# wenz116/lang2seg

Measured on AMD Instinct MI355X. Metric: train images/sec (cycle loss on), 600×1000 input, at 1/2/4/8 MI355X, higher is better.
Workload: dtype bf16; 1 GPU; train_cycle.sh step: ResNet-101 C4 + 7 spatial dynamic filters + att2in2 cycle loss, 600x1000 image, 20-token expression (V=3349), 12000->2000 proposals, 256 RoIs, per-GPU batch 1; variant=cycle, parallelism=dp1

## Files before the change

### include/lang2seg_hip.h

```cpp
#ifndef LANG2SEG_HIP_H
#define LANG2SEG_HIP_H
#include <stdint.h>
#ifdef __HIPCC__
#include <hip/hip_runtime.h>
#else
typedef struct ihipStream_t* hipStream_t;
#endif
#ifdef __cplusplus
extern "C" {
#endif

#define L2S_F32 0
#define L2S_BF16 1

int l2s_version(void);

#define L2S_CONV_RELU 1
#define L2S_CONV_OUT_F32 4
#define L2S_CONV_DECONV2X2 8
#define L2S_CONV_SCATTER 16
#define L2S_ALGO_AUTO 0
#define L2S_ALGO_STAGED 1
#define L2S_ALGO_DMA 2
#define L2S_ALGO_DMA_STAMPED 4
// ... 333 lines not shown
typedef struct { int roi; int cls; float box[4]; float score; int area; } l2s_det_record;
size_t l2s_detect_ws_bytes(int post, int ncls);
int l2s_detect_nms(const float* cls_prob, const float* bbox_pred, const float* rois, const int* nkeep, int post, int ncls, float im_scale,
                   int im_h, int im_w, int bbox_reg, float thresh, float nms_thresh, void* ws, float* boxes_dump, hipStream_t s);
int l2s_detect_select(const void* ws, int post, int ncls, int max_per_image, float im_scale, l2s_det_record* rec, float* mask_rois,
                      int* mask_labels, int cap, int* count, hipStream_t s);
int l2s_detect_paste(const float* mask_prob, int ms, l2s_det_record* rec, const int* count, int cap, int ih, int iw, uint8_t* canvases,
                     hipStream_t s);

typedef struct { int I; int U; int hit; int reserved; } l2s_det_gt;
typedef struct { int det; int cls; int hit; int reserved; long long I; long long U; double key; } l2s_det_choice;
int l2s_detect_gt_iou(const uint8_t* canvases, const l2s_det_record* rec, const int* count, int cap, int ih, int iw, const uint8_t* gt, int Hs,
                      int Ws, const float* gt_box, float im_scale, l2s_det_gt* out, int* gt_area, hipStream_t s);
int l2s_detect_choose(const l2s_det_record* rec, const l2s_det_gt* gt, const int* count, int cap, const int* gt_area, const float* expr,
                      const float* lambdas, int n_lambda, int per_token, int n_tok, l2s_det_choice* out, hipStream_t s);

int l2s_decode_pick(const float* logits, int V1, int t, int sample_max, float temperature, const float* u_in, const uint64_t* seed_dev,
                    uint64_t salt, int* finished, int64_t* seq, float* seq_logprobs, int64_t* next_token, hipStream_t s);
#define L2S_BEAM_MAX 16
#define L2S_BEAM_MAX_T 64
#define L2S_BEAM_RECORD_WORDS(T) (2 * (T) + 2)
typedef struct {
  const float* logits; int ld_logits;
  int V1, B, t, T, R, n_state;
  int* beam_seq; float* beam_seq_logprobs; float* beam_logprobs_sum;
  const float* state_in[4]; float* state_out[4]; int ld_in[4], ld_out[4];
  int64_t* next_tokens; int* parents;
  int* done; int* done_count;
} l2s_beam_step_args;
int l2s_decode_beam_step(const l2s_beam_step_args* a, hipStream_t s);
int l2s_decode_beam_step_rows(const l2s_beam_step_args* a, int rows, int row0, const int* count, hipStream_t s);
int l2s_decode_beam_finish_rows(const int* done, const int* done_count, int B, int T, int rows, int row0, const int* count,
                                int64_t* beam_seq, float* beam_logps, float* beam_p, int* beam_n, int64_t* seq, float* logprobs, hipStream_t s);
int l2s_mask_resize_nearest(const uint8_t* src, int ih, int iw, uint8_t* dst, int H, int W, hipStream_t s);

#define L2S_ROWS_MAX_W 8192
int l2s_masks_to_map(const uint8_t* masks, int rows, int row0, const int* count, int mh, int mw, int H, int W, int Hc, int Wc, float* out,
                     hipStream_t s);
int l2s_adaptive_pool_rows(const void* x, const float* pm, void* y, int rows, int row0, const int* count, int H, int W, int C, int OH, int OW,
                           int ldy, int dtype, hipStream_t s);
int l2s_cap_att_dots_rows(const float* patt, const float* att_h, int ld_att_h, const float* aw, const float* ab, int rows, int row0,
                          const int* count, int L, int D, float* dots, hipStream_t s);
int l2s_cap_apply_gates_rows(const float* P, const float* dots, const float* b_a2c, const float* sums, int ld_sums, const float* c_prev,
                             float* c, float* h, int rows, int row0, const int* count, int L, int R, hipStream_t s);
int l2s_decode_pick_rows(const float* logits, int ld_logits, int V1, int rows, int row0, const int* count, int t, int T, const int64_t* forced,
                         int* finished, int64_t* seq, float* logprobs, int64_t* next_token, float* sum, hipStream_t s);
int l2s_decode_force_rows(const float* logits, int ld_logits, int V1, int rows, int row0, const int* count, int t, int T, const int64_t* targets,
                          const int* lengths, float* logprobs, int64_t* next_token, float* sum, hipStream_t s);
typedef struct { const float* x; int ldx; const float* w; int ld; int n; } l2s_rows_seg;
typedef struct { const float* pre; int ld_pre; const float* pre2; int ld_pre2; const float* add0; const float* add1; l2s_rows_seg seg[2];
                 const float* c_prev; int ld_c_prev; float* c; int ld_c; float* h; int ld_h; } l2s_lstm_rows;
int l2s_lstm_cell_rows(const l2s_lstm_rows* a, int R, int rows, int row0, const int* count, hipStream_t s);
int l2s_cap_att_apply_rows(const float* att, const float* dots, float* att_res, int ld_res, int rows, int row0, const int* count, int L, int R,
                           hipStream_t s);
int l2s_cap_att_dots_groups(const float* patt, const float* att_h, int ld_att_h, const float* aw, const float* ab, int rows, int group,
                            int row0, const int* count, int L, int D, float* dots, hipStream_t s);
int l2s_cap_apply_gates_groups(const float* P, const float* dots, const float* b_a2c, const float* sums, int ld_sums, const float* c_prev,
                               float* c, float* h, int rows, int group, int row0, const int* count, int L, int R, hipStream_t s);
int l2s_cap_att_apply_groups(const float* att, const float* dots, float* att_res, int ld_res, int rows, int group, int row0,
                             const int* count, int L, int R, hipStream_t s);
int l2s_lstm_cell_groups(const l2s_lstm_rows* a, int R, int rows, int group, int row0, const int* count, hipStream_t s);

int l2s_stream_fork(hipStream_t from, hipStream_t to);
int l2s_event_record(int slot, hipStream_t s);
int l2s_event_wait(int slot, hipStream_t s);
int l2s_memset_async(void* p, int value, size_t bytes, hipStream_t s);
int l2s_memcpy_d2d_async(void* dst, const void* src, size_t bytes, hipStream_t s);
void* l2s_tape_begin(const hipStream_t* streams, int n);
int l2s_tape_end(void* tape);
long l2s_tape_size(void* tape);
int l2s_tape_run(void* tape, const hipStream_t* streams, int n);
int l2s_tape_pause(int on);
int l2s_tape_mark(void);
int l2s_tape_time_event(hipStream_t s);
int l2s_time_event_elapsed(int a, int b, float* ms);
int l2s_tape_segments(void* tape);
int l2s_tape_run_segment(void* tape, const hipStream_t* streams, int n, int seg);
int l2s_tape_destroy(void* tape);

typedef struct { long offset; long count; int row_len; int weight_decay; long rowscale_off; float lr_mult;
                 int chunk0;
                 int flags;
                 int reserved; } l2s_sgd_seg;
int l2s_sgd_momentum_range(float* param, float* grad, float* mom, const l2s_sgd_seg* segs, int nseg, const float* rowscale,
                           float lr, float momentum, float wd, float grad_scale, void* shadow, int shadow_dtype, int flags,
                           long lo, long hi, int chunk_lo, int chunk_hi, hipStream_t s);
int l2s_sgd_momentum_range_g16(float* param, const void* grad_bf16, long grad_lo, float* mom, const l2s_sgd_seg* segs, int nseg, const float* rowscale,
                               float lr, float momentum, float wd, float grad_scale, void* shadow, int shadow_dtype,
                               long lo, long hi, int chunk_lo, int chunk_hi, hipStream_t s);
int l2s_sgd_chunk(void);
int l2s_sgd_momentum(float* param, float* grad, float* mom, const l2s_sgd_seg* segs, int nseg, const float* rowscale,
                     float lr, float momentum, float wd, float grad_scale, void* shadow ,
                     int shadow_dtype, int clear_grad ,
                     hipStream_t s);

#ifdef __cplusplus
}
#endif
#endif
```

### lang2seg_amd/_lib.py

```python
import ctypes as C
import os

_HERE = os.path.dirname(os.path.abspath(__file__))
LIB_PATH = os.path.join(_HERE, 'lib', 'liblang2seg_hip.so')
F32, BF16 = 0, 1

vp, i32, i64, f32, u64, sz = C.c_void_p, C.c_int, C.c_long, C.c_float, C.c_uint64, C.c_size_t


class ConvDesc(C.Structure):
    _fields_ = [('x', vp), ('w', vp), ('y', vp), ('bias', vp), ('add', vp), ('ref', vp),
                ('n_img', i32), ('IH', i32), ('IW', i32), ('Cin', i32), ('OH', i32), ('OW', i32), ('Cout', i32),
                ('KH', i32), ('KW', i32), ('stride', i32), ('pad', i32),
                ('ldx', i32), ('ldy', i32), ('ldadd', i32), ('ldref', i32), ('flags', i32),
                ('out_h', i32), ('out_w', i32), ('out_stride', i32), ('tile', i32), ('split_k', i32), ('xcd_mode', i32), ('algo', i32), ('ws', vp), ('ws_floats', sz), ('prio', i32)]


class RoiBlock0Desc(C.Structure):
    _fields_ = [('feat', vp), ('rois', vp), ('w1', vp), ('b1', vp), ('w2', vp), ('b2', vp), ('pooled', vp), ('y1', vp), ('y2', vp),
                ('H', i32), ('W', i32), ('C', i32), ('R', i32), ('P', i32), ('N1', i32), ('N2', i32), ('spatial_scale', C.c_float), ('debug', i32)]


class WgradDesc(C.Structure):
    _fields_ = [('dy', vp), ('x', vp), ('dw', vp),
                ('n_img', i32), ('IH', i32), ('IW', i32), ('Cin', i32), ('OH', i32), ('OW', i32), ('Cout', i32),
                ('KH', i32), ('KW', i32), ('stride', i32), ('pad', i32), ('lddy', i32), ('ldx', i32),
                ('split_k', i32), ('tile', i32), ('ws', vp), ('ws_bytes', sz)]


class WgradProb(C.Structure):
    _fields_ = [('dy', vp * 2), ('x', vp * 2), ('n_img', i32 * 2), ('IH', i32 * 2), ('IW', i32 * 2), ('OH', i32 * 2), ('OW', i32 * 2),
                ('lddy', i32 * 2), ('ldx', i32 * 2), ('dw', vp),
                ('nseg', i32), ('Cin', i32), ('Cout', i32), ('KH', i32), ('KW', i32), ('stride', i32), ('pad', i32),
                ('split', i32), ('ws_off', i64), ('flags', i32), ('reserved', i32)]


class TransposeDesc(C.Structure):
    _fields_ = [('src', vp), ('scale', vp), ('dst', vp), ('Cout', i32), ('taps', i32), ('Cin', i32), ('force_f32', i32)]


class LstmFwdDir(C.Structure):
    _fields_ = [(n, C.c_void_p) for n in ('w_hh', 'b_hh', 'gates_in', 'h_prev', 'c_prev', 'c', 'h', 'act', 'gates_out')]


class LstmBwdDir(C.Structure):
    _fields_ = [(n, C.c_void_p) for n in ('w_hh_T', 'dgates_next', 'dh_ext', 'dc_in', 'act', 'c_prev', 'c', 'dgates', 'dc_prev')]


class GruFwdDir(C.Structure):
    _fields_ = [(n, C.c_void_p) for n in ('w_hh', 'b_hh', 'gates_in', 'h_prev', 'h', 'act')]


class GruBwdDir(C.Structure):
    _fields_ = [(n, C.c_void_p) for n in ('w_hh_T', 'dgh_next', 'dh_ext', 'dh_carry_in', 'act', 'h_prev', 'dgi', 'dgh', 'dh_carry_out')]


class RnnFwdDir(C.Structure):
    _fields_ = [(n, C.c_void_p) for n in ('w_hh', 'b_hh', 'gates_in', 'h_prev', 'h')]


class RnnBwdDir(C.Structure):
    _fields_ = [(n, C.c_void_p) for n in ('w_hh_T', 'dg_next', 'dh_ext', 'h', 'dg')]


class TopdownSeg(C.Structure):
    _fields_ = [('x', vp), ('w', vp), ('ld', i32), ('n', i32)]


class TopdownFwd(C.Structure):
    _fields_ = [('pre', vp), ('add0', vp), ('add1', vp), ('seg', TopdownSeg * 2), ('c_prev', vp), ('c', vp), ('h', vp), ('act', vp)]


class TopdownBwd(C.Structure):
    _fields_ = [('seg', TopdownSeg * 3), ('add0', vp), ('add1', vp), ('dc_in', vp), ('act', vp), ('c_prev', vp), ('c', vp), ('dgates', vp),
                ('dc_prev', vp)]


class RowsSeg(C.Structure):
    _fields_ = [('x', vp), ('ldx', i32), ('w', vp), ('ld', i32), ('n', i32)]


class LstmRows(C.Structure):
    _fields_ = [('pre', vp), ('ld_pre', i32), ('pre2', vp), ('ld_pre2', i32), ('add0', vp), ('add1', vp), ('seg', RowsSeg * 2),
                ('c_prev', vp), ('ld_c_prev', i32), ('c', vp), ('ld_c', i32), ('h', vp), ('ld_h', i32)]


class AdaattFwd(C.Structure):
    _fields_ = [(n, vp) for n in ('pre', 'fcrow', 'w_hh', 'b_hh', 'w_r', 'b_r')] + [('ld_hh', i32), ('ld_r', i32)] + \
               [(n, vp) for n in ('h_prev', 'c_prev', 'c', 'h', 'fake', 'save')]


class AdaattBwd(C.Structure):
    _fields_ = [(n, vp) for n in ('dsn', 't_hh', 't_r')] + [('ld_thh', i32), ('ld_tr', i32)] + \
               [(n, vp) for n in ('dh_ext', 'dfake', 'dc_in', 'save', 'c_prev', 'ds', 'dc_prev')]


class Bottleneck64Desc(C.Structure):
    _fields_ = [(n, vp) for n in ('a', 'x', 'w2', 'w3', 'wd', 'w1n', 'b2', 'b3', 'bd', 'b1n', 'y', 'a_next')] + [(n, i32) for n in ('H', 'W', 'Cx')]


class CapRecurFwdArgs(C.Structure):
    _fields_ = [(n, vp) for n in ('w_h2h', 'b_h2h', 'w_h2att', 'b_h2att', 'patt', 'aw', 'ab', 'P', 'b_a2c', 'sums', 'hs', 'cs', 'save', 'tanh_ws', 'wgt', 'state')] + \
               [(n, i32) for n in ('S', 'R', 'AH', 'L')]


class CapRecurBwdArgs(C.Structure):
    _fields_ = [(n, vp) for n in ('w_h2h', 'w_h2att', 'P', 'aw', 'save', 'cs', 'wgt', 'tanh_ws', 'dho', 'dsums', 'da2c', 'ddot', 'datt_h', 'state')] + \
               [(n, i32) for n in ('S', 'R', 'AH', 'L', 'ld_ddot', 'ld_datt_h')]


class BeamStepArgs(C.Structure):
    _fields_ = [('logits', vp), ('ld_logits', i32)] + [(n, i32) for n in ('V1', 'B', 't', 'T', 'R', 'n_state')] + \
               [(n, vp) for n in ('beam_seq', 'beam_seq_logprobs', 'beam_logprobs_sum')] + \
               [('state_in', vp * 4), ('state_out', vp * 4), ('ld_in', i32 * 4), ('ld_out', i32 * 4)] + \
               [(n, vp) for n in ('next_tokens', 'parents', 'done', 'done_count')]


class SgdSeg(C.Structure):
    _fields_ = [('offset', i64), ('count', i64), ('row_len', i32), ('weight_decay', i32), ('rowscale_off', i64),
                ('lr_mult', f32), ('chunk0', i32), ('flags', i32), ('reserved', i32)]


CONV_RELU, CONV_OUT_F32, CONV_DECONV2X2, CONV_SCATTER = 1, 4, 8, 16
LOSS_RPN_CLS, LOSS_RPN_BOX, LOSS_CLS, LOSS_BOX, LOSS_MASK, LOSS_CAP, LOSS_TOTAL, LOSS_RESPONSE = range(8)

SIGS = {
    'l2s_version': (i32, []),
    'l2s_conv_plan_name': (C.c_char_p, [vp, i32]),
    'l2s_last_kernel': (C.c_char_p, []),
    'l2s_roialign_block0_fwd': (i32, [C.POINTER(RoiBlock0Desc), vp]),
    'l2s_conv_igemm': (i32, [C.POINTER(ConvDesc), i32, vp]),
    'l2s_conv_wgrad': (i32, [C.POINTER(WgradDesc), i32, vp]),
    'l2s_wgrad_ws_bytes': (sz, [C.POINTER(WgradDesc), i32]),
    'l2s_wgrad_variant': (i32, [i32, i32, i32, i32, i32, i32, i32, i64, i32]),
    'l2s_wgrad_tiles': (i64, [i32, i32, i32, i32, i32]),
    'l2s_conv_wgrad_grouped': (i32, [vp, vp, i32, i32, i32, vp, sz, vp]),
    'l2s_weight_cast': (i32, [vp, vp, vp, i32, i32, i32, i32, vp]),
    'l2s_weight_transpose': (i32, [vp, vp, vp, i32, i32, i32, i32, vp]),
    'l2s_colsum': (i32, [vp, i32, i32, i32, vp, vp, i64, i32, vp]),
    'l2s_weight_transpose_batched': (i32, [vp, i32, i32, i32, vp]),
    'l2s_stem_conv': (i32, [vp, vp, vp, vp, vp, i32, i32, i32, i32, i32, vp]),
    'l2s_stem_pack_bytes': (C.c_size_t, []),
    'l2s_stem_pack': (i32, [vp, vp, vp]),
    'l2s_stem_pool_bf16': (i32, [vp, vp, vp, vp, vp, i32, i32, i32, i32, i32, i32, vp]),
    'l2s_maxpool3x3s2': (i32, [vp, vp, i32, i32, i32, i32, i32, i32, vp]),
    'l2s_fill_f32': (i32, [vp, f32, i64, vp]),
    'l2s_cast': (i32, [vp, i32, vp, i32, i64, vp]),
    'l2s_add3': (i32, [vp, vp, vp, vp, i64, i32, vp]),
    'l2s_avgpool_fwd': (i32, [vp, vp, i32, i32, i32, i32, vp]),
    'l2s_avgpool_bwd': (i32, [vp, vp, vp, vp, i32, i32, i32, i32, vp]),
    'l2s_adaptive_pool_fwd': (i32, [vp, vp, vp, i32, i32, i32, i32, i32, i32, i32, vp]),
    'l2s_adaptive_pool_bwd': (i32, [vp, i32, i32, i32, vp, vp, vp, i32, i32, i32, i32, i32, i32, vp]),
    'l2s_mask_downsample': (i32, [vp, vp, i32, i32, i32, i32, vp]),
    'l2s_dropout_mask': (i32, [vp, i64, f32, vp, u64, vp]),
    'l2s_counter_inc': (i32, [vp, vp]),
    'l2s_stamp': (i32, [vp, vp]),
    'l2s_rpn_decode': (i32, [vp, i32, vp, i32, i32, i32, i32, f32, f32, vp, vp, vp, vp]),
    'l2s_sort_topk': (i32, [vp, vp, i32, i32, vp, vp, vp, vp, vp]),
    'l2s_nms_workspace_bytes': (sz, [i32]),
    'l2s_sort_ws_ints': (i64, [i32]),
    'l2s_nms': (i32, [vp, i32, f32, i32, i32, vp, vp, vp, vp]),
    'l2s_gather_rois': (i32, [vp, vp, vp, vp, i32, vp, vp, vp]),
    'l2s_random_keys': (i32, [vp, i64, vp, u64, vp]),
    'l2s_anchor_target_ws_ints': (i64, [i32]),
    'l2s_anchor_target': (i32, [vp, i32, vp, i32, i32, i32, i32, f32, f32, vp, vp, f32, f32, i32, f32, vp, vp, vp, vp, vp, vp]),
    'l2s_proposal_target': (i32, [vp, vp, vp, i32, vp, i32, vp, i32, i32, vp, vp, vp, i32, i32, i32, f32, f32, f32,
                                  vp, vp, vp, i32, i32, vp, vp, vp, vp, vp, vp, vp, vp, vp]),
    'l2s_roialign_fwd': (i32, [vp, i32, i32, i32, vp, i32, i32, f32, vp, i32, vp]),
    'l2s_roialign_bwd': (i32, [vp, i32, i32, i32, vp, i32, i32, f32, vp, i32, vp]),
    'l2s_rpn_loss': (i32, [vp, i32, vp, vp, vp, vp, i32, i32, i32, f32, f32, vp, vp, i32, i32, vp, vp, vp]),
    'l2s_anchor_target_count': (vp, [vp]),
    'l2s_rcnn_loss': (i32, [vp, i32, vp, vp, vp, vp, i32, i32, f32, vp, vp, i32, i32, vp]),
    'l2s_mask_loss': (i32, [vp, i32, vp, vp, vp, i32, i32, f32, vp, vp, vp]),
    'l2s_total_loss': (i32, [vp, f32, vp]),
    'l2s_maskpred_ws_floats': (i64, [i32, i32]),
    'l2s_maskpred_bwd': (i32, [vp, vp, vp, i32, i32, i32, vp, vp, vp, vp, vp, vp, vp, i32, vp]),
    'l2s_maskpred_bwd_dx': (i32, [vp, vp, vp, i32, i32, i32, vp, vp, vp, vp, vp, i32, vp]),
    'l2s_maskpred_bwd_reduce': (i32, [vp, vp, vp, i32, i32, vp, vp, vp]),
    'l2s_linear_fwd': (i32, [vp, i32, vp, i32, vp, vp, i32, i32, i32, i32, i32, i32, vp]),
    'l2s_linear_bwd_x': (i32, [vp, i32, vp, vp, i32, i32, i32, i32, i32, vp, vp, i64, vp]),
    'l2s_linear_bwd_x_ws_floats': (i64, [i32, i32, i32]),
    'l2s_linear_bwd_w': (i32, [vp, i32, vp, i32, vp, vp, i32, i32, i32, vp]),
    'l2s_act_bwd': (i32, [vp, vp, i64, i32, vp]),
    'l2s_mask_relu_cast': (i32, [vp, vp, vp, vp, i32, i64, vp]),
    'l2s_embed_fwd': (i32, [vp, vp, vp, vp, i32, i32, i32, vp]),
    'l2s_embed_bwd': (i32, [vp, vp, vp, vp, vp, i32, i32, i32, vp]),
    'l2s_lstm_cell_fwd': (i32, [vp, vp, vp, vp, vp, i32, vp]),
    'l2s_lstm_cell_bwd': (i32, [vp, vp, vp, vp, vp, vp, vp, i32, vp]),
    'l2s_dynfilter_fwd': (i32, [vp, vp, vp, vp, vp, vp, i32, i32, i32, i32, i32, vp]),
    'l2s_dynfilter_ws_floats': (i64, [i32, i32, i32]),
    'l2s_dynfilter_bwd': (i32, [vp, vp, vp, vp, vp, vp, vp, vp, vp, vp, vp, i32, i32, i32, i32, i32, vp, vp]),
    'l2s_dynfilter_bwd_finish': (i32, [vp, vp, vp, vp, i32, i32, i32, vp]),
    'l2s_scale_mask': (i32, [vp, vp, vp, vp, C.c_long, i32, vp]),
    'l2s_conv3x3_c3': (i32, [vp, vp, vp, vp, i32, i32, i32, vp]),
    'l2s_maxpool2x2_fwd': (i32, [vp, vp, i32, i32, i32, i32, i32, vp]),
    'l2s_maxpool2x2_bwd': (i32, [vp, vp, vp, i32, i32, i32, i32, i32, i32, vp]),
    'l2s_cropalign_fwd': (i32, [vp, i32, i32, i32, vp, i32, i32, f32, f32, vp, i32, vp]),
    'l2s_cropalign_bwd': (i32, [vp, i32, i32, i32, vp, i32, i32, f32, f32, vp, i32, vp]),
    'l2s_roipool_fwd': (i32, [vp, i32, i32, i32, vp, i32, i32, f32, vp, vp, i32, vp]),
    'l2s_roipool_bwd': (i32, [vp, vp, i32, i32, i32, vp, i32, vp]),
    'l2s_rle_from_string': (i32, [C.c_char_p, vp, i32]),
    'l2s_prep_geometry': (i32, [i32, i32, i32, i32, C.POINTER(C.c_double), C.POINTER(i32), C.POINTER(i32)]),
    'l2s_prep_image': (i32, [vp, i32, i32, C.c_double, C.c_double, C.c_double, C.c_double, i32, i32, vp, vp]),
    'l2s_rle_ws_words': (i64, [i32, i32, i32]),
    'l2s_rle_to_mask': (i32, [vp, vp, i32, i32, i32, i32, i32, i32, vp, vp, vp]),
    'l2s_eval_pick': (i32, [vp, vp, vp, vp, i32, i32, f32, i32, i32, vp, i32, vp, vp, vp, vp]),
    'l2s_eval_mask_iou': (i32, [vp, i32, vp, vp, i32, i32, i32, i32, vp, vp]),
    'l2s_rle_encode_ws_words': (i64, [i32, i32]),
    'l2s_rle_encode_chunk_rows': (i32, []),
    'l2s_rle_from_mask': (i32, [vp, i32, i32, vp, i32, vp, vp, vp, vp]),
    'l2s_rle_from_masks': (i32, [vp, i32, vp, i32, i32, vp, i32, vp, vp, vp, vp]),
    'l2s_rle_to_string': (i32, [vp, i32, C.c_char_p, i32]),
    'l2s_detect_ws_bytes': (sz, [i32, i32]),
    'l2s_detect_nms': (i32, [vp, vp, vp, vp, i32, i32, f32, i32, i32, i32, f32, f32, vp, vp, vp]),
    'l2s_detect_select': (i32, [vp, i32, i32, i32, f32, vp, vp, vp, i32, vp, vp]),
    'l2s_detect_paste': (i32, [vp, i32, vp, vp, i32, i32, i32, vp, vp]),
    'l2s_detect_gt_iou': (i32, [vp, vp, vp, i32, i32, i32, vp, i32, i32, vp, f32, vp, vp, vp]),
    'l2s_detect_choose': (i32, [vp, vp, vp, i32, vp, vp, C.POINTER(f32), i32, i32, i32, vp, vp]),
    'l2s_decode_pick': (i32, [vp, i32, i32, i32, f32, vp, vp, u64, vp, vp, vp, vp, vp]),
# ... 129 lines not shown
```

### lang2seg_amd/csrc/conv_wgrad.hip

```cpp
#include "wgrad_common.h"
#include <stdlib.h>

namespace {
using namespace l2s_wgrad;

template <typename T> struct WGT;
template <> struct WGT<bf16_t> { static constexpr int BKP = 32; static constexpr int PADB = 32; };
template <> struct WGT<float> { static constexpr int BKP = 16; static constexpr int PADB = 64; };

template <typename T, int BM, int BN, int TX, int D, int KSTEP = 1, int WGM = 2, int WGN = 2>
__device__ __forceinline__ void wgrad_tile(const wgp& p, int co0, int ci0, int tg, int split_idx, int nsplit, float* out, bool accumulate, char* smem) {
  constexpr int ES = (int)sizeof(T);
  constexpr int VE = 16 / ES;
  constexpr int BKP0 = WGT<T>::BKP;
  constexpr int BKP = BKP0 * KSTEP;
  constexpr int RB = BKP + TX - 1;
  constexpr int NT = 64 * WGM * WGN;
  constexpr int WM = BM / WGM, WN = BN / WGN, TM = WM / 16, TN = WN / 16;
  constexpr int LRA = BM * ES + WGT<T>::PADB, LRB = BN * ES + WGT<T>::PADB;
  constexpr int VPA = BM / VE, VPB = BN / VE;
  constexpr int TPR = NT / BKP;
  static_assert(NT % BKP == 0 && VPA % TPR == 0 && VPB % TPR == 0, "loader mapping");
  constexpr int NVA = VPA / TPR, NVB = VPB / TPR;
  constexpr int BUF = BKP * LRA + RB * LRB;

  const int tid = threadIdx.x, lane = tid & 63, wave = tid >> 6;
  const int wm = wave / WGN, wn = wave % WGN;
  const int ky = TX == 3 ? tg : tg / p.KW, kx = TX == 3 ? 0 : tg - ky * p.KW;
  const int fr = lane & 15, fg = lane >> 4;

  f32x4 acc[TX][TM][TN];
#pragma unroll
  for (int t = 0; t < TX; ++t)
#pragma unroll
    for (int i = 0; i < TM; ++i)
#pragma unroll
      for (int j = 0; j < TN; ++j) acc[t][i][j] = (f32x4){0.f, 0.f, 0.f, 0.f};

  auto compute = [&](int cur) {
    const char* a = smem + cur * BUF;
    const char* b = a + BKP * LRA;
    if constexpr (sizeof(T) == 2) {
      const int trow0 = 4 * fg + ((lane >> 2) & 3), tcol = 8 * (lane & 3);
#pragma unroll
      for (int h = 0; h < KSTEP; ++h) {
        const int trow = trow0 + h * 32;
        uint4 fa[TM];
#pragma unroll
        for (int i = 0; i < TM; ++i) fa[i] = lds_frag(a + trow * LRA + (wm * WM + i * 16) * 2 + tcol, LRA);
#pragma unroll
        for (int t = 0; t < TX; ++t) {
          uint4 fb[TN];
#pragma unroll
          for (int j = 0; j < TN; ++j) fb[j] = lds_frag(b + (trow + t) * LRB + (wn * WN + j * 16) * 2 + tcol, LRB);
#pragma unroll
          for (int i = 0; i < TM; ++i)
#pragma unroll
            for (int j = 0; j < TN; ++j)
              acc[t][i][j] = __builtin_amdgcn_mfma_f32_16x16x32_bf16(__builtin_bit_cast(bf16x8, fb[j]), __builtin_bit_cast(bf16x8, fa[i]), acc[t][i][j], 0, 0, 0);
        }
      }
    } else {
#pragma unroll
      for (int ks = 0; ks < BKP / 4; ++ks) {
        float fa[TM];
#pragma unroll
        for (int i = 0; i < TM; ++i) fa[i] = *(const float*)(a + (ks * 4 + fg) * LRA + (wm * WM + i * 16 + fr) * 4);
#pragma unroll
        for (int t = 0; t < TX; ++t) {
          float fb[TN];
#pragma unroll
          for (int j = 0; j < TN; ++j) fb[j] = *(const float*)(b + (ks * 4 + fg + t) * LRB + (wn * WN + j * 16 + fr) * 4);
#pragma unroll
          for (int i = 0; i < TM; ++i)
#pragma unroll
            for (int j = 0; j < TN; ++j) acc[t][i][j] = __builtin_amdgcn_mfma_f32_16x16x4f32(fb[j], fa[i], acc[t][i][j], 0, 0, 0);
        }
      }
    }
  };

#pragma unroll
  for (int seg = 0; seg < L2S_WGRAD_MAX_SEG; ++seg) {
    if (seg >= p.nseg) break;
    const int n_img = p.n_img[seg], IH = p.IH[seg], IW = p.IW[seg], OH = p.OH[seg], OW = p.OW[seg], lddy = p.lddy[seg], ldx = p.ldx[seg];
    const int Wv = OW + (TX == 3 ? 1 : 0);
    const int ohwv = OH * Wv;
    const int Mv = n_img * ohwv;
    int sa, sb, sc;
    slice_step(BKP, ohwv, Wv, sa, sb, sc);
    const int nslices = (Mv + BKP - 1) / BKP;
    const int per = (nslices + nsplit - 1) / nsplit;
    const int s_begin = split_idx * per;
    const int NS = max(0, min(nslices, s_begin + per) - s_begin);
// ... 24 lines not shown
      const int ix = TX == 3 ? x : x * p.stride - p.pad + kx;
      const bool ok = n < n_img && x >= 0 && x < OW && iy >= 0 && iy < IH && ix >= 0 && ix < IW;
      return ok ? (unsigned)(((n * IH + iy) * IW + ix) * ldx * ES) + bcol : OOR;
    };
    auto issue = [&](uint4 (&ra)[NVA], uint4 (&rb)[NVB], uint4 (&rt)[NVB]) {
      {
        const bool ok = ax < OW && an < n_img;
        const unsigned o = ok ? (unsigned)((((an * OH + ay) * OW + ax) * lddy) * ES) + acol : OOR;
#pragma unroll
        for (int j = 0; j < NVA; ++j) ra[j] = __builtin_bit_cast(uint4, __builtin_amdgcn_raw_buffer_load_b128(rdy, acok[j] ? o + j * 16 : OOR, 0, 0));
        advance(an, ay, ax);
      }
      {
        const unsigned o = xoff(bn, by, bx);
#pragma unroll
        for (int j = 0; j < NVB; ++j) rb[j] = __builtin_bit_cast(uint4, __builtin_amdgcn_raw_buffer_load_b128(rxx, bcok[j] ? o + j * 16 : OOR, 0, 0));
        advance(bn, by, bx);
      }
      if (TX == 3) {
        const unsigned o = tail ? xoff(tn, ty, tx) : OOR;
#pragma unroll
        for (int j = 0; j < NVB; ++j) rt[j] = __builtin_bit_cast(uint4, __builtin_amdgcn_raw_buffer_load_b128(rxx, bcok[j] ? o + j * 16 : OOR, 0, 0));
        advance(tn, ty, tx);
      }
    };
    auto store_slice = [&](int buf, const uint4 (&ra)[NVA], const uint4 (&rb)[NVB], const uint4 (&rt)[NVB]) {
      char* a = smem + buf * BUF + lrow * LRA + lq * NVA * 16;
      char* b = smem + buf * BUF + BKP * LRA + lrow * LRB + lq * NVB * 16;
#pragma unroll
      for (int j = 0; j < NVA; ++j) *(uint4*)(a + j * 16) = ra[j];
#pragma unroll
      for (int j = 0; j < NVB; ++j) *(uint4*)(b + j * 16) = rb[j];
      if (TX == 3 && tail) {
#pragma unroll
        for (int j = 0; j < NVB; ++j) *(uint4*)(b + BKP * LRB + j * 16) = rt[j];
      }
    };

    uint4 qa[D][NVA], qb[D][NVB], qt[D][TX == 3 ? NVB : 1];
    auto iss = [&](int s_) { if constexpr (TX == 3) issue(qa[s_], qb[s_], qt[s_]); else issue(qa[s_], qb[s_], qb[s_]); };
    auto sto = [&](int buf, int s_) { if constexpr (TX == 3) store_slice(buf, qa[s_], qb[s_], qt[s_]); else store_slice(buf, qa[s_], qb[s_], qb[s_]); };
#pragma unroll
    for (int s = 0; s < D; ++s)
      if (s < NS) iss(s);
    __syncthreads();
    sto(0, 0);
    if (D < NS) iss(0);
    int t0 = 0;
    for (; t0 + 2 * D <= NS; t0 += D) {
#pragma unroll
      for (int s = 0; s < D; ++s) {
        const int t = t0 + s;
        const int nxt = (s + 1) % D;
        __syncthreads();
        sto((t + 1) & 1, nxt);
        iss(nxt);
        compute(t & 1);
      }
    }
#pragma unroll
    for (int s = 0; s < 2 * D; ++s) {
      const int t = t0 + s;
      if (t < NS) {
        const int nxt = (s + 1) % D;
        __syncthreads();
        if (t + 1 < NS) {
          sto((t + 1) & 1, nxt);
          if (t + 1 + D < NS) iss(nxt);
        }
        compute(t & 1);
      }
    }
  }
  const long Kw = (long)p.KH * p.KW * p.Cin;
#pragma unroll
  for (int t = 0; t < TX; ++t) {
    const int tap = TX == 3 ? ky * p.KW + t : tg;
#pragma unroll
    for (int i = 0; i < TM; ++i) {
      const int co = co0 + wm * WM + i * 16 + fr;
#pragma unroll
      for (int j = 0; j < TN; ++j) {
        const int ci = ci0 + wn * WN + j * 16 + fg * 4;
        if (co < p.Cout && ci < p.Cin) dw_store((float4*)(out + (long)co * Kw + (long)tap * p.Cin + ci), f4(acc[t][i][j]), accumulate);
      }
    }
  }
}

template <typename T, int BM, int BN, int TX, int KSTEP = 1> constexpr size_t wgrad_lds() {
  return 2 * (size_t)(WGT<T>::BKP * KSTEP * (BM * sizeof(T) + WGT<T>::PADB) + (WGT<T>::BKP * KSTEP + TX - 1) * (BN * sizeof(T) + WGT<T>::PADB));
}

template <typename T, int BM, int BN, int TX, int D>
__global__ __launch_bounds__(256) void wgrad_kernel(const wgp p, int cblocks, float* ws, long slab) {
  extern __shared__ __attribute__((aligned(16))) char smem[];
  const int tg = blockIdx.y / cblocks, ci0 = (blockIdx.y - tg * cblocks) * BN;
  float* out = slab ? ws + (long)blockIdx.z * slab : p.dw;
  wgrad_tile<T, BM, BN, TX, D>(p, blockIdx.x * BM, ci0, tg, blockIdx.z, gridDim.z, out, slab == 0, smem);
}


typedef l2s::wgrad_tile_prefix wg_prefix;

template <typename T, int BM, int BN, int TX, int D, int KSTEP, int WGM = 2, int WGN = 2>
__global__ __launch_bounds__(64 * WGM * WGN) void wgrad_grouped_kernel(const wgp* __restrict__ tab, const wg_prefix pre, float* ws) {
  extern __shared__ __attribute__((aligned(16))) char smem[];
  const int G = pre.tile0[pre.n];
  for (int L = blockIdx.x; L < G; L += gridDim.x) {
    int t;
    const wgp p = tab[tile_of(pre, L, t)];
    const int co_tiles = (p.Cout + BM - 1) / BM, ci_tiles = (p.Cin + BN - 1) / BN;
    const int split = p.split > 1 ? p.split : 1;
    const int sp = t % split; t /= split;
    const int cot = t % co_tiles, rest = t / co_tiles, cit = rest % ci_tiles, tg = rest / ci_tiles;
    float* out = split > 1 ? ws + p.ws_off + (long)sp * ((long)p.Cout * p.KH * p.KW * p.Cin) : p.dw;
    wgrad_tile<T, BM, BN, TX, D, KSTEP, WGM, WGN>(p, cot * BM, cit * BN, tg, sp, split, out, split == 1 && !(p.flags & 1), smem);
    __syncthreads();
  }
}

__device__ __forceinline__ void reduce_slabs(float* dw, const float* ws, long n4, long slab, int split, bool accumulate) {
  for (long e = blockIdx.x * (long)blockDim.x + threadIdx.x; e < n4; e += (long)gridDim.x * blockDim.x) {
    float4 s = ((const float4*)ws)[e];
    for (int k = 1; k < split; ++k) s = add4(s, ((const float4*)(ws + (long)k * slab))[e]);
    dw_store((float4*)dw + e, s, accumulate);
  }
}

__global__ __launch_bounds__(256) void wgrad_reduce_grouped_kernel(const wgp* __restrict__ tab, const float* __restrict__ ws) {
  const wgp p = tab[blockIdx.y];
  if (p.split <= 1) return;
  const long slab = (long)p.Cout * p.KH * p.KW * p.Cin;
  reduce_slabs(p.dw, ws + p.ws_off, slab / 4, slab, p.split, !(p.flags & 1));
}

__global__ __launch_bounds__(256) void wgrad_reduce_kernel(float* __restrict__ dw, const float* __restrict__ ws, long n4, long slab, int split) {
  reduce_slabs(dw, ws, n4, slab, split, true);
}

using namespace l2s_knobs;
int variant_of(int Cin, int Cout, int KH, int KW, int stride, int pad, int same_hw, long M, int tile) {
  const bool row3 = KH == 3 && KW == 3 && stride == 1 && pad == 1 && same_hw;
  const bool big = M >= 8192 && Cout >= 512 && Cin >= 512;
  if (row3 && tile == 256 && wgrad_row3_dma && (M >= wgrad_row3_min_m || (wgrad_row3_wide && Cin >= 512 && Cout >= 512)) && Cout % 128 == 0 && Cin % 128 == 0) return 5;
  if (row3) return (tile == 128 || ((!tile || tile == 256) && Cout >= 512)) ? 3 : 2;
  if (wgrad_1x1_dma && tile == 256 && big && KH * KW == 1 && stride == 1 && pad == 0 && same_hw && Cout % 256 == 0 && Cin % 256 == 0) return 6;
  if (tile == 256 && big && KH * KW == 1 && Cout % 256 == 0 && Cin % 256 == 0) return 4;
  return (tile == 128 || ((!tile || tile == 256) && big && KH * KW == 1)) ? 1 : 0;
}
int variant_of(const l2s_wgrad_desc& d) {
  return variant_of(d.Cin, d.Cout, d.KH, d.KW, d.stride, d.pad, d.OH == d.IH && d.OW == d.IW, (long)d.n_img * d.OH * d.OW, d.tile);
}
void variant_tile(int v, int& bm, int& bn, int& tx) {
  if (v == 4 || v == 6) { bm = 256; bn = 256; tx = 1; return; }
  if (v == 5) { bm = 128; bn = 128; tx = 3; return; }
  bm = (v == 1 || v == 3) ? 128 : 64; bn = v == 1 ? 128 : 64; tx = v >= 2 ? 3 : 1;
}
long variant_tiles(int v, int Cin, int Cout, int KH, int KW) {
  if (v == 5) return l2s::wgrad_row3_dma_tiles(Cin, Cout);
  int bm, bn, tx; variant_tile(v, bm, bn, tx);
  return (long)cdiv(Cout, bm) * cdiv(Cin, bn) * (tx == 3 ? KH : KH * KW);
}

wgp prob_of(const l2s_wgrad_desc& d) {
  wgp p = {};
  p.dy[0] = d.dy; p.x[0] = d.x; p.dw = d.dw;
  p.n_img[0] = d.n_img; p.IH[0] = d.IH; p.IW[0] = d.IW; p.OH[0] = d.OH; p.OW[0] = d.OW; p.lddy[0] = d.lddy; p.ldx[0] = d.ldx;
  p.nseg = 1; p.Cin = d.Cin; p.Cout = d.Cout; p.KH = d.KH; p.KW = d.KW; p.stride = d.stride; p.pad = d.pad;
  return p;
}

template <typename T, int BM, int BN, int TX, int D>
int launch_single(const l2s_wgrad_desc& d, int split, hipStream_t st) {
  const wgp p = prob_of(d);
  const int cblocks = cdiv(d.Cin, BN);
  const long slab = split > 1 ? (long)d.Cout * d.KH * d.KW * d.Cin : 0;
  dim3 grid(cdiv(d.Cout, BM), (TX == 3 ? d.KH : d.KH * d.KW) * cblocks, split);
  float* ws = d.ws;
  L2S_LAUNCH((wgrad_kernel<T, BM, BN, TX, D>), grid, dim3(256), (wgrad_lds<T, BM, BN, TX>()), st, p, cblocks, ws, slab);
  if (split > 1) {
    const long n4 = slab / 4;
    long gb = (n4 + 255) / 256; if (gb > 4096) gb = 4096;
    float* dw = d.dw; const float* wsc = d.ws;
    L2S_LAUNCH(wgrad_reduce_kernel, dim3((int)gb), dim3(256), 0, st, dw, wsc, n4, slab, split);
  }
  return l2s_check_launch();
}

template <typename T, int BM, int BN, int TX, int D, int KSTEP, int WGM = 2, int WGN = 2>
int launch_grouped(const wgp* tab, const wg_prefix& pre, float* ws, bool any_split, hipStream_t st) {
  size_t lds = wgrad_lds<T, BM, BN, TX, KSTEP>();
  constexpr size_t want = 54000, want_big = 83000;
  if (BM * BN >= 128 * 128) { if (want_big > lds) lds = want_big; }
  else if (want > lds) lds = want;
  int grid = pre.tile0[pre.n];
  {
    const int cap = l2s_knobs::wgrad_grid_cap & 0xffff, vmask = l2s_knobs::wgrad_grid_cap >> 16;
    const int var = BM == 256 ? 4 : (TX == 3 ? (BM == 128 ? 3 : 2) : (BM == 128 ? 1 : 0));
    if (cap > 0 && grid > cap && (vmask == 0 || ((vmask >> var) & 1))) grid = cap;
  }
  WGRAD_LAUNCH((wgrad_grouped_kernel<T, BM, BN, TX, D, KSTEP, WGM, WGN>), dim3(grid), dim3(64 * WGM * WGN), lds, st, tab, pre, ws);
  if (any_split) {
    const float* wsc = ws;
    L2S_LAUNCH(wgrad_reduce_grouped_kernel, dim3(64, pre.n), dim3(256), 0, st, tab, wsc);
  }
  return l2s_check_launch();
}

bool prob_ok(const wgp& p, int dtype) {
  const int ve = dtype == L2S_BF16 ? 8 : 4;
  const long esz = dtype == L2S_BF16 ? 2 : 4;
  if (p.nseg < 1 || p.nseg > L2S_WGRAD_MAX_SEG || p.Cin % ve || p.Cout % ve || ((long)p.Cout * p.KH * p.KW * p.Cin) % 4) return false;
  for (int s = 0; s < p.nseg; ++s) {
    if (p.lddy[s] % ve || p.ldx[s] % ve) return false;
    const long M = (long)p.n_img[s] * p.OH[s] * p.OW[s];
    if (M >= (1 << 24)) return false;
    if ((long)p.n_img[s] * p.IH[s] * p.IW[s] * p.ldx[s] * esz >= (1L << 31) || M * p.lddy[s] * esz >= (1L << 31)) return false;
  }
  return true;
}

}

extern "C" size_t l2s_wgrad_grouped_ws_bytes(int variant) { return variant == 5 ? l2s::wgrad_row3_dma_ws_bytes(l2s_knobs::wgrad_row3_dma_wgs) : 0; }
extern "C" int l2s_wgrad_variant(int Cin, int Cout, int KH, int KW, int stride, int pad, int same_hw, long M, int tile) {
  return variant_of(Cin, Cout, KH, KW, stride, pad, same_hw, M, tile);
}
extern "C" long l2s_wgrad_tiles(int variant, int Cin, int Cout, int KH, int KW) { return variant_tiles(variant, Cin, Cout, KH, KW); }

extern "C" int l2s_conv_wgrad_grouped(const l2s_wgrad_prob* table_dev, const l2s_wgrad_prob* table_host, int nprob, int variant, int dtype,
                                      float* ws, size_t ws_bytes, hipStream_t stream) {
  if (!table_dev || !table_host || nprob < 1 || nprob > L2S_WGRAD_MAX_GROUP || variant < 0 || variant > 6) return L2S_EINVAL;
  if (variant >= 5 && dtype != L2S_BF16) return L2S_EINVAL;
  for (int i = 0; i < nprob; ++i) if (!prob_ok(table_host[i], dtype) || !table_host[i].dw) return L2S_EINVAL;
  if (variant == 6) return l2s::wgrad_1x1_dma_launch(table_dev, table_host, nprob, stream);
  if (variant == 5) return l2s::wgrad_row3_dma_launch(table_dev, table_host, nprob, ws, ws_bytes, l2s_knobs::wgrad_row3_dma_wgs, stream);
  bool any_split = false;
  for (int i = 0; i < nprob; ++i) {
    const wgp& q = table_host[i];
    if ((variant == 2 || variant == 3) && !(q.KH == 3 && q.KW == 3 && q.stride == 1 && q.pad == 1)) return L2S_EINVAL;
    if (q.split > 1) {
      const long slab = (long)q.Cout * q.KH * q.KW * q.Cin;
      if (!ws || q.ws_off < 0 || (q.ws_off % 4) || (size_t)(q.ws_off + q.split * slab) * 4 > ws_bytes) return L2S_EINVAL;
      any_split = true;
    }
  }
  wg_prefix pre;
  if (fill_tile_prefix(pre, table_host, nprob, [&](const wgp& q) { return variant_tiles(variant, q.Cin, q.Cout, q.KH, q.KW) * (q.split > 1 ? q.split : 1); }) >= (1L << 30)) return L2S_EINVAL;
#define GO(T, KS)                                                                                \
  switch (variant) {                                                                             \
    case 0: return launch_grouped<T, 64, 64, 1, 2, KS>(table_dev, pre, ws, any_split, stream);    \
    case 1: return launch_grouped<T, 128, 128, 1, 2, KS>(table_dev, pre, ws, any_split, stream);  \
    case 2: return launch_grouped<T, 64, 64, 3, 2, KS>(table_dev, pre, ws, any_split, stream);    \
    case 3: return launch_grouped<T, 128, 64, 3, 2, KS>(table_dev, pre, ws, any_split, stream);   \
    default: break;                                                                              \
  }
  if (dtype == L2S_BF16) {
    if (variant == 4) return launch_grouped<bf16_t, 256, 256, 1, 2, 1, 4, 2>(table_dev, pre, ws, any_split, stream);
    GO(bf16_t, 2)
  }
  if (dtype == L2S_F32) { GO(float, 1) }
#undef GO
  return L2S_EINVAL;
}

static int plan_split(const l2s_wgrad_desc& d, int variant, int dtype, size_t ws_bytes) {
  int bm, bn, tx; variant_tile(variant, bm, bn, tx);
  const long tiles = variant_tiles(variant, d.Cin, d.Cout, d.KH, d.KW);
  const int bkp = dtype == L2S_BF16 ? 32 : 16;
  const long Mv = (long)d.n_img * d.OH * (d.OW + (tx == 3 ? 1 : 0));
  const int slices = cdiv(Mv, bkp);
  int split = d.split_k;
  if (split <= 0) {
    constexpr int min_wg = 256;
    split = (int)((min_wg + tiles - 1) / tiles);
    const int maxs = slices / 8 > 0 ? slices / 8 : 1;
    if (split > maxs) split = maxs;
  }
  if (split > slices) split = slices;
  if (split < 1) split = 1;
  if (split > 64) split = 64;
  const long slab = (long)d.Cout * d.KH * d.KW * d.Cin * 4;
  if (split > 1 && (long)split * slab > (long)ws_bytes) split = ws_bytes >= (size_t)(2 * slab) ? (int)(ws_bytes / slab) : 1;
  return split;
}

extern "C" size_t l2s_wgrad_ws_bytes(const l2s_wgrad_desc* d, int dtype) {
  if (!d) return 0;
  const int v = variant_of(*d);
  const int split = plan_split(*d, v, dtype, (size_t)1 << 40);
  return split > 1 ? (size_t)split * d->Cout * d->KH * d->KW * d->Cin * 4 : 0;
}

extern "C" int l2s_conv_wgrad(const l2s_wgrad_desc* d, int dtype, hipStream_t stream) {
  if (!d || !d->dy || !d->x || !d->dw) return L2S_EINVAL;
  if (!prob_ok(prob_of(*d), dtype)) return L2S_EINVAL;
  const int v = variant_of(*d);
  const int split = plan_split(*d, v, dtype, d->ws ? d->ws_bytes : 0);
#define GO(T)                                                                                    \
  switch (v) {                                                                                   \
    case 0: return launch_single<T, 64, 64, 1, 4>(*d, split, stream);                             \
    case 1: return launch_single<T, 128, 128, 1, 3>(*d, split, stream);                           \
    case 2: return launch_single<T, 64, 64, 3, 4>(*d, split, stream);                             \
    default: return launch_single<T, 128, 64, 3, 3>(*d, split, stream);                           \
  }
  if (dtype == L2S_BF16) { GO(bf16_t) }
  if (dtype == L2S_F32) { GO(float) }
#undef GO
  return L2S_EINVAL;
}
```

### lang2seg_amd/csrc/conv_wgrad_dma.hip

```cpp
#include "wgrad_common.h"

namespace {
using namespace l2s_wgrad;

constexpr int BM = 128, BN = 128, BKP = 64, ROWB = 256;
constexpr int A_BYTES = BKP * ROWB;
constexpr int B_ROWS = 68;
constexpr int STG = A_BYTES + B_ROWS * ROWB;
constexpr int NPW = 4;
constexpr int TILE_FLOATS = 3 * BM * BN;

__device__ __forceinline__ long wg_lo(long g, long U, long G) { return g * U / G; }

template <int KO, int NST>
__global__ __launch_bounds__(512) void wgrad_row3_dma_kernel(const wgp* __restrict__ tab, const l2s::wgrad_sk_plan plan, float* __restrict__ ws) {
  extern __shared__ __attribute__((aligned(16))) char smem[];
  const int tid = threadIdx.x, lane = tid & 63;
  const int wave = __builtin_amdgcn_readfirstlane(tid >> 6);
  const int wm = wave >> 2, wn = wave & 3;
  const int fr = lane & 15, fg = lane >> 4;
  const int G = gridDim.x;
  const int L = (G & 7) == 0 ? (int)((blockIdx.x & 7) * (G >> 3) + (blockIdx.x >> 3)) : (int)blockIdx.x;
  const long u_lo = wg_lo(L, plan.U, G), u_hi = wg_lo(L + 1, plan.U, G);
  const unsigned lds0 = (unsigned)(uintptr_t)(__attribute__((address_space(3))) char*)smem;

  const int g4 = lane >> 4;
  unsigned vc[2];
#pragma unroll
  for (int par = 0; par < 2; ++par) vc[par] = (unsigned)(((lane & 15) ^ ((4 * par + g4) << 1)) << 4);
  const int trow = 4 * fg + ((lane >> 2) & 3), cb = (lane & 3) >> 1, inb = (lane & 1) << 3;
  unsigned aoff[4], boff[3][2];
#pragma unroll
  for (int i = 0; i < 4; ++i) aoff[i] = (unsigned)(trow * ROWB + (((wm * 8 + 2 * i + cb) ^ ((trow & 7) << 1)) << 4) + inb);
#pragma unroll
  for (int t = 0; t < 3; ++t)
#pragma unroll
    for (int j = 0; j < 2; ++j)
      boff[t][j] = (unsigned)(A_BYTES + (trow + t) * ROWB + (((wn * 4 + 2 * j + cb) ^ (((trow + t) & 7) << 1)) << 4) + inb);
  const bool roleA = lane < 8;
  const int myrow = roleA ? 8 * wave + lane : (lane < 12 ? 4 * wave + (lane - 8) : (lane < 16 ? 32 + 4 * wave + (lane - 12) : 64 + ((lane - 16) & 3)));
  long u = u_lo;
  int part = 0;
  const int xcd = blockIdx.x & 7, ix = blockIdx.x >> 3;
  const int npass = plan.mode == 1 ? plan.Q + (plan.r ? 1 : 0) : 0;
  for (int pass = 0; plan.mode == 1 ? pass < npass : u < u_hi; ++pass) {
    int plo, S, tile, s0, s1;
    long slab_id;
    if (plan.mode == 1) {
      const int tl = ix % plan.T, c = ix / plan.T;
      int gt, pieces, piece;
      if (pass < plan.Q) { gt = (8 * pass + xcd) * plan.T + tl; pieces = plan.k1; piece = c; slab_id = (long)gt * plan.k1 + c; }
      else {
        const int j = xcd / plan.m, sub = xcd - j * plan.m;
        const int gl = j * plan.T + tl;
        gt = 8 * plan.Q * plan.T + gl; pieces = plan.m * plan.k1; piece = sub * plan.k1 + c;
        slab_id = (long)8 * plan.Q * plan.T * plan.k1 + (long)gl * pieces + piece;
      }
      S = plan.S[0];
      const int tpp = 3 * plan.T;
      plo = gt / tpp; tile = gt - plo * tpp;
      s0 = (int)((long)piece * S / pieces); s1 = (int)((long)(piece + 1) * S / pieces);
      if (pieces == 1) slab_id = -1;
      if (s0 >= s1) continue;
    } else {
      plo = 0; int phi = plan.n;
      while (phi - plo > 1) { const int mid = (plo + phi) >> 1; if (plan.unit0[mid] <= u) plo = mid; else phi = mid; }
      S = plan.S[plo];
      const long rr = u - plan.unit0[plo];
      tile = (int)(rr / S); s0 = (int)(rr - (long)tile * S);
      s1 = (int)(((long)S - s0) < (u_hi - u) ? (long)S : s0 + (u_hi - u));
      slab_id = (s0 == 0 && s1 == S) ? -1 : (long)L * 2 + part;
    }
    const wgp p = tab[plo];
    const int co_tiles = p.Cout / BM, ci_tiles = p.Cin / BN;
    const int cot = tile % co_tiles, rest = tile / co_tiles, cit = rest % ci_tiles, ky = rest / ci_tiles;
    const int co0 = cot * BM, ci0 = cit * BN;

    f32x4 acc[3][4][2];
#pragma unroll
    for (int t = 0; t < 3; ++t)
#pragma unroll
      for (int i = 0; i < 4; ++i)
#pragma unroll
        for (int j = 0; j < 2; ++j) acc[t][i][j] = (f32x4){0.f, 0.f, 0.f, 0.f};

    int sbase = 0;
#pragma unroll
    for (int seg = 0; seg < L2S_WGRAD_MAX_SEG; ++seg) {
      if (seg >= p.nseg) break;
      const int n_img = p.n_img[seg], OH = p.OH[seg], OW = p.OW[seg], lddy = p.lddy[seg], ldx = p.ldx[seg];
      const int Wv = OW + 1, ohwv = OH * Wv, Mv = n_img * ohwv;
      const int nsl = (Mv + BKP - 1) / BKP;
      const int sa_ = (s0 > sbase ? s0 : sbase) - sbase, sb_ = (s1 < sbase + nsl ? s1 : sbase + nsl) - sbase;
      sbase += nsl;
      if (sa_ >= sb_) continue;
      const int n = sb_ - sa_;
      int ja, jb, jc;
      slice_step(BKP, ohwv, Wv, ja, jb, jc);
// ... 40 lines not shown
        dma_1kib(rxx, vo[2], sb + (unsigned)(A_BYTES + (4 * wave) * ROWB));
        dma_1kib(rxx, vo[3], sb + (unsigned)(A_BYTES + (32 + 4 * wave) * ROWB));
        if (wave == 0) dma_1kib(rxx, vo[4], sb + (unsigned)(A_BYTES + 64 * ROWB));
      };
      uint4 fa[2][4], fb[2][3][2];
      auto read_all = [&](int stage) {
        const char* base = smem + stage * STG;
#pragma unroll
        for (int h = 0; h < 2; ++h) {
#pragma unroll
          for (int i = 0; i < 4; ++i) fa[h][i] = lds_frag(base + aoff[i] + h * 32 * ROWB, ROWB);
#pragma unroll
          for (int t = 0; t < 3; ++t)
#pragma unroll
            for (int j = 0; j < 2; ++j) fb[h][t][j] = lds_frag(base + boff[t][j] + h * 32 * ROWB, ROWB);
        }
      };
      auto mma_all = [&]() {
#pragma unroll
        for (int h = 0; h < 2; ++h)
#pragma unroll
          for (int t = 0; t < 3; ++t)
#pragma unroll
            for (int i = 0; i < 4; ++i)
#pragma unroll
              for (int j = 0; j < 2; ++j) {
                if (!(KO & 1)) acc[t][i][j] = __builtin_amdgcn_mfma_f32_16x16x32_bf16(__builtin_bit_cast(bf16x8, fb[h][t][j]), __builtin_bit_cast(bf16x8, fa[h][i]), acc[t][i][j], 0, 0, 0);
              }
      };
      const int grp = wave >> 2;
      lds_wait(); wg_barrier();
      auto wait_keep = [&](int younger) {
        if (wave == 0) wait_vm_keep<NPW + 1, NST - 2>(younger);
        else wait_vm_keep<NPW, NST - 2>(younger);
      };
#pragma unroll
      for (int q = 0; q < NST - 1; ++q)
        if (q < n) { prep(); request(q); }
      wait_keep(n - 1 < NST - 2 ? n - 1 : NST - 2);
      if (NST - 1 < n) prep();
      wg_barrier();
      if (grp == 1) wg_barrier();
      int st = 0;
      unsigned long long* stamps = (unsigned long long*)(ws + (long)gridDim.x * 3 * TILE_FLOATS) + grp * 32 * 8;
      const bool stamping = (KO & 8) && blockIdx.x == 0 && (wave & 3) == 0 && lane == 0 && pass == 0 && seg == 0;
      auto stamp = [&](int t, int i) {
        if constexpr ((KO & 8) != 0) {
          if (t < 32) { const unsigned long long c = __builtin_amdgcn_s_memtime(); if (stamping) stamps[t * 8 + i] = c; }
        }
      };
      for (int t = 0; t < n; ++t) {
        const int stq = st == 0 ? NST - 1 : st - 1;
        const int younger = n - 2 - t < NST - 2 ? (n - 2 - t < 0 ? 0 : n - 2 - t) : NST - 2;
        stamp(t, 0);
        const bool more = t + NST < n && !(KO & 16);
        if (more) prep_a();
        if (!(KO & 4)) read_all(st);
        if (more) prep_b();
        stamp(t, 1);
        if (t + NST - 1 < n && !(KO & 2)) request(stq);
        stamp(t, 2);
        lds_wait();
        if (more) prep_c();
        stamp(t, 3);
        if (grp == 1) wait_keep(younger);
        wg_barrier();
        stamp(t, 4);
        __builtin_amdgcn_sched_barrier(0);
        mma_all();
        __builtin_amdgcn_sched_barrier(0);
        stamp(t, 5);
        if (grp == 0) wait_keep(younger);
        stamp(t, 6);
        wg_barrier();
        stamp(t, 7);
        st = st == NST - 1 ? 0 : st + 1;
      }
      if (grp == 0) wg_barrier();
    }

    const bool full = slab_id < 0;
    const long Kw = 9L * p.Cin;
    float* slab = ws + (full ? 0 : slab_id) * TILE_FLOATS;
#pragma unroll
    for (int t = 0; t < 3; ++t)
#pragma unroll
      for (int i = 0; i < 4; ++i) {
        const int col = wm * 64 + i * 16 + fr;
#pragma unroll
        for (int j = 0; j < 2; ++j) {
          const int cil = wn * 32 + j * 16 + fg * 4;
          if (full) dw_store((float4*)(p.dw + (long)(co0 + col) * Kw + (long)(ky * 3 + t) * p.Cin + ci0 + cil), f4(acc[t][i][j]), !(p.flags & 1));
          else *(float4*)(slab + ((long)(t * BM + col) * BN + cil)) = f4(acc[t][i][j]);
        }
      }
    part = 1;
    u += s1 - s0;
  }
}

__global__ __launch_bounds__(256) void wgrad_row3_reduce_kernel(const wgp* __restrict__ tab, const l2s::wgrad_sk_plan plan, const float* __restrict__ ws, int G) {
  int T = blockIdx.y, pi = 0;
  for (; pi < plan.n; ++pi) {
    const int tiles = (int)((plan.unit0[pi + 1] - plan.unit0[pi]) / plan.S[pi]);
    if (T < tiles) break;
    T -= tiles;
  }
  if (pi >= plan.n) return;
  const wgp p = tab[pi];
  const int S = plan.S[pi];
  long g0, g1, slab0 = 0;
  const long a = plan.unit0[pi] + (long)T * S, b = a + S;
  if (plan.mode == 1) {
    const long gt = (long)pi * 3 * plan.T + T, first_last = (long)8 * plan.Q * plan.T;
    const int pieces = gt < first_last ? plan.k1 : plan.m * plan.k1;
    if (pieces == 1) return;
    slab0 = gt < first_last ? gt * plan.k1 : first_last * plan.k1 + (gt - first_last) * pieces;
    g0 = 0; g1 = pieces - 1;
  } else {
    g0 = a * G / plan.U; g1 = (b - 1) * G / plan.U;
    while (g0 + 1 < G && wg_lo(g0 + 1, plan.U, G) <= a) ++g0;
    while (g0 > 0 && wg_lo(g0, plan.U, G) > a) --g0;
    while (g1 + 1 < G && wg_lo(g1 + 1, plan.U, G) <= b - 1) ++g1;
    while (g1 > 0 && wg_lo(g1, plan.U, G) > b - 1) --g1;
    if (g0 == g1) return;
  }
  const int co_tiles = p.Cout / BM, ci_tiles = p.Cin / BN;
  const int cot = T % co_tiles, rest = T / co_tiles, cit = rest % ci_tiles, ky = rest / ci_tiles;
  const long Kw = 9L * p.Cin;
  for (int e = blockIdx.x * blockDim.x + threadIdx.x; e < TILE_FLOATS / 4; e += gridDim.x * blockDim.x) {
    float4 s = make_float4(0.f, 0.f, 0.f, 0.f);
    for (long g = g0; g <= g1; ++g) {
      const long sl = plan.mode == 1 ? slab0 + g : g * 2 + (wg_lo(g, plan.U, G) >= a ? 0 : 1);
      s = add4(s, ((const float4*)(ws + sl * TILE_FLOATS))[e]);
    }
    const int f = e * 4, t = f / (BM * BN), col = (f - t * BM * BN) / BN, cil = f % BN;
    dw_store((float4*)(p.dw + (long)(cot * BM + col) * Kw + (long)(ky * 3 + t) * p.Cin + cit * BN + cil), s, !(p.flags & 1));
  }
}

}

namespace l2s {


bool wgrad_row3_dma_ok(const l2s_wgrad_prob& q) {
  if (!(q.KH == 3 && q.KW == 3 && q.stride == 1 && q.pad == 1) || q.Cin % BN || q.Cout % BM || q.split > 1) return false;
  for (int s = 0; s < q.nseg; ++s)
    if (q.OH[s] != q.IH[s] || q.OW[s] != q.IW[s] || (q.OW[s] + 1) * q.OH[s] < 1) return false;
  return true;
}
long wgrad_row3_dma_tiles(int Cin, int Cout) { return (long)(Cout / BM) * (Cin / BN) * 3; }
size_t wgrad_row3_dma_ws_bytes(int G) { return (size_t)G * 3 * TILE_FLOATS * sizeof(float); }

int wgrad_row3_dma_launch(const l2s_wgrad_prob* tab_dev, const l2s_wgrad_prob* tab_host, int nprob, float* ws, size_t ws_bytes, int G, hipStream_t st) {
  if (G < 1 || nprob < 1 || nprob > L2S_WGRAD_MAX_GROUP) return L2S_EINVAL;
  wgrad_sk_plan plan;
  plan.n = nprob;
  long U = 0;
  int total_tiles = 0;
  for (int i = 0; i < nprob; ++i) {
    const l2s_wgrad_prob& q = tab_host[i];
    if (!wgrad_row3_dma_ok(q)) return L2S_EINVAL;
    int S = 0;
    for (int s = 0; s < q.nseg; ++s) S += cdiv((long)q.n_img[s] * q.OH[s] * (q.OW[s] + 1), BKP);
    const int tiles = (int)wgrad_row3_dma_tiles(q.Cin, q.Cout);
    plan.unit0[i] = U; plan.S[i] = S;
    U += (long)tiles * S;
    total_tiles += tiles;
  }
  for (int i = nprob; i <= L2S_WGRAD_MAX_GROUP; ++i) plan.unit0[i] = U;
  for (int i = nprob; i < L2S_WGRAD_MAX_GROUP; ++i) plan.S[i] = 1;
  plan.U = U;
  if (U < 1) return L2S_OK;
  if ((long)G > U) G = (int)U;
  if (U / 24 < G) { G = (int)(U / 24) & ~7; if (G < 8) G = U < 8 ? (int)U : 8; }
  plan.mode = 0; plan.T = plan.Ng = plan.k1 = plan.Q = plan.r = plan.m = 0;
  if (l2s_knobs::row3_plan_mode != 0 && (G & 7) == 0) {
    const int T = (int)wgrad_row3_dma_tiles(tab_host[0].Cin, tab_host[0].Cout) / 3, P = G / 8;
    bool same = true;
    for (int i = 1; i < nprob; ++i) same = same && plan.S[i] == plan.S[0] && tab_host[i].Cin == tab_host[0].Cin && tab_host[i].Cout == tab_host[0].Cout;
    const int Ng = 3 * nprob, Q = Ng / 8, r = Ng - 8 * Q;
    if (same && T >= 1 && P % T == 0 && (r == 0 || 8 % r == 0) && (long)(P / T) * (Q ? 1 : 8 / (r ? r : 1)) <= plan.S[0]) {
      plan.mode = 1; plan.T = T; plan.Ng = Ng; plan.k1 = P / T; plan.Q = Q; plan.r = r; plan.m = r ? 8 / r : 1;
    }
  }
  long nslabs = plan.mode == 1 ? (long)G * (plan.Q + (plan.r ? 1 : 0)) : (long)G * 2;
  if (plan.mode == 1 && ws_bytes < (size_t)nslabs * TILE_FLOATS * sizeof(float)) { plan.mode = 0; nslabs = (long)G * 2; }
  if (!ws || ws_bytes < (size_t)nslabs * TILE_FLOATS * sizeof(float)) return L2S_EINVAL;
#define GO(KO_, NST_) WGRAD_LAUNCH((wgrad_row3_dma_kernel<KO_, NST_>), dim3(G), dim3(512), (size_t)NST_ * STG, st, tab_dev, plan, ws);
#ifdef L2S_TOOLS
  switch (l2s_knobs::row3_form) {
    case 1: GO(1, 4) break; case 2: GO(2, 4) break; case 5: GO(5, 4) break; case 6: GO(6, 4) break; case 7: GO(7, 4) break;
    case 8: GO(8, 4) break; case 12: GO(12, 4) break; case 24: GO(24, 4) break; case 10: GO(10, 4) break;
    default: GO(0, 4) break;
  }
#else
  GO(0, 4)
#endif
#undef GO
  const float* wsc = ws;
  L2S_LAUNCH(wgrad_row3_reduce_kernel, dim3(12, total_tiles), dim3(256), 0, st, tab_dev, plan, wsc, G);
  return l2s_check_launch();
}

}
```

### lang2seg_amd/csrc/conv_wgrad_dma1.hip

```cpp
#include "wgrad_common.h"

namespace {
using namespace l2s_wgrad;

constexpr int BM = 256, BN = 256, KP = 32, ROWB = 512;
constexpr int A_BYTES = KP * ROWB;
constexpr int STG = 2 * A_BYTES;
constexpr int NP = 4;

template <int NST>
__global__ __launch_bounds__(512) void wgrad_1x1_dma_kernel(const wgp* __restrict__ tab, const l2s::wgrad_tile_prefix pre) {
  extern __shared__ __attribute__((aligned(16))) char smem[];
  const int tid = threadIdx.x, lane = tid & 63;
  const int wave = __builtin_amdgcn_readfirstlane(tid >> 6);
  const int grp = wave >> 2;
  const int wm = wave >> 1, wn = wave & 1;
  const int fr = lane & 15, fg = lane >> 4;
  int t;
  const wgp p = tab[tile_of(pre, (int)blockIdx.x, t)];
  const int co_tiles = p.Cout / BM;
  const int co0 = (t % co_tiles) * BM, ci0 = (t / co_tiles) * BN;
  const int M0 = p.n_img[0] * p.OH[0] * p.OW[0], M1 = p.nseg > 1 ? p.n_img[1] * p.OH[1] * p.OW[1] : 0;
  const int ns0 = (M0 + KP - 1) / KP, KT = ns0 + (M1 + KP - 1) / KP;
  const unsigned lds0 = (unsigned)(uintptr_t)(__attribute__((address_space(3))) char*)smem;
  const i32x4s rdy0 = rsrc(p.dy[0], (long)M0 * p.lddy[0] * 2L), rx0 = rsrc(p.x[0], (long)M0 * p.ldx[0] * 2L);
  const i32x4s rdy1 = rsrc(p.nseg > 1 ? p.dy[1] : p.dy[0], (long)M1 * p.lddy[p.nseg > 1] * 2L), rx1 = rsrc(p.nseg > 1 ? p.x[1] : p.x[0], (long)M1 * p.ldx[p.nseg > 1] * 2L);
  const int g = lane >> 5;
  const int sc = (lane & 31) ^ (2 * ((2 * wave + g) & 15));
  const int rowq[2] = {2 * wave + g, 16 + 2 * wave + g};
  const int trow = 4 * fg + ((lane >> 2) & 3), cb = (lane & 3) >> 1, inb = (lane & 1) << 3;
  unsigned aoff[4], boff[8];
#pragma unroll
  for (int i = 0; i < 4; ++i) aoff[i] = (unsigned)(trow * ROWB + (((wm * 8 + 2 * i + cb) ^ (2 * trow)) << 4) + inb);
#pragma unroll
  for (int j = 0; j < 8; ++j) boff[j] = (unsigned)(A_BYTES + trow * ROWB + (((wn * 16 + 2 * j + cb) ^ (2 * trow)) << 4) + inb);

  auto request = [&](int stage, int ts) {
    const bool s1 = ts >= ns0;
    const int m0 = (s1 ? ts - ns0 : ts) * KP;
    const int nv = (s1 ? M1 : M0) - m0;
    const int ldd = p.lddy[s1], ldxx = p.ldx[s1];
    const i32x4s rd = s1 ? rdy1 : rdy0, rxx = s1 ? rx1 : rx0;
    const unsigned sb = lds0 + (unsigned)(stage * STG);
#pragma unroll
    for (int q = 0; q < 2; ++q) {
      const int r = rowq[q];
      const unsigned va = r < nv ? (unsigned)(((m0 + r) * ldd + co0 + sc * 8) * 2) : OOR;
      dma_1kib(rd, va, sb + (unsigned)((wave + 8 * q) * 1024));
    }
#pragma unroll
    for (int q = 0; q < 2; ++q) {
      const int r = rowq[q];
      const unsigned vb = r < nv ? (unsigned)(((m0 + r) * ldxx + ci0 + sc * 8) * 2) : OOR;
      dma_1kib(rxx, vb, sb + (unsigned)(A_BYTES + (wave + 8 * q) * 1024));
    }
  };
  f32x4 acc[4][8];
#pragma unroll
  for (int i = 0; i < 4; ++i)
#pragma unroll
    for (int j = 0; j < 8; ++j) acc[i][j] = (f32x4){0.f, 0.f, 0.f, 0.f};
  uint4 fa[4], fb[8];
  auto read_all = [&](int stage) {
    const char* base = smem + stage * STG;
#pragma unroll
    for (int i = 0; i < 4; ++i) fa[i] = lds_frag(base + aoff[i], ROWB);
#pragma unroll
    for (int j = 0; j < 8; ++j) fb[j] = lds_frag(base + boff[j], ROWB);
  };
  auto mma_all = [&]() {
#pragma unroll
    for (int i = 0; i < 4; ++i)
#pragma unroll
      for (int j = 0; j < 8; ++j)
        acc[i][j] = __builtin_amdgcn_mfma_f32_16x16x32_bf16(__builtin_bit_cast(bf16x8, fb[j]), __builtin_bit_cast(bf16x8, fa[i]), acc[i][j], 0, 0, 0);
  };
  auto wait_keep = [&](int younger) { wait_vm_keep<NP, NST - 2>(younger); };
#pragma unroll
  for (int s = 0; s < NST - 1; ++s)
    if (s < KT) request(s, s);
  wait_keep(min(NST - 2, KT - 1));
  wg_barrier();
  if (grp == 1) wg_barrier();
  int st = 0;
  for (int ts = 0; ts < KT; ++ts) {
    const int stn = st == 0 ? NST - 1 : st - 1;
    read_all(st);
    if (ts + NST - 1 < KT) request(stn, ts + NST - 1);
    lds_wait();
    const int younger = max(0, min(NST - 2, KT - 2 - ts));
    if (grp == 1) wait_keep(younger);
    wg_barrier();
    __builtin_amdgcn_sched_barrier(0);
    mma_all();
    __builtin_amdgcn_sched_barrier(0);
    if (grp == 0) wait_keep(younger);
    wg_barrier();
    st = st == NST - 1 ? 0 : st + 1;
  }
  if (grp == 0) wg_barrier();
  const bool overwrite = p.flags & 1;
#pragma unroll
  for (int i = 0; i < 4; ++i) {
    const long co = co0 + wm * 64 + i * 16 + fr;
#pragma unroll
    for (int j = 0; j < 8; ++j) {
      const int ci = ci0 + wn * 128 + j * 16 + fg * 4;
      dw_store((float4*)(p.dw + co * p.Cin + ci), f4(acc[i][j]), !overwrite);
    }
  }
}

}

namespace l2s {

bool wgrad_1x1_dma_ok(const l2s_wgrad_prob& q) {
  if (!(q.KH == 1 && q.KW == 1 && q.stride == 1 && q.pad == 0) || q.Cin % BN || q.Cout % BM || q.split > 1 || q.nseg < 1 || q.nseg > 2) return false;
  for (int s = 0; s < q.nseg; ++s) {
    if (q.OH[s] != q.IH[s] || q.OW[s] != q.IW[s] || (long)q.n_img[s] * q.OH[s] * q.OW[s] < 1) return false;
    if (q.lddy[s] % 8 || q.ldx[s] % 8 || ((uintptr_t)q.dy[s] & 15) || ((uintptr_t)q.x[s] & 15)) return false;
  }
  return !((uintptr_t)q.dw & 15);
}
long wgrad_1x1_dma_tiles(int Cin, int Cout) { return (long)(Cout / BM) * (Cin / BN); }

int wgrad_1x1_dma_launch(const l2s_wgrad_prob* tab_dev, const l2s_wgrad_prob* tab_host, int nprob, hipStream_t st) {
  for (int i = 0; i < nprob; ++i) if (!wgrad_1x1_dma_ok(tab_host[i])) return L2S_EINVAL;
  wgrad_tile_prefix pre;
  const long t = fill_tile_prefix(pre, tab_host, nprob, [](const wgp& q) { return wgrad_1x1_dma_tiles(q.Cin, q.Cout); });
  const size_t lds = (size_t)4 * STG;
  WGRAD_LAUNCH(wgrad_1x1_dma_kernel<4>, dim3((unsigned)t), dim3(512), lds, st, tab_dev, pre);
  return l2s_check_launch();
}

}
```

### lang2seg_amd/csrc/misc_kernels.hip

```cpp
#include "common.h"
#include "../../include/lang2seg_hip.h"
#include "pool_bins.h"
#include "rows.h"

namespace {

__device__ __forceinline__ uint64_t mix64(uint64_t z) {
  z += 0x9E3779B97F4A7C15ull;
  z = (z ^ (z >> 30)) * 0xBF58476D1CE4E5B9ull;
  z = (z ^ (z >> 27)) * 0x94D049BB133111EBull;
  return z ^ (z >> 31);
}

inline int grid_for(long n, int block = 256, int cap = 2048) {
  long g = (n + block - 1) / block;
  if (g < 1) g = 1;
  return (int)(g > cap ? cap : g);
}

__global__ void weight_cast_kernel(const float* __restrict__ src, const float* __restrict__ scale, void* dst,
                                   long per_row, long total, int dt) {
  for (long i = blockIdx.x * (long)blockDim.x + threadIdx.x; i < total; i += (long)gridDim.x * blockDim.x) {
    float v = src[i];
    if (scale) v *= scale[i / per_row];
    stx(dst, i, dt, v);
  }
}

__global__ void weight_transpose_kernel(const float* __restrict__ src, const float* __restrict__ scale, void* dst,
                                        int Cout, int taps, int Cin, int dt) {
  __shared__ float tile[32][33];
  const int tap = blockIdx.z;
  const int co0 = blockIdx.y * 32, ci0 = blockIdx.x * 32;
  const int tx = threadIdx.x & 31, ty = threadIdx.x >> 5;
  for (int r = ty; r < 32; r += 8) {
    int co = co0 + r, ci = ci0 + tx;
    float v = 0.f;
    if (co < Cout && ci < Cin) { v = src[((long)co * taps + tap) * Cin + ci]; if (scale) v *= scale[co]; }
    tile[r][tx] = v;
  }
  __syncthreads();
  const int otap = taps - 1 - tap;
  for (int r = ty; r < 32; r += 8) {
    int ci = ci0 + r, co = co0 + tx;
    if (co < Cout && ci < Cin) stx(dst, ((long)ci * taps + otap) * Cout + co, dt, tile[tx][r]);
  }
}

__global__ __launch_bounds__(256) void weight_transpose_batched_kernel(const l2s_transpose_desc* __restrict__ table, int n, int total, int dt_in) {
  __shared__ float tile[64][65];
  const int tid = threadIdx.x;
  int di = 0, base = 0;
  l2s_transpose_desc d = table[0];
  int tci = (d.Cin + 63) / 64, tco = (d.Cout + 63) / 64, ntiles = tci * tco * d.taps;
  for (int tt = blockIdx.x; tt < total; tt += gridDim.x) {
    while (tt >= base + ntiles && di + 1 < n) {
      base += ntiles; ++di;
      d = table[di];
      tci = (d.Cin + 63) / 64; tco = (d.Cout + 63) / 64; ntiles = tci * tco * d.taps;
    }
    const int t = tt - base;
    const int dt = (d.force_f32 & 1) ? L2S_F32 : dt_in;
    const bool src16 = d.force_f32 & 2;
    const bool vec_in = (d.Cin & 3) == 0, vec_out = (d.Cout & 7) == 0;
    const int tap = t / (tci * tco), rem = t - tap * (tci * tco);
    const int co0 = (rem / tci) * 64, ci0 = (rem % tci) * 64;
    __syncthreads();
    {
      const int c4 = (tid & 15) * 4;
#pragma unroll
      for (int pass = 0; pass < 4; ++pass) {
        const int r = (tid >> 4) + pass * 16;
        const int co = co0 + r, ci = ci0 + c4;
        float4 v = make_float4(0.f, 0.f, 0.f, 0.f);
        if (co < d.Cout) {
          const float* sp = d.src + ((long)co * d.taps + tap) * d.Cin + ci;
          if (src16) {
            const bf16_t* hp = (const bf16_t*)d.src + ((long)co * d.taps + tap) * d.Cin + ci;
            if (vec_in && ci + 3 < d.Cin) { const uint2 u = *(const uint2*)hp; v = make_float4(bf2f(u.x & 0xffffu), bf2f(u.x >> 16), bf2f(u.y & 0xffffu), bf2f(u.y >> 16)); }
            else { if (ci < d.Cin) v.x = bf2f(hp[0]); if (ci + 1 < d.Cin) v.y = bf2f(hp[1]); if (ci + 2 < d.Cin) v.z = bf2f(hp[2]); if (ci + 3 < d.Cin) v.w = bf2f(hp[3]); }
          } else
          if (vec_in && ci + 3 < d.Cin) v = *(const float4*)sp;
          else { if (ci < d.Cin) v.x = sp[0]; if (ci + 1 < d.Cin) v.y = sp[1]; if (ci + 2 < d.Cin) v.z = sp[2]; if (ci + 3 < d.Cin) v.w = sp[3]; }
          if (d.scale) { const float sc = d.scale[co]; v.x *= sc; v.y *= sc; v.z *= sc; v.w *= sc; }
        }
        tile[r][c4] = v.x; tile[r][c4 + 1] = v.y; tile[r][c4 + 2] = v.z; tile[r][c4 + 3] = v.w;
// ... 359 lines not shown
      float d = ldx(dy, b + off_all + c, dt);
      if (pm) d += m * ldx(dy, b + off_mask + c, dt);
      g += d * inv;
    }
  }
  long o = (long)pix * C + c;
  if (ref && !(ldx(ref, o, dt) > 0.f)) g = 0.f;
  stx(dx, o, dt, g);
}

__global__ __launch_bounds__(256) void adaptive_pool_bwd_bf16x8_kernel(const bf16_t* __restrict__ dy, int lddy, int off_all, int off_mask, const float* __restrict__ pm,
                                                                      bf16_t* dx, const bf16_t* __restrict__ ref, int H, int W, int C, int OH, int OW) {
  const int pix = blockIdx.x, yy = pix / W, xx = pix - yy * W;
  const int c = (blockIdx.y * blockDim.x + threadIdx.x) * 8;
  if (c >= C) return;
  float g[8];
#pragma unroll
  for (int k = 0; k < 8; ++k) g[k] = 0.f;
  const float m = pm ? pm[pix] : 0.f;
  const int oyc = (yy * OH) / H, oxc = (xx * OW) / W;
  const int oya = OH <= H ? max(0, oyc - 1) : 0, oyb = OH <= H ? min(OH - 1, oyc + 1) : OH - 1;
  const int oxa = OW <= W ? max(0, oxc - 1) : 0, oxb = OW <= W ? min(OW - 1, oxc + 1) : OW - 1;
  for (int oy = oya; oy <= oyb; ++oy) {
    const int y0 = bin_lo(oy, H, OH), y1 = bin_hi(oy, H, OH);
    if (yy < y0 || yy >= y1) continue;
    for (int ox = oxa; ox <= oxb; ++ox) {
      const int x0 = bin_lo(ox, W, OW), x1 = bin_hi(ox, W, OW);
      if (xx < x0 || xx >= x1) continue;
      const float inv = 1.f / (float)((y1 - y0) * (x1 - x0));
      const long b = (long)(oy * OW + ox) * lddy;
      const uint4 a = *(const uint4*)(dy + b + off_all + c);
      uint4 q = make_uint4(0, 0, 0, 0);
      if (pm) q = *(const uint4*)(dy + b + off_mask + c);
      const uint32_t aw[4] = {a.x, a.y, a.z, a.w}, qw[4] = {q.x, q.y, q.z, q.w};
#pragma unroll
      for (int k = 0; k < 4; ++k) {
        float d0 = __uint_as_float(aw[k] << 16), d1 = __uint_as_float(aw[k] & 0xFFFF0000u);
        if (pm) { d0 += m * __uint_as_float(qw[k] << 16); d1 += m * __uint_as_float(qw[k] & 0xFFFF0000u); }
        g[2 * k] += d0 * inv; g[2 * k + 1] += d1 * inv;
      }
    }
  }
  const long o = (long)pix * C + c;
  uint4 r = make_uint4(0x3f803f80u, 0x3f803f80u, 0x3f803f80u, 0x3f803f80u);
  if (ref) r = *(const uint4*)(ref + o);
  const uint32_t rw[4] = {r.x, r.y, r.z, r.w};
  uint32_t ow[4];
#pragma unroll
  for (int k = 0; k < 4; ++k) {
    float v0 = g[2 * k], v1 = g[2 * k + 1];
    if (!(__uint_as_float(rw[k] << 16) > 0.f)) v0 = 0.f;
    if (!(__uint_as_float(rw[k] & 0xFFFF0000u) > 0.f)) v1 = 0.f;
    ow[k] = (uint32_t)f2bf(v0) | ((uint32_t)f2bf(v1) << 16);
  }
  *(uint4*)(dx + o) = make_uint4(ow[0], ow[1], ow[2], ow[3]);
}

__global__ void mask_downsample_kernel(const uint8_t* mask, float* out, int H, int W, int h, int w) {
  const int o = blockIdx.x * (blockDim.x >> 6) + (threadIdx.x >> 6), lane = threadIdx.x & 63;
  if (o >= h * w) return;
  const int oy = o / w, ox = o - oy * w;
  const float v = wave_bin_vote([&](int yy, int xx) { return mask[(long)yy * W + xx]; }, bin_lo(oy, H, h), bin_hi(oy, H, h), bin_lo(ox, W, w),
                                bin_hi(ox, W, w), lane);
  if (lane == 0) out[o] = v;
}

__global__ void counter_inc_kernel(uint64_t* c) { *c += 1; }
__global__ void stamp_kernel(uint64_t* out) { *out = wall_clock64(); }
__global__ void dropout_kernel(float* m, long n, float p, const uint64_t* seed_dev, uint64_t salt) {
  const uint64_t seed = mix64(*seed_dev * 0x9E3779B97F4A7C15ull + salt);
  const float keep = 1.f - p, inv = keep > 0.f ? 1.f / keep : 0.f;
  for (long i = blockIdx.x * (long)blockDim.x + threadIdx.x; i < n; i += (long)gridDim.x * blockDim.x) {
    uint32_t r = (uint32_t)(mix64(seed * 0x100000001B3ull + (uint64_t)i) >> 40);
    m[i] = ((float)r * (1.f / 16777216.f) < keep) ? inv : 0.f;
  }
}
__global__ void keys_kernel(uint32_t* k, long n, const uint64_t* seed_dev, uint64_t salt) {
  const uint64_t seed = mix64(*seed_dev * 0x9E3779B97F4A7C15ull + salt);
  for (long i = blockIdx.x * (long)blockDim.x + threadIdx.x; i < n; i += (long)gridDim.x * blockDim.x)
    k[i] = (uint32_t)(mix64(seed * 0x100000001B3ull + (uint64_t)i) >> 32);
}

constexpr int SGD_CHUNK = 4096;
__device__ __forceinline__ void sgd_elem(float g, float& w, float& m, float rs, float gscale, float lwd, float momentum, float llr) {
  const float gg = g * gscale * rs + lwd * w;
  m = momentum * m + gg;
  w = w - llr * m;
}
__global__ __launch_bounds__(256) void sgd_kernel(float* __restrict__ param, float* __restrict__ grad, float* __restrict__ mom,
                                                  const l2s_sgd_seg* __restrict__ segs, int nseg, const float* __restrict__ rowscale,
                                                  float lr, float momentum, float wd, float gscale, void* shadow, int sdt, int flags,
                                                  long lo, long hi, int chunk_lo, int chunk_hi, const bf16_t* __restrict__ g16, long g16_lo) {
  const bool clear = flags & 1, shadow_only = flags & 2;
  const int c0 = segs[0].chunk0;
  int total = segs[nseg - 1].chunk0 - c0 + (int)((segs[nseg - 1].count + SGD_CHUNK - 1) / SGD_CHUNK);
  if (chunk_hi >= 0 && chunk_hi < total) total = chunk_hi;
  for (int c = (chunk_lo > 0 ? chunk_lo : 0) + blockIdx.x; c < total; c += gridDim.x) {
    int slo = 0, shi = nseg - 1;
    while (slo < shi) {
      const int mid = (slo + shi + 1) >> 1;
      if (segs[mid].chunk0 - c0 <= c) slo = mid; else shi = mid - 1;
    }
    const l2s_sgd_seg sg = segs[slo];
    const long base = (long)(c - (sg.chunk0 - c0)) * SGD_CHUNK;
    const int n = (int)((sg.count - base) < SGD_CHUNK ? (sg.count - base) : SGD_CHUNK);
    const float lwd = sg.weight_decay ? wd : 0.f;
    const float llr = lr * sg.lr_mult;
    const bool clr = clear && !(sg.flags & 1);
    const long o0 = sg.offset + base;
    const bool inside = o0 >= lo && o0 + n <= hi;
    const bool vec = inside && ((sg.offset & 3) == 0) && (sg.rowscale_off < 0 || (sg.row_len & 3) == 0);
    const int nv = vec ? (n >> 2) : 0;
    float4 g4[4], w4[4], m4[4];
#pragma unroll
    for (int j = 0; j < 4; ++j) {
      const int v = threadIdx.x + j * 256;
      if (v < nv) {
        w4[j] = *(const float4*)(param + o0 + 4 * v);
        if (!shadow_only) {
          if (g16) {
            const uint2 pk = *(const uint2*)(g16 + (o0 + 4 * v - g16_lo));
            g4[j] = make_float4(bf2f((bf16_t)(pk.x & 0xffffu)), bf2f((bf16_t)(pk.x >> 16)), bf2f((bf16_t)(pk.y & 0xffffu)), bf2f((bf16_t)(pk.y >> 16)));
          } else g4[j] = *(const float4*)(grad + o0 + 4 * v);
          m4[j] = *(const float4*)(mom + o0 + 4 * v);
        }
      }
    }
#pragma unroll
    for (int j = 0; j < 4; ++j) {
      const int v = threadIdx.x + j * 256;
      if (v >= nv) continue;
      const long o = o0 + 4 * v;
      const float rs = sg.rowscale_off >= 0 ? rowscale[sg.rowscale_off + (unsigned)(base + 4 * v) / (unsigned)sg.row_len] : 1.f;
      float ww[4] = {w4[j].x, w4[j].y, w4[j].z, w4[j].w};
      if (!shadow_only) {
        float gg[4] = {g4[j].x, g4[j].y, g4[j].z, g4[j].w}, mm[4] = {m4[j].x, m4[j].y, m4[j].z, m4[j].w};
#pragma unroll
        for (int e = 0; e < 4; ++e) sgd_elem(gg[e], ww[e], mm[e], rs, gscale, lwd, momentum, llr);
        *(float4*)(mom + o) = make_float4(mm[0], mm[1], mm[2], mm[3]);
        *(float4*)(param + o) = make_float4(ww[0], ww[1], ww[2], ww[3]);
        if (clr && !g16) *(float4*)(grad + o) = make_float4(0.f, 0.f, 0.f, 0.f);
      }
      if (shadow) {
        if (sdt) {
          uint2 pk; pk.x = (uint32_t)f2bf(ww[0] * rs) | ((uint32_t)f2bf(ww[1] * rs) << 16); pk.y = (uint32_t)f2bf(ww[2] * rs) | ((uint32_t)f2bf(ww[3] * rs) << 16);
          *(uint2*)((bf16_t*)shadow + o) = pk;
        } else *(float4*)((float*)shadow + o) = make_float4(ww[0] * rs, ww[1] * rs, ww[2] * rs, ww[3] * rs);
      }
    }
    for (int i = (nv << 2) + threadIdx.x; i < n; i += 256) {
      const long o = o0 + i;
      if (o < lo || o >= hi) continue;
      const float rs = sg.rowscale_off >= 0 ? rowscale[sg.rowscale_off + (unsigned)(base + i) / (unsigned)sg.row_len] : 1.f;
      float w = param[o];
      if (!shadow_only) {
        float m = mom[o];
        sgd_elem(g16 ? bf2f(g16[o - g16_lo]) : grad[o], w, m, rs, gscale, lwd, momentum, llr);
        mom[o] = m; param[o] = w;
        if (clr && !g16) grad[o] = 0.f;
      }
      if (shadow) stx(shadow, o, sdt, w * rs);
    }
  }
}

}

extern "C" int l2s_version(void) { return 100; }

extern "C" int l2s_weight_cast(const float* src, const float* scale, void* dst, int Cout, int taps, int Cin, int dtype, hipStream_t s) {
  long per_row = (long)taps * Cin, total = per_row * Cout;
  L2S_LAUNCH(weight_cast_kernel, dim3(grid_for(total)), dim3(256), 0, s, src, scale, dst, per_row, total, dtype);
  return l2s_check_launch();
}
extern "C" int l2s_weight_transpose(const float* src, const float* scale, void* dst, int Cout, int taps, int Cin, int dtype, hipStream_t s) {
  dim3 grid(cdiv(Cin, 32), cdiv(Cout, 32), taps);
  L2S_LAUNCH(weight_transpose_kernel, grid, dim3(256), 0, s, src, scale, dst, Cout, taps, Cin, dtype);
  return l2s_check_launch();
}
extern "C" int l2s_weight_transpose_batched(const l2s_transpose_desc* table_dev, int n, int total_tiles, int dtype, hipStream_t s) {
  if (n <= 0 || total_tiles <= 0) return L2S_OK;
  L2S_LAUNCH(weight_transpose_batched_kernel, dim3(total_tiles < 2048 ? total_tiles : 2048), dim3(256), 0, s, table_dev, n, total_tiles, dtype);
  return l2s_check_launch();
}
extern "C" int l2s_colsum(const void* a, int rows, int cols, int lda, float* out, float* ws, long ws_floats, int dtype, hipStream_t s) {
  int nr = (rows + 511) / 512;
  if (nr > 32) nr = 32;
  if (!ws || ws_floats < (long)nr * cols) nr = 1;
  const int rows_per = (rows + nr - 1) / nr;
  float* part = nr > 1 ? ws : nullptr;
  L2S_LAUNCH(colsum_kernel, dim3(cdiv(cols, 64), nr), dim3(1024), 0, s, a, rows, cols, lda, out, part, rows_per, dtype);
  if (nr > 1) L2S_LAUNCH(colsum_finish_kernel, dim3(cdiv(cols, 256)), dim3(256), 0, s, (const float*)ws, nr, cols, out);
  return l2s_check_launch();
}
extern "C" int l2s_stem_conv(const float* img, const float* w, const float* scale, const float* bias, void* y, int H, int W,
                             int OH, int OW, int dtype, hipStream_t s) {
  L2S_LAUNCH(stem_kernel, dim3(cdiv((long)OH * OW, 64)), dim3(256), 0, s, img, w, scale, bias, y, H, W, OH, OW, dtype);
  return l2s_check_launch();
}
extern "C" int l2s_conv3x3_c3(const float* img, const float* w, const float* bias, void* y, int H, int W, int dtype, hipStream_t s) {
  L2S_LAUNCH(conv3x3_c3_kernel, dim3(cdiv((long)H * W, 64)), dim3(256), 0, s, img, w, bias, y, H, W, dtype);
  return l2s_check_launch();
}
extern "C" int l2s_maxpool2x2_fwd(const void* x, void* y, int n_img, int IH, int IW, int C, int dtype, hipStream_t s) {
  const int OH = IH / 2, OW = IW / 2;
  L2S_LAUNCH(maxpool2x2_fwd_kernel, dim3(grid_for((long)n_img * OH * OW * C)), dim3(256), 0, s, x, y, n_img, IH, IW, C, OH, OW, dtype);
  return l2s_check_launch();
}
extern "C" int l2s_maxpool2x2_bwd(const void* dy, const void* x, void* dx, int n_img, int IH, int IW, int C, int relu_out, int dtype, hipStream_t s) {
  const int OH = IH / 2, OW = IW / 2;
  L2S_LAUNCH(maxpool2x2_bwd_kernel, dim3(grid_for((long)n_img * ((IH + 1) / 2) * ((IW + 1) / 2) * C)), dim3(256), 0, s, dy, x, dx, n_img, IH, IW, C, OH, OW,
             dtype, relu_out);
  return l2s_check_launch();
}
extern "C" int l2s_maxpool3x3s2(const void* x, void* y, int IH, int IW, int C, int OH, int OW, int dtype, hipStream_t s) {
  L2S_LAUNCH(maxpool_kernel, dim3(grid_for((long)OH * OW * C)), dim3(256), 0, s, x, y, IH, IW, C, OH, OW, dtype);
  return l2s_check_launch();
}
extern "C" int l2s_fill_f32(float* p, float v, long n, hipStream_t s) {
  if (n <= 0) return L2S_OK;
  L2S_LAUNCH(fill_kernel, dim3(grid_for(n)), dim3(256), 0, s, p, v, n);
  return l2s_check_launch();
}
extern "C" int l2s_cast(const void* src, int sd, void* dst, int dd, long n, hipStream_t s) {
  L2S_LAUNCH(cast_kernel, dim3(grid_for(n)), dim3(256), 0, s, src, sd, dst, dd, n);
  return l2s_check_launch();
}
extern "C" int l2s_mul_f32(const float* a, const float* b, float* out, long n, hipStream_t s) {
  L2S_LAUNCH(mul_kernel, dim3(grid_for(n)), dim3(256), 0, s, a, b, out, n);
  return l2s_check_launch();
}
extern "C" int l2s_add_f32(const float* a, const float* b, float* out, long n, hipStream_t s) {
  L2S_LAUNCH(add_f32_kernel, dim3(grid_for((n + 3) / 4)), dim3(256), 0, s, a, b, out, n);
  return l2s_check_launch();
}
extern "C" int l2s_scale_mask(const void* x, const float* mask, const void* relu_ref, void* out, long n, int dtype, hipStream_t s) {
  L2S_LAUNCH(scale_mask_kernel, dim3(grid_for(n)), dim3(256), 0, s, x, mask, relu_ref, out, n, dtype);
  return l2s_check_launch();
}
extern "C" int l2s_add3(const void* a, const void* b, const float* c, void* dst, long n, int dtype, hipStream_t s) {
  if (dtype == L2S_BF16 && !(n & 7) && !((uintptr_t)a & 15) && !((uintptr_t)b & 15) && !((uintptr_t)c & 15) && !((uintptr_t)dst & 15)) {
    L2S_LAUNCH(add3_bf16x8_kernel, dim3(grid_for(n / 8)), dim3(256), 0, s, (const bf16_t*)a, (const bf16_t*)b, c, (bf16_t*)dst, n / 8);
    return l2s_check_launch();
  }
// ... 126 lines not shown
```

### lang2seg_amd/csrc/wgrad_common.h

```cpp
#pragma once
#include "common.h"
#include "../../include/lang2seg_hip.h"
#include <stddef.h>

typedef l2s_wgrad_prob wgp;

namespace l2s {
struct wgrad_sk_plan { int n; long U; long unit0[L2S_WGRAD_MAX_GROUP + 1]; int S[L2S_WGRAD_MAX_GROUP]; int mode, T, Ng, k1, Q, r, m; };
bool wgrad_row3_dma_ok(const l2s_wgrad_prob& q);
long wgrad_row3_dma_tiles(int Cin, int Cout);
size_t wgrad_row3_dma_ws_bytes(int G);
int wgrad_row3_dma_launch(const l2s_wgrad_prob* tab_dev, const l2s_wgrad_prob* tab_host, int nprob, float* ws, size_t ws_bytes, int G, hipStream_t st);
bool wgrad_1x1_dma_ok(const l2s_wgrad_prob& q);
long wgrad_1x1_dma_tiles(int Cin, int Cout);
int wgrad_1x1_dma_launch(const l2s_wgrad_prob* tab_dev, const l2s_wgrad_prob* tab_host, int nprob, hipStream_t st);

struct wgrad_tile_prefix { int n; int tile0[L2S_WGRAD_MAX_GROUP + 1]; };
}

namespace l2s_wgrad {

template <class F> long fill_tile_prefix(l2s::wgrad_tile_prefix& pre, const wgp* tab_host, int nprob, F tiles) {
  pre.n = nprob;
  long t = 0;
  for (int i = 0; i < nprob; ++i) { pre.tile0[i] = (int)t; t += tiles(tab_host[i]); }
  for (int i = nprob; i <= L2S_WGRAD_MAX_GROUP; ++i) pre.tile0[i] = (int)t;
  return t;
}

#define WGRAD_LAUNCH(kern, grid, block, lds, st, ...)                                                                                     \
  do {                                                                                                                                    \
    static bool attr_done = false;                                                                                                        \
    if (!attr_done) { (void)hipFuncSetAttribute((const void*)kern, hipFuncAttributeMaxDynamicSharedMemorySize, (int)(lds)); attr_done = true; } \
    L2S_LAUNCH(kern, grid, block, lds, st, __VA_ARGS__);                                                                                  \
  } while (0)

typedef int i32x4s __attribute__((ext_vector_type(4)));
constexpr unsigned OOR = 0x80000000u;

__device__ __forceinline__ i32x4s rsrc(const void* base, long bytes = 0x7FFFFFFF) {
  i32x4s r; r.x = (int)(uintptr_t)base; r.y = (int)((uintptr_t)base >> 32); r.z = (int)bytes; r.w = 0x00020000; return r;
}

__device__ __forceinline__ void dma_1kib(const i32x4s& r, unsigned voff, unsigned lds_) {
  const unsigned lds = (unsigned)__builtin_amdgcn_readfirstlane((int)lds_);
  asm volatile("s_mov_b32 m0, %2\n\ts_nop 0\n\tbuffer_load_dwordx4 %0, %1, 0 offen lds" ::"v"(voff), "s"(r), "s"(lds) : "memory");
}

template <int PER, int KMAX = 3> __device__ __forceinline__ void wait_vm_keep(int younger) {
  if (KMAX >= 3 && younger >= 3) asm volatile("s_waitcnt vmcnt(%0)" ::"n"(3 * PER) : "memory");
  else if (KMAX >= 2 && younger >= 2) asm volatile("s_waitcnt vmcnt(%0)" ::"n"(2 * PER) : "memory");
  else if (KMAX >= 1 && younger == 1) asm volatile("s_waitcnt vmcnt(%0)" ::"n"(PER) : "memory");
  else asm volatile("s_waitcnt vmcnt(0)" ::: "memory");
}
__device__ __forceinline__ void wg_barrier() { asm volatile("s_barrier" ::: "memory"); }
__device__ __forceinline__ void lds_wait() { asm volatile("s_waitcnt lgkmcnt(0)" ::: "memory"); }

__device__ __forceinline__ uint4 lds_frag(const char* q, int rowbytes) {
  const s16x4 lo = __builtin_amdgcn_ds_read_tr16_b64_v4i16((__attribute__((address_space(3))) s16x4*)(q));
  const s16x4 hi = __builtin_amdgcn_ds_read_tr16_b64_v4i16((__attribute__((address_space(3))) s16x4*)(q + 16 * rowbytes));
  return __builtin_bit_cast(uint4, (s16x8){lo[0], lo[1], lo[2], lo[3], hi[0], hi[1], hi[2], hi[3]});
}

__device__ __forceinline__ int tile_of(const l2s::wgrad_tile_prefix& pre, int L, int& t) {
  const int G = pre.tile0[pre.n], x = L & 7, slot = L >> 3, q = G >> 3, r = G & 7;
  const int bid = x * q + min(x, r) + slot;
  int lo = 0, hi = pre.n;
  while (hi - lo > 1) { const int mid = (lo + hi) >> 1; if (pre.tile0[mid] <= bid) lo = mid; else hi = mid; }
  t = bid - pre.tile0[lo];
  return lo;
}

__device__ __forceinline__ void pixel_split(int pix, int ohwv, int Wv, int& n, int& y, int& x) {
  n = pix / ohwv; const int rem = pix - n * ohwv; y = rem / Wv; x = rem - y * Wv;
}
__device__ __forceinline__ void pixel_place(int pix, int ohwv, int Wv, int& n, int& y, int& x) {
  if (pix < 0) { n = 0; y = 0; x = -1; }
  else pixel_split(pix, ohwv, Wv, n, y, x);
}
__device__ __forceinline__ void slice_step(int bkp, int ohwv, int Wv, int& a, int& b, int& c) {
  a = bkp / ohwv; b = (bkp - a * ohwv) / Wv; c = bkp - a * ohwv - b * Wv;
}

__device__ __forceinline__ float4 add4(float4 a, const float4& b) { a.x += b.x; a.y += b.y; a.z += b.z; a.w += b.w; return a; }
__device__ __forceinline__ float4 f4(const f32x4& a) { return make_float4(a[0], a[1], a[2], a[3]); }
__device__ __forceinline__ void dw_store(float4* q, float4 v, bool accumulate) {
  if (accumulate) v = add4(v, *q);
  *q = v;
}

}
```

### lang2seg_amd/nets/network.py

```python
import numpy as np
import os
import torch

from .. import ops as O
from .._lib import F32, BF16, LOSS_CAP
from ..model.config import cfg
from .params import ParamStore
from . import anchors as ANC


class ConvOp(object):

    def __init__(self, net, wkey, Cin, Cout, k=1, stride=1, pad=0, bias_key=None, need_dgrad=True, group=None, Cout_pad=None, full_map=False):
        self.net, self.wkey, self.Cin, self.Cout, self.k, self.stride, self.pad = net, wkey, Cin, Cout, k, stride, pad
        self.full_map = bool(full_map and k > 1 and pad == 0 and stride == 1)
        self.t_taps, self.t_cin = (1, k * k * Cin) if self.full_map else (k * k, Cin)
        self.bias_key, self.need_dgrad, self.group = bias_key, need_dgrad, group
        self.Np = Cout if Cout_pad is None else Cout_pad
        self.prio = 1 if str(wkey).startswith(('resnet.layer1.', 'resnet.layer2.', 'resnet.layer3.')) and getattr(net, 'chain_prio', True) else 0
        P = net.P
        taps = k * k
        cnt = self.Np * taps * Cin
        if group is not None:
            self.trainable = True
# ... 6 lines not shown
        else:
            self.trainable = wkey in P.offsets
            self.scale = P.bn_scale.get(wkey)
            if self.trainable:
                self.w_master = P.view(wkey); self.w_grad = P.view(wkey, P.grad); self.wf = P.view(wkey, P.shadow)
            else:
                self.w_master = P.frozen[wkey].view(-1)
                self.w_grad = None
                self.wf = O.empty((cnt,), net.dt)
            if bias_key is not None and bias_key in P.offsets:
                self.bias = P.view(bias_key); self.bias_grad = P.view(bias_key, P.grad)
            elif bias_key is not None:
                self.bias = P.frozen[bias_key]; self.bias_grad = None
            else:
                self.bias = P.bn_bias.get(wkey); self.bias_grad = None
        self.wb = O.empty((cnt,), net.dt) if (need_dgrad and self.trainable) else None
        net.convs.append(self)

    def refresh(self, full=False):
        taps = self.k * self.k
        if not self.trainable and full:
            O.weight_cast(self.w_master, self.scale, self.wf, self.Np, taps, self.Cin)
        if self.wb is not None:
            O.weight_transpose(self.w_master, self.scale, self.wb, self.Np, self.t_taps, self.t_cin)

    def out_hw(self, IH, IW):
        return (IH + 2 * self.pad - self.k) // self.stride + 1, (IW + 2 * self.pad - self.k) // self.stride + 1

    def fwd(self, x, n, IH, IW, y, add=None, relu=False, out_f32=False, tile=0):
        OH, OW = self.out_hw(IH, IW)
        O.conv_igemm(x, self.wf, y, n, IH, IW, self.Cin, OH, OW, self.Np, self.k, self.k, self.stride, self.pad,
                     bias=self.bias, add=add, relu=relu, out_f32=out_f32, tile=tile, dt=self.net.dt, ws=self.net.splitk_ws(n * OH * OW * self.Np), prio=max(self.prio, self.net.prio_floor),
                     algo=(self.net.conv_algo if self.k == 1 and self.stride == 1 and self.Np >= 1024 else None))
        return y

    def dgrad(self, g, n, IH, IW, dx, add=None, ref=None):
        OH, OW = self.out_hw(IH, IW)
        if self.full_map:
            assert IH == self.k and IW == self.k and OH == 1 and OW == 1
            O.conv_igemm(g, self.wb, dx, n, 1, 1, self.Np, 1, 1, self.t_cin, 1, 1, 1, 0, add=add, ref=ref, dt=self.net.dt,
                         prio=max(self.prio, self.net.prio_floor))
            return dx
        if self.stride == 1:
            O.conv_igemm(g, self.wb, dx, n, OH, OW, self.Np, IH, IW, self.Cin, self.k, self.k, 1, self.k - 1 - self.pad,
                         add=add, ref=ref, dt=self.net.dt, ws=self.net.splitk_ws(n * IH * IW * self.Cin), prio=max(self.prio, self.net.prio_floor),
                         algo=(self.net.conv_algo if self.k == 1 and self.Cin >= 1024 else None))
        else:
            assert self.k == 1
            O.conv_igemm(g, self.wb, dx, n, OH, OW, self.Np, OH, OW, self.Cin, 1, 1, 1, 0, add=add, ref=ref,
                         scatter=(IH, IW, self.stride), dt=self.net.dt, prio=max(self.prio, self.net.prio_floor))
        return dx

    def wgrad(self, g, x, n, IH, IW):
        ko = self.net.knockout
        if 'wgrad' in ko or ('wgrad4' in ko and str(self.wkey).startswith('resnet.layer4.')) or \
                ('wgrad3' in ko and str(self.wkey).startswith(('resnet.layer3.', 'resnet.layer2.'))):
            return
        OH, OW = self.out_hw(IH, IW)
        self.net.wgq.add(self.w_grad, g, x, n, IH, IW, self.Cin, OH, OW, self.Np, self.k, self.stride, self.pad)
        if self.bias_grad is not None:
            with self.net.fork_wgrad():
                O.colsum(g, n * OH * OW, self.Np, self.Np, self.bias_grad, ws=self.net.buf('colsum.ws.' + str(self.bias_key or self.group[1]), (32 * self.Np,), torch.float32))


class WgradQueue(object):

    def __init__(self, net):
        self.net, self.items, self.tables = net, [], {}
        self.deferred = []
        self.on_launch = None

    def defer(self):
        self.deferred.extend(self.items)
        self.items = []

    def flush_deferred(self, tag):
        assert not self.items, 'weight gradients queued behind the deferred ones'
        self.items, self.deferred = self.deferred, []
        self.flush(tag)

    def add(self, dw, g, x, n, IH, IW, Cin, OH, OW, Cout, k, stride, pad, lddy=None, ldx=None):
        self.items.append((dw, g, x, n, IH, IW, Cin, OH, OW, Cout, k, stride, pad, Cout if lddy is None else lddy, Cin if ldx is None else ldx))

    def flush(self, tag):
        from .._lib import WgradProb, ptr, load
        import ctypes as C
        if not self.items:
            return False
        lib = load()
        net = self.net
        items, self.items = self.items, []
        by_dw = {}
        for it in items:
            by_dw.setdefault((it[0].data_ptr(), it[6], it[9], it[10], it[11], it[12]), []).append(it)
        rounds = {}
        for key, uses in by_dw.items():
            for r in range(0, len(uses), 2):
                seg = uses[r:r + 2]
                dw, g, x, n, IH, IW, Cin, OH, OW, Cout, k, stride, pad, lddy, ldx = seg[0]
                M = max(u[3] * u[7] * u[8] for u in seg)
                same = all(u[7] == u[4] and u[8] == u[5] for u in seg)
                tl = 256 if net.dt == BF16 else 0
                if self.SMALL_M_TILE and net.dt == BF16 and M < 8192 and Cin >= 256 and Cout >= 256 and Cin % 128 == 0 and Cout % 128 == 0:
                    tl = self.SMALL_M_TILE
                v = int(lib.l2s_wgrad_variant(Cin, Cout, k, k, stride, pad, int(same), M, tl))
                rounds.setdefault((r // 2, v), []).append(seg)
        bkp = 32 if net.dt == BF16 else 16
        fresh = getattr(net, '_fresh', None) if getattr(net, 'wgrad_overwrite', False) else None
        order = sorted(rounds)
        plan = [('wg', order)]
        if tag == 'layer2' and net.use_streams and getattr(net, 'layer2_side', False):
            plan = [('wg2', order)]
            net._layer2_on_side = True
        if self.V5_STREAM != 'wg' and net.use_streams and getattr(net, 'dp', None) is None and (0, 5) in rounds and (0, 4) in rounds:
            plan = [(self.V5_STREAM, [(0, 5)]), ('wg', [o for o in order if o != (0, 5)])]
        for sname, keys in plan:
          with net.fork_wgrad(fixed=sname):
            ws = net.wgrad_ws() if sname == 'wg' else net.wgrad_ws(alt=True)
            for (rnd, v) in keys:
                probs = rounds[(rnd, v)]
                for c0 in range(0, len(probs), 64):
                    chunk = probs[c0:c0 + 64]
                    tiles = [int(lib.l2s_wgrad_tiles(v, seg[0][6], seg[0][9], seg[0][10], seg[0][10])) for seg in chunk]
                    total = sum(tiles)
                    want = max(1, -(-self.MIN_WG // max(total, 1)))
                    if v == 4:
                        want = max(1, self.V4_FILL // max(total, 1))
                    arr = (WgradProb * len(chunk))()
                    flop, off = 0.0, 0
                    for i, seg in enumerate(chunk):
                        dw, g, x, n, IH, IW, Cin, OH, OW, Cout, k, stride, pad, lddy, ldx = seg[0]
                        q = arr[i]
                        q.dw, q.nseg, q.Cin, q.Cout, q.KH, q.KW, q.stride, q.pad = dw.data_ptr(), len(seg), Cin, Cout, k, k, stride, pad
                        q.flags = 0
                        if fresh is not None and rnd == 0 and dw.data_ptr() not in fresh and dw.numel() == Cout * k * k * Cin:
                            q.flags = 1
                            fresh.add(dw.data_ptr())
                        slices = min(u[3] * u[7] * (u[8] + (1 if v in (2, 3, 5) else 0)) // bkp for u in seg)
                        split = max(1, min(want, slices // 16, 16))
                        if v in (5, 6):
                            split = 1
                        slab = Cout * k * k * Cin
                        if split > 1 and (off + split * slab) * 4 <= ws.numel() * 4:
                            q.split, q.ws_off = split, off
                            off += split * slab
                        else:
                            q.split, q.ws_off = 1, 0
                        for s_, u in enumerate(seg):
                            q.dy[s_], q.x[s_] = u[1].data_ptr(), u[2].data_ptr()
                            q.n_img[s_], q.IH[s_], q.IW[s_], q.OH[s_], q.OW[s_], q.lddy[s_], q.ldx[s_] = u[3], u[4], u[5], u[7], u[8], u[13], u[14]
                            flop += 2.0 * u[3] * u[7] * u[8] * Cout * k * k * Cin
                    raw = bytes(arr)
                    ck = (tag, rnd, v, c0, getattr(net, '_rec_key', None))
                    ent = self.tables.get(ck)
                    if ent is None or ent[0] != raw:
                        host = torch.frombuffer(bytearray(raw), dtype=torch.uint8)
                        if net.device != 'cpu' and torch.cuda.is_available():
                            host = host.pin_memory()
                        ent = (raw, host.to(net.device, non_blocking=True), host)
                        self.tables[ck] = ent
                    dt = O.dt_of(chunk[0][0][2])
                    ctx = self.on_launch(tag, v, flop, chunk[0][0][10]) if self.on_launch is not None else None
                    if ctx is not None:
                        ctx.__enter__()
                    O.call('l2s_conv_wgrad_grouped', ent[1].data_ptr(), C.cast(arr, C.c_void_p), len(chunk), v, dt, ws.data_ptr(),
                           ws.numel() * 4, O.stream())
                    if ctx is not None:
                        ctx.__exit__(None, None, None)
        return True

    V5_STREAM = 'wg'
    SMALL_M_TILE = 0
    MIN_WG = 256
    V4_FILL = 128


class Bottleneck(object):

    def __init__(self, net, prefix, inplanes, planes, stride, has_down, need_dx=True):
        self.net, self.prefix, self.stride, self.need_dx = net, prefix, stride, need_dx
        self.inpl, self.planes = inplanes, planes
        self.c1 = ConvOp(net, prefix + '.conv1.weight', inplanes, planes, 1, stride, 0, need_dgrad=need_dx)
        self.c2 = ConvOp(net, prefix + '.conv2.weight', planes, planes, 3, 1, 1)
        self.c3 = ConvOp(net, prefix + '.conv3.weight', planes, planes * 4, 1, 1, 0)
        self.down = ConvOp(net, prefix + '.downsample.0.weight', inplanes, planes * 4, 1, stride, 0, need_dgrad=need_dx) if has_down else None

    def fwd(self, x, n, IH, IW, tag):
        net = self.net
        OH, OW = self.c1.out_hw(IH, IW)
        a1 = net.buf(tag + '.a1', (n * OH * OW, self.planes))
        a2 = net.buf(tag + '.a2', (n * OH * OW, self.planes))
        y = net.buf(tag + '.y', (n * OH * OW, self.planes * 4))
        self.c1.fwd(x, n, IH, IW, a1, relu=True)
        self.c2.fwd(a1, n, OH, OW, a2, relu=True)
        if self.down is not None:
            sc = net.buf(tag + '.sc', (n * OH * OW, self.planes * 4))
            self.down.fwd(x, n, IH, IW, sc)
            self.c3.fwd(a2, n, OH, OW, y, add=sc, relu=True)
        else:
            self.c3.fwd(a2, n, OH, OW, y, add=x, relu=True)
        return y, OH, OW, (x, a1, a2, IH, IW, OH, OW, n)

    def fwd_rest(self, x, a1, sc, n, IH, IW, tag):
        net = self.net
        a2 = net.buf(tag + '.a2', (n * IH * IW, self.planes))
        y = net.buf(tag + '.y', (n * IH * IW, self.planes * 4))
        self.c2.fwd(a1, n, IH, IW, a2, relu=True)
        self.c3.fwd(a2, n, IH, IW, y, add=sc, relu=True)
        return y, IH, IW, (x, a1, a2, IH, IW, IH, IW, n)

    def bwd(self, g, saved, tag, x_is_relu_out=True):
        net = self.net
        x, a1, a2, IH, IW, OH, OW, n = saved
        self.c3.wgrad(g, a2, n, OH, OW)
        dz2 = net.buf(tag + '.dz2', (n * OH * OW, self.planes))
        self.c3.dgrad(g, n, OH, OW, dz2, ref=a2)
        self.c2.wgrad(dz2, a1, n, OH, OW)
        dz1 = net.buf(tag + '.dz1', (n * OH * OW, self.planes))
        self.c2.dgrad(dz2, n, OH, OW, dz1, ref=a1)
        self.c1.wgrad(dz1, x, n, IH, IW)
        if self.down is not None:
            self.down.wgrad(g, x, n, IH, IW)
        if not self.need_dx:
            return None
        dx = net.buf(tag + '.dx', (n * IH * IW, self.inpl))
        ref = x if x_is_relu_out else None
        if self.down is not None:
            if self.stride != 1 and tag not in net._precleared:
                O.memset_zero(dx)
            self.c1.dgrad(dz1, n, IH, IW, dx)
            self.down.dgrad(g, n, IH, IW, dx, add=dx, ref=ref)
        else:
            self.c1.dgrad(dz1, n, IH, IW, dx, add=g, ref=ref)
        return dx


class Network(object):
    def __init__(self, batch_size=1):
        self._feat_stride = [16, ]
        self._batch_size = batch_size
        self._predictions = {}
        self._losses = {}
        self._anchor_targets = {}
        self._proposal_targets = {}
        self._mode = 'TRAIN'
        self.training = True
        self.device = 'cuda'
        self._bufs = {}
        self._buf_users = {}
# ... 234 lines not shown
    def splitk_ws(self, need):
        if not getattr(self, 'conv_split_k', False) or need > self.SPLITK_WS_FLOATS // 2 or self.device == 'cpu':
            return None
        pool = self.__dict__.setdefault('_skws', {})
        key = torch.cuda.current_stream().cuda_stream
        ws = pool.get(key)
        if ws is None:
            ws = pool[key] = torch.empty(self.SPLITK_WS_FLOATS, dtype=torch.float32, device=self.device)
        return ws

    def _init_modules(self):
        raise NotImplementedError

    def train(self, mode=True):
        self.training = mode
        return self

    def eval(self):
        return self.train(False)

    def cuda(self):
        return self

    def state_dict(self):
        self.join_update()
        dp = getattr(self, 'dp', None)
        if dp is not None and getattr(dp, 'master_stale', False):
            raise RuntimeError('state_dict() of a sharded data-parallel run: call net.dp.gather_master() on every rank first')
        return self.P.state_dict()

    def load_state_dict(self, sd, strict=False):
        self.join_update()
        self.P.load_state_dict(sd, strict)
        self.refresh_weights(full=True)

    def named_parameters(self):
        from .params import from_internal
        self.join_update()
        dp = getattr(self, 'dp', None)
        if dp is not None and getattr(dp, 'master_stale', False):
            raise RuntimeError('named_parameters() of a sharded data-parallel run: call net.dp.gather_master() on every rank first')
        for k in self.P.trainable:
            yield k, from_internal(k, self.P.view(k), self.P.shapes[k])

    def refresh_weights(self, full=False):
        if full:
            for c in self.convs:
                if not c.trainable:
                    O.weight_cast(c.w_master, c.scale, c.wf, c.Np, c.k * c.k, c.Cin)
        if getattr(self, '_tr_table', None) is None:
            from .._lib import TransposeDesc
            items = [c for c in self.convs if c.wb is not None] + list(getattr(self, 'extra_transposes', []))
            arr = (TransposeDesc * len(items))()
            for i, c in enumerate(items):
                arr[i].src, arr[i].scale, arr[i].dst = c.w_master.data_ptr(), (c.scale.data_ptr() if c.scale is not None else None), c.wb.data_ptr()
                arr[i].Cout, arr[i].taps, arr[i].Cin, arr[i].force_f32 = c.Np, getattr(c, 't_taps', c.k * c.k), getattr(c, 't_cin', c.Cin), int(getattr(c, 'force_f32', 0))
                if self.dt == BF16 and isinstance(c, ConvOp) and c.trainable and not arr[i].force_f32:
                    arr[i].src, arr[i].scale, arr[i].force_f32 = c.wf.data_ptr(), None, 2
            self._tr_table = torch.frombuffer(bytearray(bytes(arr)), dtype=torch.uint8).to(self.device)
            self._tr_n = len(items)
            self._tr_tiles = sum(((c.Cin + 63) // 64) * ((c.Np + 63) // 64) * c.k * c.k for c in items)
        if self.use_streams and not full:
            S = self.streams()
            self.sfork(torch.cuda.current_stream(), S['tr'])
            with torch.cuda.stream(S['tr']):
                O.weight_transpose_batched(self._tr_table, self._tr_n, self._tr_tiles, self.dt)
            self._tr_pending = True
        else:
            O.weight_transpose_batched(self._tr_table, self._tr_n, self._tr_tiles, self.dt)

    update_on_wg = False
    defer_heads = False
    conv_algo = None
    roi_pdma = False
    layer1_fused = True
    cap_persistent = True
    _precleared = frozenset()
    prio_floor = 0
    cap_map_prio = 0
    rpn_wgrad_early = False
    rpn_bwd_early = True
    join_before_layer1 = False
    stem_mfma = True
    wgrad_overwrite = True
    update_clears_grad = False
    SLOT_UPDATE_REST = 0
    SLOT_UPDATE_L2 = 1
    SLOT_WGRADS = 2
    update_split = False
    layer2_side = False

    def join_update(self, full=True, layer2_only=False):
        if self.use_streams and self.update_on_wg:
            if layer2_only and self.update_split and not self.defer_heads and not getattr(self, '_pass_without_step', False):
                O.event_wait(self.SLOT_UPDATE_L2, torch.cuda.current_stream())
                if not self.layer2_side:
                    O.event_wait(self.SLOT_WGRADS, torch.cuda.current_stream())
            elif self.defer_heads and not full:
                O.event_wait(self.SLOT_UPDATE_REST, torch.cuda.current_stream())
            else:
                self.sfork(self.streams()['wg'], torch.cuda.current_stream())
                if self.layer2_side:
                    self.sfork(self.streams()['wg2'], torch.cuda.current_stream())

    def join_backlog(self):
        if self.use_streams and self.update_on_wg and self.layer2_side and self.update_split and not self.defer_heads \
                and not getattr(self, '_pass_without_step', False):
            O.event_wait(self.SLOT_WGRADS, torch.cuda.current_stream())

    def join_deferred(self):
        if self.use_streams and self.update_on_wg and self.defer_heads:
            self.sfork(self.streams()['wg'], torch.cuda.current_stream())

    def join_transposes(self):
        if self.use_streams:
            self.sfork(self.streams()['tr'], torch.cuda.current_stream())
            self._tr_pending = False

    def upload_blob(self, blobs, idx):
        cache = blobs.setdefault('_device', {}) if isinstance(blobs, dict) else {}
        dev = self.device
        if 'data' not in cache:
            cache['data'] = torch.from_numpy(np.ascontiguousarray(blobs['data'], dtype=np.float32)).to(dev)
        key = ('sent', idx)
        if key not in cache:
            labels = blobs['labels']
            labels = labels.cpu().numpy() if isinstance(labels, torch.Tensor) else np.asarray(labels)
            lab = labels[idx:idx + 1]
            max_len = int((lab != 0).sum(1).max())
            lab = np.ascontiguousarray(lab[:, :max_len]).astype(np.int64)
            if blobs.get('cap_labels') is not None:
                cap = np.ascontiguousarray(blobs['cap_labels'][idx:idx + 1]).astype(np.int64)
                S = 1
                while S < cap.shape[1] - 1 and cap[0, S] != 0:
                    S += 1
                cm = np.ascontiguousarray(blobs['cap_masks'][idx:idx + 1]).astype(np.float32)
            else:
                cap = np.zeros((1, 2), np.int64); cm = np.zeros((1, 2), np.float32); S = 1
            if '_gt_masks_ref' in cache:
                r = cache['_sent_ref_host'][idx]
                gm = cache['_gt_masks_ref'][r:r + 1]
            else:
                gm = torch.from_numpy(np.ascontiguousarray(blobs['gt_masks'][idx:idx + 1], dtype=np.uint8)).to(dev)
            cache[key] = dict(
                gt_boxes=torch.from_numpy(np.ascontiguousarray(blobs['gt_boxes'][idx:idx + 1], dtype=np.float32)).to(dev),
                gt_masks=gm,
                labels=torch.from_numpy(lab[0]).to(dev), T=max_len, S=S,
                cap_in=torch.from_numpy(cap[0, :S].copy()).to(dev), cap_tgt=torch.from_numpy(cap[0, 1:S + 1].copy()).to(dev),
                cap_mask=torch.from_numpy(cm[0, 1:S + 1].copy()).to(dev))
        d = dict(cache[key])
        d['data'] = cache['data']
        d['im_info'] = np.asarray(blobs['im_info'], dtype=np.float32).reshape(-1)[:3]
        return d

    def train_step(self, blobs, idx, train_op):
        loss = self.train_step_async(blobs, idx, train_op)
        vals = loss.cpu().numpy()
        if not np.isfinite(vals[np.asarray(self._loss_slots())]).all():
            self.check_cap_recur()
        return tuple(float(vals[i]) for i in self._loss_slots())

    def check_cap_recur(self):
        from .._lib import L2SError
        st = getattr(self, '_cap_state', None)
        if st is None:
            return
        torch.cuda.synchronize()
        err = [int(s[1].item()) for s in st]
        if any(err):
            for s in st:
                s.zero_()
            raise L2SError('captioner recurrence: a workgroup of the resident %s launch gave up waiting for its peers (not co-resident); the '
                           'exchange state was reset - set Network.cap_persistent = False to run the per-token launches' %
                           ' / '.join(n for n, e in zip(('forward', 'backward'), err) if e))

    def _loss_slots(self):
        from .variants import loss_names, SLOT
        return [SLOT[k] for k in loss_names(getattr(self, 'variant', 'cycle'))]

    def _loss_names(self):
        from .variants import loss_names
        return loss_names(getattr(self, 'variant', 'cycle'))

    def train_step_async(self, blobs, idx, train_op):
        dev = self.upload_blob(blobs, idx)
        self._early_op = train_op if (self.dp is None and self.use_streams and self.parity is None
                                      and getattr(train_op, 'early', False) and str(self.device).startswith('cuda')) else None
        if getattr(self, 'use_tape', False) and self.use_streams and self.parity is None:
            loss = self.tape_step(dev, train_op)
        elif getattr(self, 'use_graph', False) and self.dp is None and self.parity is None:
            loss = self.graph_step(dev, train_op)
        else:
            loss = self.forward_backward(dev)
            if self.dp is not None:
                self.dp.finish()
            train_op.step()
        self._early_op = None
        self._step += 1
        return loss

    def train_step_with_summary(self, blobs, idx, train_op):
        r = self.train_step(blobs, idx, train_op)
        return r + ([(n, v) for n, v in zip(self._loss_names(), r)],)

    def get_summary(self, blobs, idx):
        was = self.training
        self.eval()
        dev = self.upload_blob(blobs, idx)
        loss = self.forward_backward(dev, backward=False).cpu().numpy()
        self.train(was)
        return [(n, float(loss[i])) for n, i in zip(self._loss_names(), self._loss_slots())]
```

### lang2seg_amd/nets/params.py

```python
import ctypes as C
import numpy as np
import torch

from .. import ops as O
from .._lib import SgdSeg

RESNET_LAYERS = {50: [3, 4, 6, 3], 101: [3, 4, 23, 3], 152: [3, 8, 36, 3]}
BN_EPS = 1e-5


def to_internal(name, t):
    if name == 'vgg.classifier.0.weight':
        return t.view(t.shape[0], 512, 7, 7).permute(0, 2, 3, 1).contiguous().view(t.shape[0], -1)
    if t.dim() == 4 and name == 'mask_up_sampling.weight':
        return t.permute(0, 2, 3, 1).contiguous()
    if t.dim() == 4:
        return t.permute(0, 2, 3, 1).contiguous()
    return t.contiguous()


def from_internal(name, t, ref_shape):
    if name == 'vgg.classifier.0.weight':
        return t.view(ref_shape[0], 7, 7, 512).permute(0, 3, 1, 2).contiguous().view(ref_shape)
    if len(ref_shape) == 4 and name == 'mask_up_sampling.weight':
        ci, co, kh, kw = ref_shape
        return t.view(ci, kh, kw, co).permute(0, 3, 1, 2).contiguous()
    if len(ref_shape) == 4:
        o, i, kh, kw = ref_shape
        return t.view(o, kh, kw, i).permute(0, 3, 1, 2).contiguous()
    return t.view(ref_shape).contiguous()


RNN_GATES = {'lstm': 4, 'gru': 3, 'rnn': 1}


def encoder_config(opt):
    typ = str(opt.get('rnn_type', 'lstm')).lower()
    if typ not in RNN_GATES:
        raise ValueError("rnn_type %r: the encoder has 'lstm', 'gru' and 'rnn' (tanh) cells" % (opt.get('rnn_type'),))
    layers = int(opt.get('rnn_num_layers', 1))
    if layers < 1:
        raise ValueError('rnn_num_layers %r: at least one layer' % (opt.get('rnn_num_layers'),))
    if int(opt['rnn_hidden_size']) % 4 or int(opt['rnn_hidden_size']) < 4:
        raise ValueError('rnn_hidden_size %r: the recurrent kernels need a multiple of 4' % (opt['rnn_hidden_size'],))
    if int(opt.get('variable_lengths', 1)) <= 0:
        raise ValueError('variable_lengths %r: the reference encoder returns no hidden state with variable_lengths 0' % (opt.get('variable_lengths'),))
    return typ, layers, (2 if int(opt.get('bidirectional', 1)) > 0 else 1), RNN_GATES[typ]


def encoder_rnn_shapes(opt):
    typ, layers, ndir, G = encoder_config(opt)
    WV, Hh = opt['word_vec_size'], opt['rnn_hidden_size']
    s = {}
    for k in range(layers):
        for sfx in ['', '_reverse'][:ndir]:
            s['rnn_encoder.rnn.weight_ih_l%d%s' % (k, sfx)] = (G * Hh, WV if k == 0 else ndir * Hh)
            s['rnn_encoder.rnn.weight_hh_l%d%s' % (k, sfx)] = (G * Hh, Hh)
            s['rnn_encoder.rnn.bias_ih_l%d%s' % (k, sfx)] = (G * Hh,)
            s['rnn_encoder.rnn.bias_hh_l%d%s' % (k, sfx)] = (G * Hh,)
    return s


CAPTIONERS = ('att2in2', 'topdown', 'adaatt', 'adaattmo')
CAPTIONER_MARK = {'att2in2': 'core.i2h.weight', 'topdown': 'core.att_lstm.weight_ih', 'adaatt': 'core.lstm.w2h.weight',
                  'adaattmo': 'core.lstm.w2h.weight'}
ADAATT_GATES = {'adaatt': 4, 'adaattmo': 5}
FC_CAPTIONERS = ('topdown', 'adaatt', 'adaattmo')


def caption_config(opt):
    m = str(opt.get('caption_model', 'att2in2'))
    if m not in CAPTIONERS or (m in ADAATT_GATES and not int(opt.get('adaatt') or 0)):
        raise ValueError("--caption_model %r: the caption branch has 'att2in2' and 'topdown', and with --adaatt 1 'adaatt' and 'adaattmo'"
                         % (opt.get('caption_model'),))
    if m != 'att2in2' and (int(opt['rnn_size']) % 4 or int(opt['rnn_size']) < 4):
        raise ValueError('rnn_size %r: the recurrent kernels of --caption_model %s need a multiple of 4' % (opt['rnn_size'], m))
    if m in ADAATT_GATES:
        if not (int(opt['input_encoding_size']) == int(opt['rnn_size']) == int(opt['att_hid_size'])):
            raise ValueError('--caption_model %s needs input_encoding_size == rnn_size == att_hid_size (%r, %r, %r): the reference concatenates '
                             'the sentinel with the attention features' % (m, opt['input_encoding_size'], opt['rnn_size'], opt['att_hid_size']))
        if int(opt.get('num_layers', 1)) != 1:
            raise ValueError('--num_layers %r with --caption_model %s: the stacked AdaAtt cell (i2h, r_i2h, inter-layer dropout) is not built'
                             % (opt.get('num_layers'), m))
    return m


def caption_shapes(opt):
    m = caption_config(opt)
# ... 307 lines not shown
            bad.append('rnn_type / rnn_num_layers / bidirectional / word_vec_size: %s is %s there and %s here' % (diff[0], theirs.get(diff[0]), mine.get(diff[0])))
        raise ValueError('the state dict holds another language encoder; it was trained with ' + ', '.join(bad))

    def check_caption_keys(self, sd):
        if self.var['cap'] is not None:
            check_caption_keys(self.opt, sd)

    def load_state_dict(self, sd, strict=False):
        self.check_encoder_keys(sd)
        self.check_caption_keys(sd)
        for k, shp in self.shapes.items():
            if k not in sd:
                if strict:
                    raise KeyError(k)
                continue
            t = sd[k]
            t = torch.from_numpy(np.ascontiguousarray(t)) if isinstance(t, np.ndarray) else t.detach().cpu()
            t = t.float()
            assert tuple(t.shape) == tuple(shp), (k, tuple(t.shape), shp)
            ti = to_internal(k, t).reshape(-1).to(self.device)
            if k in self.offsets:
                self.view(k).copy_(ti)
            else:
                self.frozen[k].copy_(ti.view(self.frozen[k].shape))
        self._fold_bn()
        self.refresh_shadow_full()

    def state_dict(self):
        out = {}
        for k, shp in self.shapes.items():
            if k in self.offsets:
                out[k] = from_internal(k, self.view(k).detach().clone(), shp).cpu()
            else:
                out[k] = from_internal(k, self.frozen[k].detach().clone().reshape(-1), shp).cpu()
        return out

    def _fold_bn(self):
        for k in self.shapes:
            bn = self.bn_of(k)
            if bn is None:
                continue
            g, b = self.frozen[bn + '.weight'], self.frozen[bn + '.bias']
            m, v = self.frozen[bn + '.running_mean'], self.frozen[bn + '.running_var']
            s = g / torch.sqrt(v + BN_EPS)
            self.bn_scale[k].copy_(s)
            self.bn_bias[k].copy_(b - m * s)
            if k in self.rowscale_off:
                o = self.rowscale_off[k]
                self.rowscale[o:o + s.numel()].copy_(s)

    def param_group(self, k, double_bias=False, bias_decay=False, lang_lr_mult=None, from_frcn=False, gamma=0.1):
        from .variants import SOLVERS, LANG_LR_KEYS
        mult = SOLVERS[self.variant]['lang_lr_mult'] if lang_lr_mult is None else float(lang_lr_mult)
        is_bias = 'bias' in k
        if from_frcn:
            f = 1.0 if 'mask' in k else float(gamma)
        else:
            f = mult if any(t in k for t in LANG_LR_KEYS) else 1.0
        if is_bias and double_bias:
            f *= 2.0
        return f, (1 if (not is_bias or bias_decay) else 0)

    def build_segments(self, double_bias=False, bias_decay=False, lang_lr_mult=None, from_frcn=False, gamma=0.1):
        segs = []
        for k in self.trainable:
            cnt = int(np.prod(self.shapes[k]))
            sg = SgdSeg()
            sg.offset, sg.count = self.offsets[k], cnt
            sg.row_len = cnt // self.shapes[k][0] if k in self.rowscale_off else 1
            sg.lr_mult, sg.weight_decay = self.param_group(k, double_bias, bias_decay, lang_lr_mult, from_frcn, gamma)
            sg.rowscale_off = self.rowscale_off.get(k, -1)
            segs.append(sg)
        self.seg_rule = (bool(double_bias), bool(bias_decay), lang_lr_mult, bool(from_frcn), float(gamma))
        CH = int(O.sgd_chunk())

        def table(seq):
            run = 0
            for g in seq:
                g.chunk0 = run
                run += -(-int(g.count) // CH)
            arr = (SgdSeg * len(seq))(*seq)
            self._seg_tables.append(arr)
            return torch.frombuffer(bytearray(bytes(arr)), dtype=torch.uint8).to(self.device)
        self._seg_tables, self._ow_key = [], frozenset()
        self.nseg = len(segs)
        self.seg_ends = [int(g.offset + g.count) for g in segs]
        self.seg_offs = [int(g.offset) for g in segs]
        self.seg_chunks = [-(-int(g.count) // CH) for g in segs]
        self.seg_chunk0 = [sum(self.seg_chunks[:i]) for i in range(len(segs))]
        self.sgd_chunk = CH
        self.seg_size = C.sizeof(SgdSeg)
        self.segs_dev = table(segs)
        lo, hi = self.defer_range
        cp = lambda g: SgdSeg.from_buffer_copy(bytes(g))
        rest = [cp(g) for g in segs if not (lo <= g.offset < hi)]
        late = [cp(g) for g in segs if lo <= g.offset < hi]
        self.n_rest = len(rest)
        self.segs_split_dev = table(rest + late)
        return self.nseg

    def mark_overwritten(self, ptrs):
        key = frozenset(ptrs)
        if key == self._ow_key:
            return
        base = self.grad.data_ptr()
        torch.cuda.synchronize() if self.grad.is_cuda else None
        for arr, dev in zip(self._seg_tables, (self.segs_dev, self.segs_split_dev)):
            for g in arr:
                was, now = g.flags & 1, int(base + 4 * int(g.offset) in key)
                if was and not now:
                    self.grad[int(g.offset):int(g.offset + g.count)].zero_()
                g.flags = now
            dev.copy_(torch.frombuffer(bytearray(bytes(arr)), dtype=torch.uint8))
        torch.cuda.synchronize() if self.grad.is_cuda else None
        self._ow_key = key

    def stale_marked(self, s0, s1, fresh):
        if not self._ow_key:
            return []
        base = self.grad.data_ptr()
        return [base + 4 * o for o in self.seg_offs[s0:s1] if (base + 4 * o) in self._ow_key and (base + 4 * o) not in fresh]

    def chunk_range(self, lo, hi):
        import bisect
        s0 = bisect.bisect_right(self.seg_ends, lo)
        s1 = bisect.bisect_left(self.seg_offs, hi)
        if s0 >= s1:
            return 0, 0
        c_lo = self.seg_chunk0[s0] + max(0, lo - self.seg_offs[s0]) // self.sgd_chunk
        last = s1 - 1
        c_hi = self.seg_chunk0[last] + min(self.seg_chunks[last], -(-(min(hi, self.seg_ends[last]) - self.seg_offs[last]) // self.sgd_chunk))
        return c_lo, c_hi

    def refresh_shadow_full(self):
        if not hasattr(self, 'segs_dev'):
            self.build_segments()
        zero = torch.zeros_like(self.grad)
        O.sgd_momentum(self.param, zero, self.mom, self.segs_dev, self.nseg, self.rowscale, 0.0, 1.0, 0.0, 0.0, shadow=self.shadow)
```

### lang2seg_amd/nets/resnet_v1.py

```python
import os
import numpy as np
import torch

from .. import ops as O
from .._lib import F32, BF16
from ..model.config import cfg
from .network import Network, ConvOp, Bottleneck
from .params import ParamStore, encoder_config, caption_config
from .captioners import CAPTIONERS
from .variants import solver_cfg
from . import anchors as ANC
from . import decode
from . import caption_rows

f32 = torch.float32


class resnetv1(Network):
    variant = 'cycle'

    def __init__(self, opt, batch_size=1, num_layers=50, variant=None):
        Network.__init__(self, batch_size=batch_size)
        from .variants import VARIANTS
        if variant is not None:
# ... 448 lines not shown
        dfc7 = self.buf('roi.dfc7', (R, 2048))
        self.rcnn_heads.dgrad(d_cheads, R, 1, 1, dfc7)
        dup = self.buf('mask.dup', (FGM * MS * MS, 256))
        mws = self.buf('mask.pred_ws', (FGM * 14 * 257,), f32)
        O.maskpred_bwd_dx(dscore, labels, counts, FGM, MS * MS, 256, P.view('mask_pred_net.weight'), up, up, dup, mws)
        with self.fork_wgrad():
            O.maskpred_bwd_reduce(mws, labels, counts, FGM, 256, P.view('mask_pred_net.weight', P.grad), P.view('mask_pred_net.bias', P.grad))
            O.colsum(dup, FGM * MS * MS, 256, 256, P.view('mask_up_sampling.bias', P.grad), ws=self.buf('mask.up_bias_ws', (32 * 256,), f32))
        self.wgq.add(P.view('mask_up_sampling.weight', P.grad), fc7s, dup, FGM, MS, MS, 256, PS, PS, 2048, 2, 2, 0)
        dmask_fc7 = self.buf('mask.dfc7s', (FGM * PS * PS, 2048))
        O.conv_igemm(dup, P.view('mask_up_sampling.weight', P.shadow), dmask_fc7, FGM, MS, MS, 256, PS, PS, 2048, 2, 2, 2, 0, dt=dt)
        g = self.buf('l4r.g', (R * PS * PS, 2048))
        O.avgpool_bwd(dfc7, g, dmask_fc7, fc7s, FGM, PS * PS, 2048)
        if R > FGM:
            off = FGM * PS * PS
            O.avgpool_bwd(dfc7[FGM:], g[off:], None, fc7s[off:], R - FGM, PS * PS, 2048)
        for b in reversed(range(len(self.layers[4]))):
            g = self.layers[4][b].bwd(g, saved[('4r', b)], 'l4r.%d' % b, x_is_relu_out=(b > 0))
        self._mark('roi head bwd')
        return self._rois_pool_bwd(g, Hc, Wc, rois, R, saved)

    def _filter_fwd(self, d):
        P = self.P
        C4 = self._C4_feat_dim
        hidden = self._encoder_fwd(d)
        HD = hidden.numel()
        NF, NFP = 7 * C4 + 7, self._NFP
        filt = self.buf('dyn.filt', (NF,), f32, zero=(NFP != NF))
        O.linear_fwd(hidden, P.gview('dyn_w', NFP * HD), P.gview('dyn_b', NFP), filt, 1, NFP, HD, act=2)
        if NFP != NF:
            if not hasattr(self, '_r_one'):
                self._r_one = torch.tensor([1.0, 0, 0, 0, 0, 0, 0], dtype=f32, device=self.device)
            O.memcpy(filt[7 * C4:], self._r_one)
        return filt

    def _dynfilter_fwd(self, base, filt, Hc, Wc):
        C4 = self._C4_feat_dim
        net_conv = self.buf('dyn.y', (Hc * Wc, C4)); resp = self.buf('dyn.resp', (Hc * Wc,), f32); respk = self.buf('dyn.respk', (Hc * Wc, 7), f32)
        O.dynfilter_fwd(base, filt, filt[7 * C4:], net_conv, resp, respk, Hc, Wc, C4, gate=1 if self.var['gate'] == 'sigmoid' else 0)
        return net_conv, resp, respk

    def _rpn_fwd(self, net_conv, Hc, Wc):
        A, HW, NPR = self._num_anchors, Hc * Wc, self.P.rpn_npad
        rpn = self.buf('rpn.a', (HW, 512))
        self.rpn_conv.fwd(net_conv, 1, Hc, Wc, rpn, relu=True)
        rheads = self.buf('rpn.heads', (HW, NPR), f32)
        self.rpn_heads.fwd(rpn, 1, Hc, Wc, rheads, out_f32=True)
        nA = HW * A
        prob = self.buf('rpn.prob', (HW, 2 * A), f32); boxes = self.buf('rpn.boxes', (nA, 4), f32); scores = self.buf('rpn.scores', (nA,), f32)
        O.rpn_decode(rheads, NPR, self.base_anchors, Hc, Wc, A, 16, self._im_hw[0], self._im_hw[1], prob, boxes, scores)
        return rpn, rheads, prob, boxes, scores

    def _nms_proposals(self, scores, boxes, nA, key, pfx):
        c = cfg[key]
        pre, post = int(c.RPN_PRE_NMS_TOP_N), int(c.RPN_POST_NMS_TOP_N)
        pre = nA if pre <= 0 else min(pre, nA)
        sb = self.buf(pfx + '.sb', (pre, 4), f32); ss = self.buf(pfx + '.ss', (pre,), f32); si = self.buf(pfx + '.si', (pre,), torch.int32)
        O.sort_topk(scores, boxes, nA, pre, self.buf('prop.sortws', (O.sort_ws_ints(nA),), torch.int32), sb, ss, si)
        nms_ws = self.buf(pfx + '.nmsws', (O.nms_workspace_bytes(pre) // 8 + 8,), torch.int64)
        keep = self.buf(pfx + '.keep', (post,), torch.int32); nkeep = self.buf(pfx + '.nkeep', (1,), torch.int32)
        O.nms(sb, pre, float(c.RPN_NMS_THRESH), 0 if cfg.NMS_CMP == 'ge' else 1, post, nms_ws, keep, nkeep)
        rois = self.buf(pfx + '.rois', (post, 5), f32); rsc = self.buf(pfx + '.rsc', (post,), f32)
        O.gather_rois(sb, ss, keep, nkeep, post, rois, rsc)
        return rois, rsc, nkeep

    keep_logprobs = False

    def forward_backward(self, d, backward=True):
        P, dt = self.P, self.dt
        self.t = t = {}
        TR = cfg.TRAIN
        A, nc = self._num_anchors, self._num_classes
        R = int(TR.BATCH_SIZE); FGS = int(round(TR.FG_FRACTION * R))
        FGM = R if getattr(TR, 'MASK_SLOTS_ALL', False) else FGS
        PS, MS = int(cfg.POOLING_SIZE), int(cfg.MASK_SIZE)
        C4 = self._C4_feat_dim
        H, W = int(d['data'].shape[1]), int(d['data'].shape[2])
        im_h, im_w = float(d['im_info'][0]), float(d['im_info'][1])
        self._im_hw = (im_h, im_w)
        self._mark('step start')
        main = torch.cuda.current_stream()
        S = self.streams() if self.use_streams else None
        if backward:
            self._fresh = set()
        if self.update_clears_grad:
            if backward:
                if getattr(self, '_bwd_pending', 0):
                    raise RuntimeError('two backward passes without an optimiser update in between: the gradients would add up '
                                       '(the update clears them; construct SGD(keep_grad=True) to have every step clear them itself)')
                self._bwd_pending = 1
        elif S is not None and self.update_on_wg:
            self.sfork(main, S['wg'])
            with torch.cuda.stream(S['wg']):
                O.memset_zero(P.grad)
        else:
            O.memset_zero(P.grad)
        import contextlib
        def on(name):
            return torch.cuda.stream(S[name]) if S is not None else contextlib.nullcontext()
        if S is not None:
            self.sfork(main, S['lang'])
        key = 'TRAIN' if self._mode == 'TRAIN' else 'TEST'
        post = int(cfg[key].RPN_POST_NMS_TOP_N)
        n_gt = int(d['gt_boxes'].shape[0])
        with on('lang'):
            O.counter_inc(self.seed_counter())
            loss = self.buf('loss', (8,), f32, zero=True)
            dfilt_ = self.buf('dyn.dfilt', (7 * C4 + 7,), f32, zero=True) if backward else None
            roi_keys = (self._keys('roi_fg_keys', post + n_gt), self._keys('roi_bg_keys', post + n_gt), self._keys('roi_bg_rand', R))
        if S is not None and self.update_on_wg:
            with torch.cuda.stream(S['lang']):
                self.join_update(full=False)
        with on('lang'):
            filt = self._filter_fwd(d)
            self._cap_pre = self._caption_pre(d) if (self.var['cap'] is not None and 'cap' not in self.knockout) else None
        self._mark('encoder_fwd(lang)')
        saved = {}
        base, Hc, Wc = self._backbone_fwd(d, saved)
        self._mark('layer1-3 fwd')
        HW = Hc * Wc
        t['net_conv_base'] = base
        self.join_deferred()
        self.join_transposes()
        if S is not None:
            self.sfork(S['lang'], main)
        self._precleared = set()
        if backward and S is not None:
            with on('lang'):
                for li in (3, 2):
                    if (li, 0) not in saved:
                        continue
                    blk = self.layers[li][0]
                    if li > cfg.RESNET.FIXED_BLOCKS and blk.down is not None and blk.stride != 1 and blk.need_dx:
                        x_, a1_, a2_, IH_, IW_, OH_, OW_, n_ = saved[(li, 0)]
                        O.memset_zero(self.buf('l%d.0.dx' % li, (n_ * IH_ * IW_, blk.inpl)))
                        self._precleared.add('l%d.0' % li)
        net_conv, resp, respk = self._dynfilter_fwd(base, filt, Hc, Wc)
        t['net_conv'], t['response'] = net_conv, resp
        gate = 1 if self.var['gate'] == 'sigmoid' else 0
        dresp_extra = None
        if gate:
            dresp_extra = self.buf('dyn.dresp_loss', (HW,), f32)
            O.response_loss(resp, d['gt_masks'], H, W, Hc, Wc, 1.0, loss, dresp_extra)
        AF = self.opt['att_feat_size']

        def l4_on_map_bwd(g, tag, in_relu=False):
            self.prio_floor = self.cap_map_prio
            for b in reversed(range(len(self.layers[4]))):
                g = self.layers[4][b].bwd(g, saved[(tag, b)], '%s.%d' % (tag, b), x_is_relu_out=(b > 0 or in_relu))
            self.prio_floor = 0
            return g

        def caption_branch():
            if 'cap' in self.knockout:
                return self.buf('l4m.skip', (HW, C4)), None
            self._mark('dyn fwd')
            feats = self._l4_on_map(net_conv, Hc, Wc, 'l4m', saved)
            self._mark('cap: layer4 on map fwd')
            if self.var['cap'] == 'mask':
                gm = self.buf('cap.gm', (HW,), f32)
                O.mask_downsample(d['gt_masks'], gm, H, W, Hc, Wc)
                att, fc = self._caption_pools([(feats, None), (feats, gm)], Hc, Wc)
                t.update({'feats_all': feats, 'att_feats': att, 'gt_mask_small': gm})
            else:
                feats_b = self._l4_on_map(base, Hc, Wc, 'l4b', saved)
                att, fc = self._caption_pools([(feats_b, None), (feats, None)], Hc, Wc)
# ... 352 lines not shown
```

### lang2seg_amd/ops.py

```python
import ctypes as C
import torch
from . import _lib
from ._lib import ptr, call, F32, BF16, ConvDesc, WgradDesc

TORCH_DT = {F32: torch.float32, BF16: torch.bfloat16}


def stream():
    return torch.cuda.current_stream().cuda_stream


def dt_of(t):
    return BF16 if t.dtype == torch.bfloat16 else F32


def empty(shape, dt, device='cuda'):
    return torch.empty(shape, dtype=TORCH_DT[dt], device=device)


def stream_fork(from_stream, to_stream):
    call('l2s_stream_fork', from_stream.cuda_stream, to_stream.cuda_stream)


def event_record(slot, s):
# ... 948 lines not shown

def cap_gates_fwd(sums, a2c, c_prev, c, h, save, R):
    call('l2s_cap_gates_fwd', ptr(sums), ptr(a2c), ptr(c_prev), ptr(c), ptr(h), ptr(save), R, stream())


def cap_gates_bwd(dh, dc_in, save, c_prev, dsums, da2c, dc_prev, R, dh2=None):
    call('l2s_cap_gates_bwd', ptr(dh), ptr(dh2), ptr(dc_in), ptr(save), ptr(c_prev), ptr(dsums), ptr(da2c), ptr(dc_prev), R, stream())


def linear2_fwd(x, K, w1, b1, y1, N1, acc1, w2, b2, y2, N2, acc2):
    call('l2s_linear2_fwd', ptr(x), K, ptr(w1), ptr(b1), ptr(y1), N1, int(acc1), ptr(w2), ptr(b2), ptr(y2), N2, int(acc2), stream())


def linear_sum2_fwd(x1, w1, K1, x2, w2, K2, y, N, accumulate=False):
    call('l2s_linear_sum2_fwd', ptr(x1), ptr(w1), K1, ptr(x2), ptr(w2), K2, ptr(y), N, int(accumulate), stream())


def cap_a2c_gates_fwd(att_res, w_a2c, b_a2c, K, sums, c_prev, c, h, save, R):
    call('l2s_cap_a2c_gates_fwd', ptr(att_res), ptr(w_a2c), ptr(b_a2c), K, ptr(sums), ptr(c_prev), ptr(c), ptr(h), ptr(save), R, stream())


def cap_att_dots_fwd(patt, att_h, aw, ab, L, D, tanh_ws, dots):
    call('l2s_cap_att_dots_fwd', ptr(patt), ptr(att_h), ptr(aw), ptr(ab), L, D, ptr(tanh_ws), ptr(dots), stream())


def cap_apply_gates_fwd(P, dots, b_a2c, sums, c_prev, c, h, save, weight, L, R):
    call('l2s_cap_apply_gates_fwd', ptr(P), ptr(dots), ptr(b_a2c), ptr(sums), ptr(c_prev), ptr(c), ptr(h), ptr(save), ptr(weight), L, R, stream())


def bottleneck64_fwd(a, x, w2, b2, w3, b3, y, H, W, wd=None, bd=None, w1n=None, b1n=None, a_next=None):
    d = _lib.Bottleneck64Desc(ptr(a), ptr(x), ptr(w2), ptr(w3), ptr(wd), ptr(w1n), ptr(b2), ptr(b3), ptr(bd), ptr(b1n), ptr(y), ptr(a_next), H, W, x.shape[-1])
    call('l2s_bottleneck64_fwd', C.byref(d), stream())


def cap_recur_supported(S, R, AH, L):
    return bool(_lib.load().l2s_cap_recur_supported(int(S), int(R), int(AH), int(L)))


def cap_recur_state(backward, device='cuda'):
    n = int(_lib.load().l2s_cap_recur_state_bytes(int(backward)))
    return torch.zeros((n + 3) // 4, dtype=torch.int32, device=device)


def cap_recur_fwd(w_h2h, b_h2h, w_h2att, b_h2att, patt, aw, ab, P, b_a2c, sums, hs, cs, save, tanh_ws, wgt, state, S, R, AH, L):
    a = _lib.CapRecurFwdArgs(ptr(w_h2h), ptr(b_h2h), ptr(w_h2att), ptr(b_h2att), ptr(patt), ptr(aw), ptr(ab), ptr(P), ptr(b_a2c), ptr(sums), ptr(hs), ptr(cs),
                             ptr(save), ptr(tanh_ws), ptr(wgt), ptr(state), S, R, AH, L)
    call('l2s_cap_recur_fwd', C.byref(a), stream())


def cap_recur_bwd(w_h2h, w_h2att, P, aw, save, cs, wgt, tanh_ws, dho, dsums, da2c, ddot, datt_h, state, S, R, AH, L):
    a = _lib.CapRecurBwdArgs(ptr(w_h2h), ptr(w_h2att), ptr(P), ptr(aw), ptr(save), ptr(cs), ptr(wgt), ptr(tanh_ws), ptr(dho), ptr(dsums), ptr(da2c), ptr(ddot),
                             ptr(datt_h), ptr(state), S, R, AH, L, ddot.stride(0), datt_h.stride(0))
    call('l2s_cap_recur_bwd', C.byref(a), stream())


def cap_gates_bwd_dw(dh, dc_in, save, c_prev, P, dsums, da2c, dc_prev, dweight, L, R, dh2=None):
    call('l2s_cap_gates_bwd_dw', ptr(dh), ptr(dh2), ptr(dc_in), ptr(save), ptr(c_prev), ptr(P), ptr(dsums), ptr(da2c), ptr(dc_prev), ptr(dweight),
         L, R, stream())


def cap_attention_bwd_step2(dweight, tanh_ws, weight, aw, L, D, ddot, datt_h):
    call('l2s_cap_attention_bwd_step2', ptr(dweight), ptr(tanh_ws), ptr(weight), ptr(aw), L, D, ptr(ddot), ptr(datt_h), stream())


def cap_attention_bwd_step(datt_res, att, tanh_ws, weight, aw, L, D, ddot, datt_h):
    call('l2s_cap_attention_bwd_step', ptr(datt_res), ptr(att), ptr(tanh_ws), ptr(weight), ptr(aw), L, D, ptr(ddot), ptr(datt_h), stream())


def cap_attention_bwd_batched(ddot, weight, datt_res, ldr, tanh_ws, aw, S, L, D, dpatt, datt, daw, dab):
    call('l2s_cap_attention_bwd_batched', ptr(ddot), ptr(weight), ptr(datt_res), ldr, ptr(tanh_ws), ptr(aw), S, L, D, ptr(dpatt), ptr(datt),
         ptr(daw), ptr(dab), stream())


def logsoftmax_nll(logits, target, mask, S, V1, gscale, loss_slot, dlogits, logprobs=None):
    call('l2s_logsoftmax_nll', ptr(logits), ptr(target), ptr(mask), S, V1, float(gscale), ptr(loss_slot), ptr(dlogits),
         ptr(logprobs), stream())


def sgd_momentum(param, grad, mom, segs_dev, nseg, rowscale, lr, momentum, wd, gscale=1.0, shadow=None, clear_grad=False):
    call('l2s_sgd_momentum', ptr(param), ptr(grad), ptr(mom), ptr(segs_dev), nseg, ptr(rowscale), float(lr), float(momentum),
         float(wd), float(gscale), ptr(shadow), dt_of(shadow) if shadow is not None else 0, 1 if clear_grad else 0, stream())


def sgd_momentum_range(param, grad, mom, segs_dev, nseg, rowscale, lr, momentum, wd, gscale, shadow, flags, lo, hi, chunk_lo, chunk_hi):
    call('l2s_sgd_momentum_range', ptr(param), ptr(grad), ptr(mom), ptr(segs_dev), nseg, ptr(rowscale), float(lr), float(momentum),
         float(wd), float(gscale), ptr(shadow), dt_of(shadow) if shadow is not None else 0, int(flags), int(lo), int(hi), int(chunk_lo), int(chunk_hi), stream())


def sgd_momentum_range_g16(param, grad_bf16, grad_lo, mom, segs_dev, nseg, rowscale, lr, momentum, wd, gscale, shadow, lo, hi, chunk_lo, chunk_hi):
    call('l2s_sgd_momentum_range_g16', ptr(param), ptr(grad_bf16), int(grad_lo), ptr(mom), ptr(segs_dev), nseg, ptr(rowscale), float(lr), float(momentum),
         float(wd), float(gscale), ptr(shadow), dt_of(shadow) if shadow is not None else 0, int(lo), int(hi), int(chunk_lo), int(chunk_hi), stream())


def sgd_chunk():
    return int(_lib.load().l2s_sgd_chunk())


def add_f32(a, b, out):
    call('l2s_add_f32', ptr(a), ptr(b), ptr(out), a.numel(), stream())


def mul(a, b, out):
    call('l2s_mul_f32', ptr(a), ptr(b), ptr(out), a.numel(), stream())
```

### lang2seg_amd/optim.py

```python
import bisect

import torch

from . import ops as O


class SGD(object):
    def __init__(self, net, lr, momentum=0.9, weight_decay=1e-4, grad_scale=1.0, keep_grad=False):
        self.net = net
        self.lr, self.momentum, self.weight_decay, self.grad_scale = float(lr), float(momentum), float(weight_decay), float(grad_scale)
        self.param_groups = [self.__dict__]
        self.side_active = bool(self.side and getattr(net, 'use_streams', False) and hasattr(net, 'flush_wgrads'))
        if self.side_active:
            net.update_on_wg = True
        self._early = bool(type(self)._early and not self.defer)
        self.defer_active = bool(self.defer and self.side_active and not self._early and hasattr(net, 'wgq') and getattr(net, 'dp', None) is None)
        net.defer_heads = self.defer_active
        net.update_split = bool(self.side_active and getattr(net, 'dp', None) is None and not self.defer_active)
        net.layer2_side = bool(net.update_split and self.layer2_side and getattr(net.P, 'fixed_blocks', 1) == 1 and not getattr(net.P, 'is_vgg', False))
        dp = getattr(net, 'dp', None)
        if dp is not None and getattr(dp, 'shard_update', None) is True:
            dp.shard_update = self
        if dp is not None and getattr(dp, 'bucket_update', None) is True:
            dp.bucket_update = self
        self.in_reducer = dp is not None and (getattr(dp, 'shard_update', None) is self or getattr(dp, 'bucket_update', None) is self)
        self.clear_grad = not keep_grad and getattr(dp, 'shard_update', None) is None
        net.update_clears_grad = self.clear_grad

    def zero_grad(self):
        pass

    _early = True
    _seg_done = 0

    @property
    def early(self):
        return self._early

    @early.setter
    def early(self, v):
        self._early = bool(v)
        if self._early and getattr(self, 'defer_active', False):
            self.defer_active = False
            self.net.defer_heads = False

    def _launch(self, s0, s1, table=None):
        P = self.net.P
        if s1 > s0:
            O.sgd_momentum(P.param, P.grad, P.mom, (P.segs_dev if table is None else table)[s0 * P.seg_size:], s1 - s0, P.rowscale, self.lr,
                           self.momentum, self.weight_decay, self.grad_scale, shadow=P.shadow, clear_grad=self.clear_grad)

    def partial(self, stage):
        net = self.net
        P = net.P
        if not hasattr(self, '_bounds'):
            from .parallel import bucket_bounds
            self._bounds = bucket_bounds(P)
            assert all(a <= b for a, b in zip(P.seg_ends, P.seg_ends[1:]))
        hi = bisect.bisect_right(P.seg_ends, self._bounds[stage])
        if hi <= self._seg_done:
            return
        stale = P.stale_marked(self._seg_done, hi, getattr(net, '_fresh', ()))
        if stale:
            P.mark_overwritten(P._ow_key - frozenset(stale))
        S = net.streams()
        tr = S['tr']
        net.sfork(torch.cuda.current_stream(), tr)
        for name in ('wg', 'wg2', 'lang', 'cap'):
            net.sfork(S[name], tr)
        with torch.cuda.stream(tr):
            self._launch(self._seg_done, hi)
            net._mark('partial update %s (tr)' % stage)
        self._seg_done = hi

    side = True

    layer2_side = True
    defer = False

    def _mark_overwritten(self):
        net = self.net
        if self.clear_grad and not self.defer_active and getattr(net, 'wgrad_overwrite', False):
            net.P.mark_overwritten(getattr(net, '_fresh', ()))

    def step(self):
        P = self.net.P
        net = self.net
        net._bwd_pending = 0
        net._pass_without_step = False
        if getattr(getattr(net, 'dp', None), 'shard_update', None) is not None:
            gathered = bool(getattr(net.dp, 'gather_shadow', False))
            if self.side_active and net.use_streams:
                net.flush_wgrads('final')
                with torch.cuda.stream(net.streams()['wg']):
                    if not gathered:
                        self.refresh_shadow()
                    net.refresh_weights()
                    net._mark('update done (wg)')
                return
            if hasattr(net, 'join_wgrad'):
                net.join_wgrad()
            if not gathered:
                self.refresh_shadow()
            net.refresh_weights()
            return
        if getattr(getattr(net, 'dp', None), 'bucket_update', None) is self:
            if self.side_active and net.use_streams:
                net.flush_wgrads('final')
                self._mark_overwritten()
                with torch.cuda.stream(net.streams()['wg']):
                    net.refresh_weights()
                    net._mark('update done (wg)')
                return
            if hasattr(net, 'join_wgrad'):
                net.join_wgrad()
            self._mark_overwritten()
            net.refresh_weights()
            return
        if self.side_active and net.use_streams:
            net.flush_wgrads('final')
            self._mark_overwritten()
            S = net.streams()
            early_tail = bool(self._seg_done and net.update_split and not self.defer_active and getattr(net.wgq, 'V5_STREAM', 'wg') != 'tr')
            side2 = bool(early_tail and getattr(net, '_layer2_on_side', False))
            net._layer2_on_side = False
            if not side2:
                net.sfork(S['wg2'], S['wg'])
            if getattr(net.wgq, 'V5_STREAM', 'wg') == 'tr':
                net.sfork(S['tr'], S['wg'])
            O.event_record(net.SLOT_WGRADS, S['wg'])
            if early_tail:
                T = S['wg2'] if side2 else S['wg']
                net.sfork(torch.cuda.current_stream(), T)
                with torch.cuda.stream(T):
                    self._launch(self._seg_done, P.nseg)
                    O.event_record(net.SLOT_UPDATE_L2, T)
                    net._mark('update of layer2 done')
                for k in ('wg2', 'lang', 'cap', 'tr'):
                    net.sfork(S[k], S['wg'])
                net.sfork(torch.cuda.current_stream(), S['wg'])
                with torch.cuda.stream(S['wg']):
                    net.refresh_weights()
                    net._mark('update done (wg)')
                self._seg_done = 0
                return
            for k in ('wg2', 'lang', 'cap'):
                net.sfork(S[k], S['wg'])
            if self._seg_done or getattr(net.wgq, 'V5_STREAM', 'wg') == 'tr':
                net.sfork(S['tr'], S['wg'])
            net.sfork(torch.cuda.current_stream(), S['wg'])
            with torch.cuda.stream(S['wg']):
                if self.defer_active:
                    self._launch(0, P.n_rest, P.segs_split_dev)
                    O.event_record(net.SLOT_UPDATE_REST, S['wg'])
                    net._mark('update of the rest done (wg)')
                    net.wgq.flush_deferred('heads')
                    net._mark('deferred weight gradients done (wg)')
                    self._launch(P.n_rest, P.nseg, P.segs_split_dev)
                else:
                    self._launch(self._seg_done, P.nseg)
                    O.event_record(net.SLOT_UPDATE_L2, S['wg'])
                net.refresh_weights()
                net._mark('update done (wg)')
            self._seg_done = 0
            return
        if hasattr(self.net, 'join_wgrad'):
            self.net.join_wgrad()
        if self._seg_done:
# ... 37 lines not shown
```

Baseline: 224.5 img/s.

## Fold SGD momentum update into grouped conv weight-gradient kernel epilogues

Adds a grouped wgrad entry point that, for segments whose gradient is fully overwritten, applies the SGD momentum update (param, momentum, bf16 shadow) directly in the wgrad store or split-K reduce epilogue. Segments handled this way are flagged SEG_UPDATED so the later optimizer pass skips them. The goal is to drop a separate read-modify-write pass over those weights and gradients. In exchange, segment tables must be kept in sync with host-side synchronizations, and weights are now updated during backward.

```diff
diff --git a/include/lang2seg_hip.h b/include/lang2seg_hip.h
--- a/include/lang2seg_hip.h
+++ b/include/lang2seg_hip.h
@@ -439,6 +439,7 @@
                  int chunk0;
                  int flags;
                  int reserved; } l2s_sgd_seg;
+#define L2S_SEG_UPDATED 2
 int l2s_sgd_momentum_range(float* param, float* grad, float* mom, const l2s_sgd_seg* segs, int nseg, const float* rowscale,
                            float lr, float momentum, float wd, float grad_scale, void* shadow, int shadow_dtype, int flags,
                            long lo, long hi, int chunk_lo, int chunk_hi, hipStream_t s);
@@ -451,6 +452,14 @@
                      int shadow_dtype, int clear_grad ,
                      hipStream_t s);
 
+typedef struct { float* param; float* mom; void* shadow;
+                 const l2s_sgd_seg* seg;
+               } l2s_wgrad_upd;
+typedef struct { const float* rowscale; float lr, momentum, wd, grad_scale; int shadow_dtype; int reserved; } l2s_wgrad_upd_args;
+int l2s_conv_wgrad_grouped_update(const l2s_wgrad_prob* table_dev, const l2s_wgrad_prob* table_host, const l2s_wgrad_upd* upd_dev,
+                                  const l2s_wgrad_upd* upd_host, int nprob, int variant, int dtype, float* ws, size_t ws_bytes,
+                                  const l2s_wgrad_upd_args* args, hipStream_t stream);
+
 #ifdef __cplusplus
 }
 #endif
diff --git a/lang2seg_amd/_lib.py b/lang2seg_amd/_lib.py
--- a/lang2seg_amd/_lib.py
+++ b/lang2seg_amd/_lib.py
@@ -35,6 +35,14 @@
                 ('split', i32), ('ws_off', i64), ('flags', i32), ('reserved', i32)]
 
 
+class WgradUpd(C.Structure):
+    _fields_ = [('param', vp), ('mom', vp), ('shadow', vp), ('seg', vp)]
+
+
+class WgradUpdArgs(C.Structure):
+    _fields_ = [('rowscale', vp), ('lr', f32), ('momentum', f32), ('wd', f32), ('grad_scale', f32), ('shadow_dtype', i32), ('reserved', i32)]
+
+
 class TransposeDesc(C.Structure):
     _fields_ = [('src', vp), ('scale', vp), ('dst', vp), ('Cout', i32), ('taps', i32), ('Cin', i32), ('force_f32', i32)]
 
@@ -122,6 +130,7 @@
 
 
 CONV_RELU, CONV_OUT_F32, CONV_DECONV2X2, CONV_SCATTER = 1, 4, 8, 16
+SEG_OVERWRITTEN, SEG_UPDATED = 1, 2
 LOSS_RPN_CLS, LOSS_RPN_BOX, LOSS_CLS, LOSS_BOX, LOSS_MASK, LOSS_CAP, LOSS_TOTAL, LOSS_RESPONSE = range(8)
 
 SIGS = {
@@ -135,6 +144,7 @@
     'l2s_wgrad_variant': (i32, [i32, i32, i32, i32, i32, i32, i32, i64, i32]),
     'l2s_wgrad_tiles': (i64, [i32, i32, i32, i32, i32]),
     'l2s_conv_wgrad_grouped': (i32, [vp, vp, i32, i32, i32, vp, sz, vp]),
+    'l2s_conv_wgrad_grouped_update': (i32, [vp, vp, vp, vp, i32, i32, i32, vp, sz, C.POINTER(WgradUpdArgs), vp]),
     'l2s_weight_cast': (i32, [vp, vp, vp, i32, i32, i32, i32, vp]),
     'l2s_weight_transpose': (i32, [vp, vp, vp, i32, i32, i32, i32, vp]),
     'l2s_colsum': (i32, [vp, i32, i32, i32, vp, vp, i64, i32, vp]),
diff --git a/lang2seg_amd/csrc/conv_wgrad.hip b/lang2seg_amd/csrc/conv_wgrad.hip
--- a/lang2seg_amd/csrc/conv_wgrad.hip
+++ b/lang2seg_amd/csrc/conv_wgrad.hip
@@ -9,7 +9,8 @@
 template <> struct WGT<float> { static constexpr int BKP = 16; static constexpr int PADB = 64; };
 
 template <typename T, int BM, int BN, int TX, int D, int KSTEP = 1, int WGM = 2, int WGN = 2>
-__device__ __forceinline__ void wgrad_tile(const wgp& p, int co0, int ci0, int tg, int split_idx, int nsplit, float* out, bool accumulate, char* smem) {
+__device__ __forceinline__ void wgrad_tile(const wgp& p, int co0, int ci0, int tg, int split_idx, int nsplit, float* out, bool accumulate, char* smem,
+                                           const upd_prob& u, const l2s_wgrad_upd_args& ua) {
   constexpr int ES = (int)sizeof(T);
   constexpr int VE = 16 / ES;
   constexpr int BKP0 = WGT<T>::BKP;
@@ -200,7 +201,7 @@
 #pragma unroll
       for (int j = 0; j < TN; ++j) {
         const int ci = ci0 + wn * WN + j * 16 + fg * 4;
-        if (co < p.Cout && ci < p.Cin) dw_store((float4*)(out + (long)co * Kw + (long)tap * p.Cin + ci), f4(acc[t][i][j]), accumulate);
+        if (co < p.Cout && ci < p.Cin) dw_store_or_finish(u, ua, out, (long)co * Kw + (long)tap * p.Cin + ci, co, f4(acc[t][i][j]), accumulate);
       }
     }
   }
@@ -215,46 +216,49 @@
   extern __shared__ __attribute__((aligned(16))) char smem[];
   const int tg = blockIdx.y / cblocks, ci0 = (blockIdx.y - tg * cblocks) * BN;
   float* out = slab ? ws + (long)blockIdx.z * slab : p.dw;
-  wgrad_tile<T, BM, BN, TX, D>(p, blockIdx.x * BM, ci0, tg, blockIdx.z, gridDim.z, out, slab == 0, smem);
+  wgrad_tile<T, BM, BN, TX, D>(p, blockIdx.x * BM, ci0, tg, blockIdx.z, gridDim.z, out, slab == 0, smem, upd_prob{}, l2s_wgrad_upd_args{});
 }
 
 
 typedef l2s::wgrad_tile_prefix wg_prefix;
 
 template <typename T, int BM, int BN, int TX, int D, int KSTEP, int WGM = 2, int WGN = 2>
-__global__ __launch_bounds__(64 * WGM * WGN) void wgrad_grouped_kernel(const wgp* __restrict__ tab, const wg_prefix pre, float* ws) {
+__global__ __launch_bounds__(64 * WGM * WGN) void wgrad_grouped_kernel(const wgp* __restrict__ tab, const wg_prefix pre, float* ws, const l2s::wgrad_upd_ctx uc) {
   extern __shared__ __attribute__((aligned(16))) char smem[];
   const int G = pre.tile0[pre.n];
   for (int L = blockIdx.x; L < G; L += gridDim.x) {
     int t;
-    const wgp p = tab[tile_of(pre, L, t)];
+    const int pi = tile_of(pre, L, t);
+    const wgp p = tab[pi];
     const int co_tiles = (p.Cout + BM - 1) / BM, ci_tiles = (p.Cin + BN - 1) / BN;
     const int split = p.split > 1 ? p.split : 1;
     const int sp = t % split; t /= split;
     const int cot = t % co_tiles, rest = t / co_tiles, cit = rest % ci_tiles, tg = rest / ci_tiles;
     float* out = split > 1 ? ws + p.ws_off + (long)sp * ((long)p.Cout * p.KH * p.KW * p.Cin) : p.dw;
-    wgrad_tile<T, BM, BN, TX, D, KSTEP, WGM, WGN>(p, cot * BM, cit * BN, tg, sp, split, out, split == 1 && !(p.flags & 1), smem);
+    const upd_prob u = split == 1 ? upd_of(uc, pi, p) : upd_prob{};
+    wgrad_tile<T, BM, BN, TX, D, KSTEP, WGM, WGN>(p, cot * BM, cit * BN, tg, sp, split, out, split == 1 && !(p.flags & 1), smem, u, uc.a);
     __syncthreads();
   }
 }
 
-__device__ __forceinline__ void reduce_slabs(float* dw, const float* ws, long n4, long slab, int split, bool accumulate) {
+__device__ __forceinline__ void reduce_slabs(float* dw, const float* ws, long n4, long slab, int split, bool accumulate, const upd_prob& u,
+                                             const l2s_wgrad_upd_args& ua, long Kw) {
   for (long e = blockIdx.x * (long)blockDim.x + threadIdx.x; e < n4; e += (long)gridDim.x * blockDim.x) {
     float4 s = ((const float4*)ws)[e];
     for (int k = 1; k < split; ++k) s = add4(s, ((const float4*)(ws + (long)k * slab))[e]);
-    dw_store((float4*)dw + e, s, accumulate);
-  }
-}
-
-__global__ __launch_bounds__(256) void wgrad_reduce_grouped_kernel(const wgp* __restrict__ tab, const float* __restrict__ ws) {
+    dw_store_or_finish(u, ua, dw, 4 * e, u.on ? (int)(4 * e / Kw) : 0, s, accumulate);
+  }
+}
+
+__global__ __launch_bounds__(256) void wgrad_reduce_grouped_kernel(const wgp* __restrict__ tab, const float* __restrict__ ws, const l2s::wgrad_upd_ctx uc) {
   const wgp p = tab[blockIdx.y];
   if (p.split <= 1) return;
   const long slab = (long)p.Cout * p.KH * p.KW * p.Cin;
-  reduce_slabs(p.dw, ws + p.ws_off, slab / 4, slab, p.split, !(p.flags & 1));
+  reduce_slabs(p.dw, ws + p.ws_off, slab / 4, slab, p.split, !(p.flags & 1), upd_of(uc, blockIdx.y, p), uc.a, (long)p.KH * p.KW * p.Cin);
 }
 
 __global__ __launch_bounds__(256) void wgrad_reduce_kernel(float* __restrict__ dw, const float* __restrict__ ws, long n4, long slab, int split) {
-  reduce_slabs(dw, ws, n4, slab, split, true);
+  reduce_slabs(dw, ws, n4, slab, split, true, upd_prob{}, l2s_wgrad_upd_args{}, 1);
 }
 
 using namespace l2s_knobs;
@@ -307,7 +311,7 @@
 }
 
 template <typename T, int BM, int BN, int TX, int D, int KSTEP, int WGM = 2, int WGN = 2>
-int launch_grouped(const wgp* tab, const wg_prefix& pre, float* ws, bool any_split, hipStream_t st) {
+int launch_grouped(const wgp* tab, const wg_prefix& pre, float* ws, bool any_split, const l2s::wgrad_upd_ctx& uc, hipStream_t st) {
   size_t lds = wgrad_lds<T, BM, BN, TX, KSTEP>();
   constexpr size_t want = 54000, want_big = 83000;
   if (BM * BN >= 128 * 128) { if (want_big > lds) lds = want_big; }
@@ -318,10 +322,10 @@
     const int var = BM == 256 ? 4 : (TX == 3 ? (BM == 128 ? 3 : 2) : (BM == 128 ? 1 : 0));
     if (cap > 0 && grid > cap && (vmask == 0 || ((vmask >> var) & 1))) grid = cap;
   }
-  WGRAD_LAUNCH((wgrad_grouped_kernel<T, BM, BN, TX, D, KSTEP, WGM, WGN>), dim3(grid), dim3(64 * WGM * WGN), lds, st, tab, pre, ws);
+  WGRAD_LAUNCH((wgrad_grouped_kernel<T, BM, BN, TX, D, KSTEP, WGM, WGN>), dim3(grid), dim3(64 * WGM * WGN), lds, st, tab, pre, ws, uc);
   if (any_split) {
     const float* wsc = ws;
-    L2S_LAUNCH(wgrad_reduce_grouped_kernel, dim3(64, pre.n), dim3(256), 0, st, tab, wsc);
+    L2S_LAUNCH(wgrad_reduce_grouped_kernel, dim3(64, pre.n), dim3(256), 0, st, tab, wsc, uc);
   }
   return l2s_check_launch();
 }
@@ -347,13 +351,13 @@
 }
 extern "C" long l2s_wgrad_tiles(int variant, int Cin, int Cout, int KH, int KW) { return variant_tiles(variant, Cin, Cout, KH, KW); }
 
-extern "C" int l2s_conv_wgrad_grouped(const l2s_wgrad_prob* table_dev, const l2s_wgrad_prob* table_host, int nprob, int variant, int dtype,
-                                      float* ws, size_t ws_bytes, hipStream_t stream) {
+static int wgrad_grouped_go(const l2s_wgrad_prob* table_dev, const l2s_wgrad_prob* table_host, int nprob, int variant, int dtype,
+                            float* ws, size_t ws_bytes, const l2s::wgrad_upd_ctx& uc, hipStream_t stream) {
   if (!table_dev || !table_host || nprob < 1 || nprob > L2S_WGRAD_MAX_GROUP || variant < 0 || variant > 6) return L2S_EINVAL;
   if (variant >= 5 && dtype != L2S_BF16) return L2S_EINVAL;
   for (int i = 0; i < nprob; ++i) if (!prob_ok(table_host[i], dtype) || !table_host[i].dw) return L2S_EINVAL;
-  if (variant == 6) return l2s::wgrad_1x1_dma_launch(table_dev, table_host, nprob, stream);
-  if (variant == 5) return l2s::wgrad_row3_dma_launch(table_dev, table_host, nprob, ws, ws_bytes, l2s_knobs::wgrad_row3_dma_wgs, stream);
+  if (variant == 6) return l2s::wgrad_1x1_dma_launch(table_dev, table_host, nprob, uc, stream);
+  if (variant == 5) return l2s::wgrad_row3_dma_launch(table_dev, table_host, nprob, ws, ws_bytes, l2s_knobs::wgrad_row3_dma_wgs, uc, stream);
   bool any_split = false;
   for (int i = 0; i < nprob; ++i) {
     const wgp& q = table_host[i];
@@ -368,19 +372,38 @@
   if (fill_tile_prefix(pre, table_host, nprob, [&](const wgp& q) { return variant_tiles(variant, q.Cin, q.Cout, q.KH, q.KW) * (q.split > 1 ? q.split : 1); }) >= (1L << 30)) return L2S_EINVAL;
 #define GO(T, KS)                                                                                \
   switch (variant) {                                                                             \
-    case 0: return launch_grouped<T, 64, 64, 1, 2, KS>(table_dev, pre, ws, any_split, stream);    \
-    case 1: return launch_grouped<T, 128, 128, 1, 2, KS>(table_dev, pre, ws, any_split, stream);  \
-    case 2: return launch_grouped<T, 64, 64, 3, 2, KS>(table_dev, pre, ws, any_split, stream);    \
-    case 3: return launch_grouped<T, 128, 64, 3, 2, KS>(table_dev, pre, ws, any_split, stream);   \
+    case 0: return launch_grouped<T, 64, 64, 1, 2, KS>(table_dev, pre, ws, any_split, uc, stream);    \
+    case 1: return launch_grouped<T, 128, 128, 1, 2, KS>(table_dev, pre, ws, any_split, uc, stream);  \
+    case 2: return launch_grouped<T, 64, 64, 3, 2, KS>(table_dev, pre, ws, any_split, uc, stream);    \
+    case 3: return launch_grouped<T, 128, 64, 3, 2, KS>(table_dev, pre, ws, any_split, uc, stream);   \
     default: break;                                                                              \
   }
   if (dtype == L2S_BF16) {
-    if (variant == 4) return launch_grouped<bf16_t, 256, 256, 1, 2, 1, 4, 2>(table_dev, pre, ws, any_split, stream);
+    if (variant == 4) return launch_grouped<bf16_t, 256, 256, 1, 2, 1, 4, 2>(table_dev, pre, ws, any_split, uc, stream);
     GO(bf16_t, 2)
   }
   if (dtype == L2S_F32) { GO(float, 1) }
 #undef GO
   return L2S_EINVAL;
+}
+
+extern "C" int l2s_conv_wgrad_grouped(const l2s_wgrad_prob* table_dev, const l2s_wgrad_prob* table_host, int nprob, int variant, int dtype,
+                                      float* ws, size_t ws_bytes, hipStream_t stream) {
+  return wgrad_grouped_go(table_dev, table_host, nprob, variant, dtype, ws, ws_bytes, l2s::wgrad_upd_ctx{}, stream);
+}
+
+extern "C" int l2s_conv_wgrad_grouped_update(const l2s_wgrad_prob* table_dev, const l2s_wgrad_prob* table_host, const l2s_wgrad_upd* upd_dev,
+                                             const l2s_wgrad_upd* upd_host, int nprob, int variant, int dtype, float* ws, size_t ws_bytes,
+                                             const l2s_wgrad_upd_args* args, hipStream_t stream) {
+  if (!upd_dev || !upd_host || !args || !table_host || nprob < 1 || nprob > L2S_WGRAD_MAX_GROUP) return L2S_EINVAL;
+  for (int i = 0; i < nprob; ++i) {
+    const l2s_wgrad_upd& d = upd_host[i];
+    if (!d.param) continue;
+    if (!d.mom || !d.seg || !(table_host[i].flags & 1)) return L2S_EINVAL;
+    if (((uintptr_t)d.param & 15) || ((uintptr_t)d.mom & 15) || ((uintptr_t)d.shadow & (args->shadow_dtype ? 7 : 15))) return L2S_EINVAL;
+  }
+  l2s::wgrad_upd_ctx uc; uc.tab = upd_dev; uc.a = *args;
+  return wgrad_grouped_go(table_dev, table_host, nprob, variant, dtype, ws, ws_bytes, uc, stream);
 }
 
 static int plan_split(const l2s_wgrad_desc& d, int variant, int dtype, size_t ws_bytes) {
diff --git a/lang2seg_amd/csrc/conv_wgrad_dma.hip b/lang2seg_amd/csrc/conv_wgrad_dma.hip
--- a/lang2seg_amd/csrc/conv_wgrad_dma.hip
+++ b/lang2seg_amd/csrc/conv_wgrad_dma.hip
@@ -13,7 +13,7 @@
 __device__ __forceinline__ long wg_lo(long g, long U, long G) { return g * U / G; }
 
 template <int KO, int NST>
-__global__ __launch_bounds__(512) void wgrad_row3_dma_kernel(const wgp* __restrict__ tab, const l2s::wgrad_sk_plan plan, float* __restrict__ ws) {
+__global__ __launch_bounds__(512) void wgrad_row3_dma_kernel(const wgp* __restrict__ tab, const l2s::wgrad_sk_plan plan, float* __restrict__ ws, const l2s::wgrad_upd_ctx uc) {
   extern __shared__ __attribute__((aligned(16))) char smem[];
   const int tid = threadIdx.x, lane = tid & 63;
   const int wave = __builtin_amdgcn_readfirstlane(tid >> 6);
@@ -220,6 +220,7 @@
     const bool full = slab_id < 0;
     const long Kw = 9L * p.Cin;
     float* slab = ws + (full ? 0 : slab_id) * TILE_FLOATS;
+    const upd_prob up = full ? upd_of(uc, plo, p) : upd_prob{};
 #pragma unroll
     for (int t = 0; t < 3; ++t)
 #pragma unroll
@@ -228,7 +229,7 @@
 #pragma unroll
         for (int j = 0; j < 2; ++j) {
           const int cil = wn * 32 + j * 16 + fg * 4;
-          if (full) dw_store((float4*)(p.dw + (long)(co0 + col) * Kw + (long)(ky * 3 + t) * p.Cin + ci0 + cil), f4(acc[t][i][j]), !(p.flags & 1));
+          if (full) dw_store_or_finish(up, uc.a, p.dw, (long)(co0 + col) * Kw + (long)(ky * 3 + t) * p.Cin + ci0 + cil, co0 + col, f4(acc[t][i][j]), !(p.flags & 1));
           else *(float4*)(slab + ((long)(t * BM + col) * BN + cil)) = f4(acc[t][i][j]);
         }
       }
@@ -237,7 +238,7 @@
   }
 }
 
-__global__ __launch_bounds__(256) void wgrad_row3_reduce_kernel(const wgp* __restrict__ tab, const l2s::wgrad_sk_plan plan, const float* __restrict__ ws, int G) {
+__global__ __launch_bounds__(256) void wgrad_row3_reduce_kernel(const wgp* __restrict__ tab, const l2s::wgrad_sk_plan plan, const float* __restrict__ ws, int G, const l2s::wgrad_upd_ctx uc) {
   int T = blockIdx.y, pi = 0;
   for (; pi < plan.n; ++pi) {
     const int tiles = (int)((plan.unit0[pi + 1] - plan.unit0[pi]) / plan.S[pi]);
@@ -266,6 +267,7 @@
   const int co_tiles = p.Cout / BM, ci_tiles = p.Cin / BN;
   const int cot = T % co_tiles, rest = T / co_tiles, cit = rest % ci_tiles, ky = rest / ci_tiles;
   const long Kw = 9L * p.Cin;
+  const upd_prob u = upd_of(uc, pi, p);
   for (int e = blockIdx.x * blockDim.x + threadIdx.x; e < TILE_FLOATS / 4; e += gridDim.x * blockDim.x) {
     float4 s = make_float4(0.f, 0.f, 0.f, 0.f);
     for (long g = g0; g <= g1; ++g) {
@@ -273,7 +275,7 @@
       s = add4(s, ((const float4*)(ws + sl * TILE_FLOATS))[e]);
     }
     const int f = e * 4, t = f / (BM * BN), col = (f - t * BM * BN) / BN, cil = f % BN;
-    dw_store((float4*)(p.dw + (long)(cot * BM + col) * Kw + (long)(ky * 3 + t) * p.Cin + cit * BN + cil), s, !(p.flags & 1));
+    dw_store_or_finish(u, uc.a, p.dw, (long)(cot * BM + col) * Kw + (long)(ky * 3 + t) * p.Cin + cit * BN + cil, cot * BM + col, s, !(p.flags & 1));
   }
 }
 
@@ -291,7 +293,7 @@
 long wgrad_row3_dma_tiles(int Cin, int Cout) { return (long)(Cout / BM) * (Cin / BN) * 3; }
 size_t wgrad_row3_dma_ws_bytes(int G) { return (size_t)G * 3 * TILE_FLOATS * sizeof(float); }
 
-int wgrad_row3_dma_launch(const l2s_wgrad_prob* tab_dev, const l2s_wgrad_prob* tab_host, int nprob, float* ws, size_t ws_bytes, int G, hipStream_t st) {
+int wgrad_row3_dma_launch(const l2s_wgrad_prob* tab_dev, const l2s_wgrad_prob* tab_host, int nprob, float* ws, size_t ws_bytes, int G, const wgrad_upd_ctx& uc, hipStream_t st) {
   if (G < 1 || nprob < 1 || nprob > L2S_WGRAD_MAX_GROUP) return L2S_EINVAL;
   wgrad_sk_plan plan;
   plan.n = nprob;
@@ -326,7 +328,7 @@
   long nslabs = plan.mode == 1 ? (long)G * (plan.Q + (plan.r ? 1 : 0)) : (long)G * 2;
   if (plan.mode == 1 && ws_bytes < (size_t)nslabs * TILE_FLOATS * sizeof(float)) { plan.mode = 0; nslabs = (long)G * 2; }
   if (!ws || ws_bytes < (size_t)nslabs * TILE_FLOATS * sizeof(float)) return L2S_EINVAL;
-#define GO(KO_, NST_) WGRAD_LAUNCH((wgrad_row3_dma_kernel<KO_, NST_>), dim3(G), dim3(512), (size_t)NST_ * STG, st, tab_dev, plan, ws);
+#define GO(KO_, NST_) WGRAD_LAUNCH((wgrad_row3_dma_kernel<KO_, NST_>), dim3(G), dim3(512), (size_t)NST_ * STG, st, tab_dev, plan, ws, uc);
 #ifdef L2S_TOOLS
   switch (l2s_knobs::row3_form) {
     case 1: GO(1, 4) break; case 2: GO(2, 4) break; case 5: GO(5, 4) break; case 6: GO(6, 4) break; case 7: GO(7, 4) break;
@@ -338,7 +340,7 @@
 #endif
 #undef GO
   const float* wsc = ws;
-  L2S_LAUNCH(wgrad_row3_reduce_kernel, dim3(12, total_tiles), dim3(256), 0, st, tab_dev, plan, wsc, G);
+  L2S_LAUNCH(wgrad_row3_reduce_kernel, dim3(12, total_tiles), dim3(256), 0, st, tab_dev, plan, wsc, G, uc);
   return l2s_check_launch();
 }
 
diff --git a/lang2seg_amd/csrc/conv_wgrad_dma1.hip b/lang2seg_amd/csrc/conv_wgrad_dma1.hip
--- a/lang2seg_amd/csrc/conv_wgrad_dma1.hip
+++ b/lang2seg_amd/csrc/conv_wgrad_dma1.hip
@@ -9,7 +9,7 @@
 constexpr int NP = 4;
 
 template <int NST>
-__global__ __launch_bounds__(512) void wgrad_1x1_dma_kernel(const wgp* __restrict__ tab, const l2s::wgrad_tile_prefix pre) {
+__global__ __launch_bounds__(512) void wgrad_1x1_dma_kernel(const wgp* __restrict__ tab, const l2s::wgrad_tile_prefix pre, const l2s::wgrad_upd_ctx uc) {
   extern __shared__ __attribute__((aligned(16))) char smem[];
   const int tid = threadIdx.x, lane = tid & 63;
   const int wave = __builtin_amdgcn_readfirstlane(tid >> 6);
@@ -17,7 +17,8 @@
   const int wm = wave >> 1, wn = wave & 1;
   const int fr = lane & 15, fg = lane >> 4;
   int t;
-  const wgp p = tab[tile_of(pre, (int)blockIdx.x, t)];
+  const int pi = tile_of(pre, (int)blockIdx.x, t);
+  const wgp p = tab[pi];
   const int co_tiles = p.Cout / BM;
   const int co0 = (t % co_tiles) * BM, ci0 = (t / co_tiles) * BN;
   const int M0 = p.n_img[0] * p.OH[0] * p.OW[0], M1 = p.nseg > 1 ? p.n_img[1] * p.OH[1] * p.OW[1] : 0;
@@ -100,13 +101,14 @@
   }
   if (grp == 0) wg_barrier();
   const bool overwrite = p.flags & 1;
+  const upd_prob u = upd_of(uc, pi, p);
 #pragma unroll
   for (int i = 0; i < 4; ++i) {
     const long co = co0 + wm * 64 + i * 16 + fr;
 #pragma unroll
     for (int j = 0; j < 8; ++j) {
       const int ci = ci0 + wn * 128 + j * 16 + fg * 4;
-      dw_store((float4*)(p.dw + co * p.Cin + ci), f4(acc[i][j]), !overwrite);
+      dw_store_or_finish(u, uc.a, p.dw, co * p.Cin + ci, (int)co, f4(acc[i][j]), !overwrite);
     }
   }
 }
@@ -125,12 +127,12 @@
 }
 long wgrad_1x1_dma_tiles(int Cin, int Cout) { return (long)(Cout / BM) * (Cin / BN); }
 
-int wgrad_1x1_dma_launch(const l2s_wgrad_prob* tab_dev, const l2s_wgrad_prob* tab_host, int nprob, hipStream_t st) {
+int wgrad_1x1_dma_launch(const l2s_wgrad_prob* tab_dev, const l2s_wgrad_prob* tab_host, int nprob, const wgrad_upd_ctx& uc, hipStream_t st) {
   for (int i = 0; i < nprob; ++i) if (!wgrad_1x1_dma_ok(tab_host[i])) return L2S_EINVAL;
   wgrad_tile_prefix pre;
   const long t = fill_tile_prefix(pre, tab_host, nprob, [](const wgp& q) { return wgrad_1x1_dma_tiles(q.Cin, q.Cout); });
   const size_t lds = (size_t)4 * STG;
-  WGRAD_LAUNCH(wgrad_1x1_dma_kernel<4>, dim3((unsigned)t), dim3(512), lds, st, tab_dev, pre);
+  WGRAD_LAUNCH(wgrad_1x1_dma_kernel<4>, dim3((unsigned)t), dim3(512), lds, st, tab_dev, pre, uc);
   return l2s_check_launch();
 }
 
diff --git a/lang2seg_amd/csrc/misc_kernels.hip b/lang2seg_amd/csrc/misc_kernels.hip
--- a/lang2seg_amd/csrc/misc_kernels.hip
+++ b/lang2seg_amd/csrc/misc_kernels.hip
@@ -2,6 +2,7 @@
 #include "../../include/lang2seg_hip.h"
 #include "pool_bins.h"
 #include "rows.h"
+#include "sgd_elem.h"
 
 namespace {
 
@@ -527,11 +528,8 @@
 }
 
 constexpr int SGD_CHUNK = 4096;
-__device__ __forceinline__ void sgd_elem(float g, float& w, float& m, float rs, float gscale, float lwd, float momentum, float llr) {
-  const float gg = g * gscale * rs + lwd * w;
-  m = momentum * m + gg;
-  w = w - llr * m;
-}
+using l2s_sgd::sgd_elem;
+using l2s_sgd::shadow_val;
 __global__ __launch_bounds__(256) void sgd_kernel(float* __restrict__ param, float* __restrict__ grad, float* __restrict__ mom,
                                                   const l2s_sgd_seg* __restrict__ segs, int nseg, const float* __restrict__ rowscale,
                                                   float lr, float momentum, float wd, float gscale, void* shadow, int sdt, int flags,
@@ -547,6 +545,7 @@
       if (segs[mid].chunk0 - c0 <= c) slo = mid; else shi = mid - 1;
     }
     const l2s_sgd_seg sg = segs[slo];
+    if ((sg.flags & L2S_SEG_UPDATED) && clear && !shadow_only) continue;
     const long base = (long)(c - (sg.chunk0 - c0)) * SGD_CHUNK;
     const int n = (int)((sg.count - base) < SGD_CHUNK ? (sg.count - base) : SGD_CHUNK);
     const float lwd = sg.weight_decay ? wd : 0.f;
@@ -588,9 +587,9 @@
       }
       if (shadow) {
         if (sdt) {
-          uint2 pk; pk.x = (uint32_t)f2bf(ww[0] * rs) | ((uint32_t)f2bf(ww[1] * rs) << 16); pk.y = (uint32_t)f2bf(ww[2] * rs) | ((uint32_t)f2bf(ww[3] * rs) << 16);
+          uint2 pk; pk.x = (uint32_t)f2bf(shadow_val(ww[0], rs)) | ((uint32_t)f2bf(shadow_val(ww[1], rs)) << 16); pk.y = (uint32_t)f2bf(shadow_val(ww[2], rs)) | ((uint32_t)f2bf(shadow_val(ww[3], rs)) << 16);
           *(uint2*)((bf16_t*)shadow + o) = pk;
-        } else *(float4*)((float*)shadow + o) = make_float4(ww[0] * rs, ww[1] * rs, ww[2] * rs, ww[3] * rs);
+        } else *(float4*)((float*)shadow + o) = make_float4(shadow_val(ww[0], rs), shadow_val(ww[1], rs), shadow_val(ww[2], rs), shadow_val(ww[3], rs));
       }
     }
     for (int i = (nv << 2) + threadIdx.x; i < n; i += 256) {
@@ -604,7 +603,7 @@
         mom[o] = m; param[o] = w;
         if (clr && !g16) grad[o] = 0.f;
       }
-      if (shadow) stx(shadow, o, sdt, w * rs);
+      if (shadow) stx(shadow, o, sdt, shadow_val(w, rs));
     }
   }
 }
diff --git a/lang2seg_amd/csrc/sgd_elem.h b/lang2seg_amd/csrc/sgd_elem.h
--- /dev/null
+++ b/lang2seg_amd/csrc/sgd_elem.h
@@ -0,0 +1,18 @@
+#pragma once
+#include <hip/hip_runtime.h>
+
+namespace l2s_sgd {
+
+__device__ __forceinline__ void sgd_elem(float g, float& w, float& m, float rs, float gscale, float lwd, float momentum, float llr) {
+#pragma clang fp contract(off)
+  const float gg = __fmaf_rn(lwd, w, __fmul_rn(__fmul_rn(g, gscale), rs));
+  m = __fmaf_rn(momentum, m, gg);
+  w = __fmaf_rn(-llr, m, w);
+}
+
+__device__ __forceinline__ float shadow_val(float w, float rs) {
+#pragma clang fp contract(off)
+  return __fmul_rn(w, rs);
+}
+
+}
diff --git a/lang2seg_amd/csrc/wgrad_common.h b/lang2seg_amd/csrc/wgrad_common.h
--- a/lang2seg_amd/csrc/wgrad_common.h
+++ b/lang2seg_amd/csrc/wgrad_common.h
@@ -1,19 +1,21 @@
 #pragma once
 #include "common.h"
 #include "../../include/lang2seg_hip.h"
+#include "sgd_elem.h"
 #include <stddef.h>
 
 typedef l2s_wgrad_prob wgp;
 
 namespace l2s {
+struct wgrad_upd_ctx { const l2s_wgrad_upd* tab; l2s_wgrad_upd_args a; };
 struct wgrad_sk_plan { int n; long U; long unit0[L2S_WGRAD_MAX_GROUP + 1]; int S[L2S_WGRAD_MAX_GROUP]; int mode, T, Ng, k1, Q, r, m; };
 bool wgrad_row3_dma_ok(const l2s_wgrad_prob& q);
 long wgrad_row3_dma_tiles(int Cin, int Cout);
 size_t wgrad_row3_dma_ws_bytes(int G);
-int wgrad_row3_dma_launch(const l2s_wgrad_prob* tab_dev, const l2s_wgrad_prob* tab_host, int nprob, float* ws, size_t ws_bytes, int G, hipStream_t st);
+int wgrad_row3_dma_launch(const l2s_wgrad_prob* tab_dev, const l2s_wgrad_prob* tab_host, int nprob, float* ws, size_t ws_bytes, int G, const wgrad_upd_ctx& uc, hipStream_t st);
 bool wgrad_1x1_dma_ok(const l2s_wgrad_prob& q);
 long wgrad_1x1_dma_tiles(int Cin, int Cout);
-int wgrad_1x1_dma_launch(const l2s_wgrad_prob* tab_dev, const l2s_wgrad_prob* tab_host, int nprob, hipStream_t st);
+int wgrad_1x1_dma_launch(const l2s_wgrad_prob* tab_dev, const l2s_wgrad_prob* tab_host, int nprob, const wgrad_upd_ctx& uc, hipStream_t st);
 
 struct wgrad_tile_prefix { int n; int tile0[L2S_WGRAD_MAX_GROUP + 1]; };
 }
@@ -89,4 +91,39 @@
   *q = v;
 }
 
+
+struct upd_prob { float* param; float* mom; void* shadow; long rs_off; float lwd, llr; bool on; };
+__device__ __forceinline__ upd_prob upd_of(const l2s::wgrad_upd_ctx& c, int pi, const wgp& p) {
+  upd_prob u = {};
+  if (!c.tab || !(p.flags & 1)) return u;
+  const l2s_wgrad_upd d = c.tab[pi];
+  if (!d.param) return u;
+  const l2s_sgd_seg sg = *d.seg;
+  if (!(sg.flags & L2S_SEG_UPDATED)) return u;
+  u.param = d.param; u.mom = d.mom; u.shadow = d.shadow; u.rs_off = sg.rowscale_off;
+  u.lwd = sg.weight_decay ? c.a.wd : 0.f; u.llr = c.a.lr * sg.lr_mult; u.on = true;
+  return u;
 }
+__device__ __forceinline__ void dw_finish(const upd_prob& u, const l2s_wgrad_upd_args& a, long e, int co, const float4& g) {
+  const float4 w4 = *(const float4*)(u.param + e), m4 = *(const float4*)(u.mom + e);
+  const float rs = u.rs_off >= 0 ? a.rowscale[u.rs_off + co] : 1.f;
+  float gg[4] = {g.x, g.y, g.z, g.w}, ww[4] = {w4.x, w4.y, w4.z, w4.w}, mm[4] = {m4.x, m4.y, m4.z, m4.w};
+#pragma unroll
+  for (int k = 0; k < 4; ++k) l2s_sgd::sgd_elem(gg[k], ww[k], mm[k], rs, a.grad_scale, u.lwd, a.momentum, u.llr);
+  *(float4*)(u.mom + e) = make_float4(mm[0], mm[1], mm[2], mm[3]);
+  *(float4*)(u.param + e) = make_float4(ww[0], ww[1], ww[2], ww[3]);
+  if (u.shadow) {
+#pragma unroll
+    for (int k = 0; k < 4; ++k) ww[k] = l2s_sgd::shadow_val(ww[k], rs);
+    if (a.shadow_dtype) {
+      uint2 pk; pk.x = (uint32_t)f2bf(ww[0]) | ((uint32_t)f2bf(ww[1]) << 16); pk.y = (uint32_t)f2bf(ww[2]) | ((uint32_t)f2bf(ww[3]) << 16);
+      *(uint2*)((bf16_t*)u.shadow + e) = pk;
+    } else *(float4*)((float*)u.shadow + e) = make_float4(ww[0], ww[1], ww[2], ww[3]);
+  }
+}
+__device__ __forceinline__ void dw_store_or_finish(const upd_prob& u, const l2s_wgrad_upd_args& a, float* dw, long e, int co, const float4& v, bool accumulate) {
+  if (u.on) dw_finish(u, a, e, co, v);
+  else dw_store((float4*)(dw + e), v, accumulate);
+}
+
+}
diff --git a/lang2seg_amd/nets/network.py b/lang2seg_amd/nets/network.py
--- a/lang2seg_amd/nets/network.py
+++ b/lang2seg_amd/nets/network.py
@@ -112,8 +112,17 @@
     def add(self, dw, g, x, n, IH, IW, Cin, OH, OW, Cout, k, stride, pad, lddy=None, ldx=None):
         self.items.append((dw, g, x, n, IH, IW, Cin, OH, OW, Cout, k, stride, pad, Cout if lddy is None else lddy, Cin if ldx is None else ldx))
 
+    def _fold_op(self):
+        net = self.net
+        op = getattr(net, '_early_op', None)
+        if not net.update_fold or op is None or net.dp is not None or net.defer_heads or not getattr(net, 'wgrad_overwrite', False):
+            return None
+        if not getattr(op, 'clear_grad', False) or getattr(op, 'defer_active', False) or getattr(net, '_fresh', None) is None:
+            return None
+        return op
+
     def flush(self, tag):
-        from .._lib import WgradProb, ptr, load
+        from .._lib import WgradProb, WgradUpd, L2SError, ptr, load
         import ctypes as C
         if not self.items:
             return False
@@ -124,6 +133,12 @@
         for it in items:
             by_dw.setdefault((it[0].data_ptr(), it[6], it[9], it[10], it[11], it[12]), []).append(it)
         rounds = {}
+        fold_op = self._fold_op()
+        P = getattr(net, 'P', None)
+        given = getattr(net, '_fold_given', None)
+        if given is None:
+            given = net._fold_given = set()
+        several = set(key[0] for key, uses in by_dw.items() if len(uses) > 2)
         for key, uses in by_dw.items():
             for r in range(0, len(uses), 2):
                 seg = uses[r:r + 2]
@@ -157,6 +172,8 @@
                     if v == 4:
                         want = max(1, self.V4_FILL // max(total, 1))
                     arr = (WgradProb * len(chunk))()
+                    uarr = (WgradUpd * len(chunk))()
+                    nfold = 0
                     flop, off = 0.0, 0
                     for i, seg in enumerate(chunk):
                         dw, g, x, n, IH, IW, Cin, OH, OW, Cout, k, stride, pad, lddy, ldx = seg[0]
@@ -166,6 +183,22 @@
                         if fresh is not None and rnd == 0 and dw.data_ptr() not in fresh and dw.numel() == Cout * k * k * Cin:
                             q.flags = 1
                             fresh.add(dw.data_ptr())
+                        dp_ = dw.data_ptr()
+                        if q.flags == 1 and fold_op is not None and dp_ not in several and dp_ not in net._fold_blocked:
+                            si = P.fold_segment(dw, Cout, k * k * Cin)
+                            if si is not None:
+                                off, ud = int(P.seg_offs[si]), uarr[i]
+                                ud.param, ud.mom = P.param.data_ptr() + 4 * off, P.mom.data_ptr() + 4 * off
+                                ud.shadow = P.shadow.data_ptr() + P.shadow.element_size() * off
+                                ud.seg = P.segs_dev.data_ptr() + si * P.seg_size
+                                given.add(dp_)
+                                nfold += 1
+                        elif dp_ in given:
+                            if dp_ in P._upd_key:
+                                raise L2SError('a weight gradient was added to a tensor that its first launch of the step had already updated '
+                                               '(the schedule changed under ParamStore.mark_updated); set Network.update_fold = False')
+                            given.discard(dp_)
+                            net._fold_blocked = net._fold_blocked | {dp_}
                         slices = min(u[3] * u[7] * (u[8] + (1 if v in (2, 3, 5) else 0)) // bkp for u in seg)
                         split = max(1, min(want, slices // 16, 16))
                         if v in (5, 6):
@@ -180,7 +213,7 @@
                             q.dy[s_], q.x[s_] = u[1].data_ptr(), u[2].data_ptr()
                             q.n_img[s_], q.IH[s_], q.IW[s_], q.OH[s_], q.OW[s_], q.lddy[s_], q.ldx[s_] = u[3], u[4], u[5], u[7], u[8], u[13], u[14]
                             flop += 2.0 * u[3] * u[7] * u[8] * Cout * k * k * Cin
-                    raw = bytes(arr)
+                    raw = bytes(arr) + (bytes(uarr) if nfold else b'')
                     ck = (tag, rnd, v, c0, getattr(net, '_rec_key', None))
                     ent = self.tables.get(ck)
                     if ent is None or ent[0] != raw:
@@ -193,8 +226,12 @@
                     ctx = self.on_launch(tag, v, flop, chunk[0][0][10]) if self.on_launch is not None else None
                     if ctx is not None:
                         ctx.__enter__()
-                    O.call('l2s_conv_wgrad_grouped', ent[1].data_ptr(), C.cast(arr, C.c_void_p), len(chunk), v, dt, ws.data_ptr(),
-                           ws.numel() * 4, O.stream())
+                    if nfold:
+                        O.wgrad_grouped_update(ent[1], arr, ent[1][C.sizeof(arr):], uarr, len(chunk), v, dt, ws, P.rowscale, fold_op.lr,
+                                               fold_op.momentum, fold_op.weight_decay, fold_op.grad_scale, O.dt_of(P.shadow))
+                    else:
+                        O.call('l2s_conv_wgrad_grouped', ent[1].data_ptr(), C.cast(arr, C.c_void_p), len(chunk), v, dt, ws.data_ptr(),
+                               ws.numel() * 4, O.stream())
                     if ctx is not None:
                         ctx.__exit__(None, None, None)
         return True
@@ -595,6 +632,8 @@
     rpn_bwd_early = True
     join_before_layer1 = False
     stem_mfma = True
+    update_fold = True
+    _fold_blocked = frozenset()
     wgrad_overwrite = True
     update_clears_grad = False
     SLOT_UPDATE_REST = 0
@@ -684,7 +723,9 @@
             for s in st:
                 s.zero_()
             raise L2SError('captioner recurrence: a workgroup of the resident %s launch gave up waiting for its peers (not co-resident); the '
-                           'exchange state was reset - set Network.cap_persistent = False to run the per-token launches' %
+                           'exchange state was reset - set Network.cap_persistent = False to run the per-token launches.  The step that '
+                           'produced the non-finite loss has already been applied: weights and momentum were updated with its gradients '
+                           '(the update has no finite guard), so restore them from a snapshot before going on' %
                            ' / '.join(n for n, e in zip(('forward', 'backward'), err) if e))
 
     def _loss_slots(self):
diff --git a/lang2seg_amd/nets/params.py b/lang2seg_amd/nets/params.py
--- a/lang2seg_amd/nets/params.py
+++ b/lang2seg_amd/nets/params.py
@@ -3,7 +3,7 @@
 import torch
 
 from .. import ops as O
-from .._lib import SgdSeg
+from .._lib import SgdSeg, SEG_UPDATED
 
 RESNET_LAYERS = {50: [3, 4, 6, 3], 101: [3, 4, 23, 3], 152: [3, 8, 36, 3]}
 BN_EPS = 1e-5
@@ -477,10 +477,11 @@
             arr = (SgdSeg * len(seq))(*seq)
             self._seg_tables.append(arr)
             return torch.frombuffer(bytearray(bytes(arr)), dtype=torch.uint8).to(self.device)
-        self._seg_tables, self._ow_key = [], frozenset()
+        self._seg_tables, self._ow_key, self._upd_key = [], frozenset(), frozenset()
         self.nseg = len(segs)
         self.seg_ends = [int(g.offset + g.count) for g in segs]
         self.seg_offs = [int(g.offset) for g in segs]
+        self.seg_index = {int(g.offset): i for i, g in enumerate(segs)}
         self.seg_chunks = [-(-int(g.count) // CH) for g in segs]
         self.seg_chunk0 = [sum(self.seg_chunks[:i]) for i in range(len(segs))]
         self.sgd_chunk = CH
@@ -505,7 +506,7 @@
                 was, now = g.flags & 1, int(base + 4 * int(g.offset) in key)
                 if was and not now:
                     self.grad[int(g.offset):int(g.offset + g.count)].zero_()
-                g.flags = now
+                g.flags = (g.flags & ~1) | now
             dev.copy_(torch.frombuffer(bytearray(bytes(arr)), dtype=torch.uint8))
         torch.cuda.synchronize() if self.grad.is_cuda else None
         self._ow_key = key
@@ -515,6 +516,37 @@
             return []
         base = self.grad.data_ptr()
         return [base + 4 * o for o in self.seg_offs[s0:s1] if (base + 4 * o) in self._ow_key and (base + 4 * o) not in fresh]
+
+    def fold_segment(self, dw, Cout, row):
+        if not hasattr(self, 'segs_dev') or dw.numel() != Cout * row:
+            return None
+        off = (dw.data_ptr() - self.grad.data_ptr()) // 4
+        i = self.seg_index.get(off)
+        if i is None or dw.data_ptr() != self.grad.data_ptr() + 4 * off:
+            return None
+        g = self._seg_tables[0][i]
+        if int(g.count) != Cout * row or off % 4 or (g.rowscale_off >= 0 and int(g.row_len) != row):
+            return None
+        return i
+
+    def mark_updated(self, ptrs):
+        key = frozenset(ptrs)
+        if key == self._upd_key:
+            return
+        base = self.grad.data_ptr()
+        torch.cuda.synchronize() if self.grad.is_cuda else None
+        arr = self._seg_tables[0]
+        for g in arr:
+            g.flags = (g.flags & ~SEG_UPDATED) | (SEG_UPDATED if (base + 4 * int(g.offset)) in key else 0)
+        self.segs_dev.copy_(torch.frombuffer(bytearray(bytes(arr)), dtype=torch.uint8))
+        torch.cuda.synchronize() if self.grad.is_cuda else None
+        self._upd_key = key
+
+    def stale_updated(self, s0, s1, given):
+        if not self._upd_key:
+            return []
+        base = self.grad.data_ptr()
+        return [base + 4 * o for o in self.seg_offs[s0:s1] if (base + 4 * o) in self._upd_key and (base + 4 * o) not in given]
 
     def chunk_range(self, lo, hi):
         import bisect
diff --git a/lang2seg_amd/nets/resnet_v1.py b/lang2seg_amd/nets/resnet_v1.py
--- a/lang2seg_amd/nets/resnet_v1.py
+++ b/lang2seg_amd/nets/resnet_v1.py
@@ -554,6 +554,7 @@
         main = torch.cuda.current_stream()
         S = self.streams() if self.use_streams else None
         if backward:
+            self._fold_given = set()
             self._fresh = set()
         if self.update_clears_grad:
             if backward:
diff --git a/lang2seg_amd/ops.py b/lang2seg_amd/ops.py
--- a/lang2seg_amd/ops.py
+++ b/lang2seg_amd/ops.py
@@ -1054,6 +1054,12 @@
          float(wd), float(gscale), ptr(shadow), dt_of(shadow) if shadow is not None else 0, 1 if clear_grad else 0, stream())
 
 
+def wgrad_grouped_update(table_dev, table_host, upd_dev, upd_host, nprob, variant, dt, ws, rowscale, lr, momentum, wd, gscale, shadow_dt):
+    args = _lib.WgradUpdArgs(ptr(rowscale), float(lr), float(momentum), float(wd), float(gscale), int(shadow_dt), 0)
+    call('l2s_conv_wgrad_grouped_update', ptr(table_dev), C.cast(table_host, C.c_void_p), ptr(upd_dev), C.cast(upd_host, C.c_void_p), int(nprob), int(variant),
+         int(dt), ptr(ws), ws.numel() * 4 if ws is not None else 0, C.byref(args), stream())
+
+
 def sgd_momentum_range(param, grad, mom, segs_dev, nseg, rowscale, lr, momentum, wd, gscale, shadow, flags, lo, hi, chunk_lo, chunk_hi):
     call('l2s_sgd_momentum_range', ptr(param), ptr(grad), ptr(mom), ptr(segs_dev), nseg, ptr(rowscale), float(lr), float(momentum),
          float(wd), float(gscale), ptr(shadow), dt_of(shadow) if shadow is not None else 0, int(flags), int(lo), int(hi), int(chunk_lo), int(chunk_hi), stream())
diff --git a/lang2seg_amd/optim.py b/lang2seg_amd/optim.py
--- a/lang2seg_amd/optim.py
+++ b/lang2seg_amd/optim.py
@@ -47,6 +47,10 @@
     def _launch(self, s0, s1, table=None):
         P = self.net.P
         if s1 > s0:
+            if table is None and P._upd_key:
+                stale = P.stale_updated(s0, s1, getattr(self.net, '_fold_given', ()))
+                if stale:
+                    P.mark_updated(P._upd_key - frozenset(stale))
             O.sgd_momentum(P.param, P.grad, P.mom, (P.segs_dev if table is None else table)[s0 * P.seg_size:], s1 - s0, P.rowscale, self.lr,
                            self.momentum, self.weight_decay, self.grad_scale, shadow=P.shadow, clear_grad=self.clear_grad)
 
@@ -84,6 +88,12 @@
             net.P.mark_overwritten(getattr(net, '_fresh', ()))
 
     def step(self):
+        self._step()
+        net = self.net
+        if self.clear_grad and not self.defer_active and getattr(net, 'wgrad_overwrite', False) and hasattr(net.P, 'mark_updated'):
+            net.P.mark_updated(getattr(net, '_fold_given', ()) if getattr(net, 'update_fold', False) else ())
+
+    def _step(self):
         P = self.net.P
         net = self.net
         net._bwd_pending = 0
```

Result: slower. 213.8 img/s (-4.8%).
